# google/FluidNet

Measured on AMD Instinct MI355X. Metric: simulate_mcells_per_s, higher is better.
Workload: dtype f32

## Files before the change

fluidnet_amd/csrc/abi.cpp:

```cpp
#include "../../include/tfluids_hip.h"

#include <hip/hip_runtime.h>

#include <algorithm>
#include <cmath>
#include <cstdarg>
#include <cstdio>
#include <cstdlib>
#include <cstring>
#include <string>

#include <vector>

#include "tfl_device.hpp"
#include "tfl_host.hpp"
#include "tfl_advect.hpp"

struct tfl_layer {
  int cin = 0, cout = 0, k = 0;
  int pool = 1;
  int up = 1;
  float* w = nullptr;
  float* b = nullptr;
  int dil = 1;
// ... 285 lines not shown
    char tmp[256];
    snprintf(tmp, sizeof(tmp), "%s\"%s\": {\"calls\": %lld, \"ms\": %.6f}", i ? ", " : "", names[i].c_str(), calls[i], ms[i]);
    js += tmp;
  }
  js += "}";
  if (buf && cap > 0) {
    const size_t n = js.size() < (size_t)cap - 1 ? js.size() : (size_t)cap - 1;
    memcpy(buf, js.data(), n);
    buf[n] = 0;
  }
  return (int)names.size();
}

int64_t tfl_trace_errors(tfl_ctx* c) {
  if (!c) return -1;
  unsigned long long v = 0;
  if (hipMemcpyAsync(&v, c->d_trace_err, sizeof(v), hipMemcpyDeviceToHost, c->stream) != hipSuccess) return -1;
  if (hipMemsetAsync(c->d_trace_err, 0, sizeof(v), c->stream) != hipSuccess) return -1;
  if (hipStreamSynchronize(c->stream) != hipSuccess) return -1;
  return (int64_t)v;
}

int tfl_advectScalar(tfl_ctx* c, float dt, const tfl_tensor* s, const tfl_tensor* U, const tfl_tensor* flags,
                     const tfl_tensor* fwd, const tfl_tensor* bwd, int is3D, const char* method,
                     const tfl_tensor* fwdPos, const tfl_tensor* bwdPos, int boundaryWidth, int sampleOutsideFluid,
                     float maccormackStrength, const tfl_tensor* sDst) {
  (void)bwd; (void)boundaryWidth;
  TRY(check_flags(c, "advectScalar", flags));
  TRY(check_vel(c, "advectScalar", "U", U, flags, is3D));
  TRY(check_scalar(c, "advectScalar", "s", s, flags));
  TRY(check_scalar(c, "advectScalar", "sDst", sDst, flags));
  const int m = parse_method(method);
  if (m < 0) return fail(c, TFL_EINVAL, "advectScalar: unknown advection method '%s'", method ? method : "(null)");
  if (sDst->data == s->data && m != tfl::kMacCormackOurs)
    return fail(c, TFL_EINVAL, "advectScalar: sDst must not alias s for method '%s'", method);
  float* fwd_p = nullptr;
  float* bounds_p = nullptr;
  float* mm_p = nullptr;
  if (m == tfl::kMacCormack || m == tfl::kMacCormackOurs) {
    TRY(check_scalar(c, "advectScalar", "fwd", fwd, flags));
    fwd_p = fwd->data;
  }
  if (m == tfl::kMacCormackOurs) {
    TRY(check_vel(c, "advectScalar", "fwdPos", fwdPos, flags, is3D));
    TRY(check_vel(c, "advectScalar", "bwdPos", bwdPos, flags, is3D));
    bounds_p = fwdPos->data;
    mm_p = bwdPos->data;
  }
  WindowScope win(c);
  tfl::advect_scalar(c->stream, is3D != 0, m, flags->B, flags->Z, flags->Y, flags->X, dt, maccormackStrength,
                     sampleOutsideFluid != 0, c->d_trace_err, s->data, U->data, flags->data, fwd_p, bounds_p, mm_p,
                     sDst->data, stages_of(c));
  return check_launch(c, "advectScalar");
}

int tfl_advectVel(tfl_ctx* c, float dt, const tfl_tensor* U, const tfl_tensor* flags, const tfl_tensor* fwd,
                  const tfl_tensor* bwd, int is3D, const char* method, int boundaryWidth, float maccormackStrength,
                  const tfl_tensor* UDst) {
  (void)bwd; (void)boundaryWidth;
  TRY(check_flags(c, "advectVel", flags));
  TRY(check_vel(c, "advectVel", "U", U, flags, is3D));
  TRY(check_vel(c, "advectVel", "UDst", UDst, flags, is3D));
  int m = parse_method(method);
  if (m < 0) return fail(c, TFL_EINVAL, "advectVel: unknown advection method '%s'", method ? method : "(null)");
  if (UDst->data == U->data) return fail(c, TFL_EINVAL, "advectVel: UDst must not alias U");
  float* fwd_p = nullptr;
  if (m != tfl::kEuler && m != tfl::kEulerOurs) {
    TRY(check_vel(c, "advectVel", "fwd", fwd, flags, is3D));
    fwd_p = fwd->data;
  }
  WindowScope win(c);
  tfl::advect_vel(c->stream, is3D != 0, m, flags->B, flags->Z, flags->Y, flags->X, dt, maccormackStrength,
                  c->d_trace_err, U->data, flags->data, fwd_p, UDst->data, stages_of(c));
  return check_launch(c, "advectVel");
}

}
namespace tfl {
int advect_pair(tfl_ctx* c, float dt, float strength, const tfl_tensor* s, const tfl_tensor* U, const tfl_tensor* flags,
                const tfl_tensor* sfwd, const tfl_tensor* sbounds, const tfl_tensor* sDst, const tfl_tensor* vfwd, const tfl_tensor* UDst,
                const BcFoldArg& fold_s, const BcFoldArg& fold_v) {
  TRY(check_flags(c, "advectPair", flags));
  TRY(check_vel(c, "advectPair", "U", U, flags, 1));
  TRY(check_vel(c, "advectPair", "UDst", UDst, flags, 1));
  TRY(check_vel(c, "advectPair", "vfwd", vfwd, flags, 1));
  TRY(check_scalar(c, "advectPair", "s", s, flags));
  TRY(check_scalar(c, "advectPair", "sDst", sDst, flags));
  TRY(check_scalar(c, "advectPair", "sfwd", sfwd, flags));
  if (!sbounds || !sbounds->data || sbounds->C < 2 || !same_dims(sbounds, flags)) return fail(c, TFL_EINVAL, "advectPair: bounds needs two planes of the flags size");
  if (UDst->data == U->data) return fail(c, TFL_EINVAL, "advectPair: UDst must not alias U");
  WindowScope win(c);
  AdvArgs a; a.d = make_dom(flags->Z, flags->Y, flags->X); a.dt = dt; a.strength = strength; a.outside = 0; a.err = c->d_trace_err; a.fast = g_advect_fast;
  a.ord = BlockOrder{};
  if (!advect_pair3(c->stream, a, flags->B, s->data, U->data, flags->data, sfwd->data, sbounds->data, sDst->data, vfwd->data, UDst->data,
                    stages_of(c), fold_s, fold_v))
    return TFL_EUNSUPPORTED;
  return check_launch(c, "advectPair");
}
}
extern "C" {

int tfl_setWallBcsForward(tfl_ctx* c, const tfl_tensor* U, const tfl_tensor* flags, int is3D) {
  TRY(check_flags(c, "setWallBcsForward", flags));
  TRY(check_vel(c, "setWallBcsForward", "U", U, flags, is3D));
  tfl::set_wall_bcs(c->stream, is3D != 0, flags->B, flags->Z, flags->Y, flags->X, U->data, flags->data);
  return check_launch(c, "setWallBcsForward");
}

int tfl_velocityDivergenceForward(tfl_ctx* c, const tfl_tensor* U, const tfl_tensor* flags, const tfl_tensor* UDiv,
                                  int is3D) {
  TRY(check_flags(c, "velocityDivergenceForward", flags));
  TRY(check_vel(c, "velocityDivergenceForward", "U", U, flags, is3D));
  TRY(check_scalar(c, "velocityDivergenceForward", "UDiv", UDiv, flags));
  tfl::velocity_divergence(c->stream, is3D != 0, flags->B, flags->Z, flags->Y, flags->X, U->data, flags->data,
                           UDiv->data);
  return check_launch(c, "velocityDivergenceForward");
}

int tfl_velocityUpdateForward(tfl_ctx* c, const tfl_tensor* U, const tfl_tensor* flags, const tfl_tensor* p,
                              int is3D) {
  TRY(check_flags(c, "velocityUpdateForward", flags));
  TRY(check_vel(c, "velocityUpdateForward", "U", U, flags, is3D));
  TRY(check_scalar(c, "velocityUpdateForward", "p", p, flags));
  tfl::velocity_update(c->stream, is3D != 0, flags->B, flags->Z, flags->Y, flags->X, U->data, flags->data, p->data);
  return check_launch(c, "velocityUpdateForward");
}

int tfl_vorticityConfinement(tfl_ctx* c, const tfl_tensor* U, const tfl_tensor* flags, float strength,
                             const tfl_tensor* centered, const tfl_tensor* curl, const tfl_tensor* curlNorm,
                             const tfl_tensor* force, int is3D) {
  (void)centered; (void)force;
  TRY(check_flags(c, "vorticityConfinement", flags));
  TRY(check_vel(c, "vorticityConfinement", "U", U, flags, is3D));
  if (!curl || !curl->data || curl->C != 3 || !same_dims(curl, flags))
    return fail(c, TFL_EINVAL, "vorticityConfinement: curl must be a 3-channel grid of the flags size");
  TRY(check_scalar(c, "vorticityConfinement", "curlNorm", curlNorm, flags));
  WindowScope win(c);
  const int stg = stages_of(c);
  tfl::vorticity_confinement(c->stream, is3D != 0, flags->B, flags->Z, flags->Y, flags->X, U->data, flags->data,
                             strength, curl->data, curlNorm->data, ((stg & 2) ? 1 : 0) | ((stg & 4) ? 2 : 0));
  return check_launch(c, "vorticityConfinement");
}

int tfl_vorticityConfinementFrom(tfl_ctx* c, const tfl_tensor* USrc, const tfl_tensor* U, const tfl_tensor* flags, float strength,
                                 const tfl_tensor* curl, const tfl_tensor* curlNorm, int is3D) {
  TRY(check_flags(c, "vorticityConfinementFrom", flags));
  TRY(check_vel(c, "vorticityConfinementFrom", "U", U, flags, is3D));
  TRY(check_vel(c, "vorticityConfinementFrom", "USrc", USrc, flags, is3D));
  if (USrc->data == U->data) return fail(c, TFL_EINVAL, "vorticityConfinementFrom: U must not alias USrc (use vorticityConfinement)");
  if (!curl || !curl->data || curl->C != 3 || !same_dims(curl, flags))
    return fail(c, TFL_EINVAL, "vorticityConfinementFrom: curl must be a 3-channel grid of the flags size");
  TRY(check_scalar(c, "vorticityConfinementFrom", "curlNorm", curlNorm, flags));
  WindowScope win(c);
  if (is3D && !c->vort_from_two_launch && tfl::vorticity_confinement_fused_ok(true, flags->Z, flags->Y, flags->X) &&
      tfl::vorticity_confinement_fused(c->stream, flags->B, flags->Z, flags->Y, flags->X, USrc->data, U->data, flags->data, strength))
    return check_launch(c, "vorticityConfinementFrom");
  const tfl::ZWin w0 = tfl::g_zwin;
  const bool windowed = w0.a1 > w0.a0 || w0.b1 > w0.b0;
  if (windowed) {
    tfl::ZWin wa = {std::max(w0.a0 - 2, 0), std::min(w0.a1 + 2, (int)flags->Z), 0, 0};
    if (w0.b1 > w0.b0) { wa.b0 = std::max(w0.b0 - 2, 0); wa.b1 = std::min(w0.b1 + 2, (int)flags->Z); }
    if (w0.a1 <= w0.a0) { wa.a0 = wa.b0; wa.a1 = wa.b1; wa.b0 = wa.b1 = 0; }
    else if (wa.b1 > wa.b0 && wa.b0 <= wa.a1) { wa.a1 = wa.b1; wa.b0 = wa.b1 = 0; }
    tfl::g_zwin = wa;
    const bool a_ok = tfl::vorticity_confinement(c->stream, is3D != 0, flags->B, flags->Z, flags->Y, flags->X, U->data, flags->data, strength,
                                                 curl->data, curlNorm->data, 1, USrc->data);
    tfl::g_zwin = w0;
    if (a_ok && tfl::vorticity_confinement(c->stream, is3D != 0, flags->B, flags->Z, flags->Y, flags->X, U->data, flags->data, strength,
                                           curl->data, curlNorm->data, 2, USrc->data))
      return check_launch(c, "vorticityConfinementFrom");
    if (a_ok) return fail(c, TFL_EUNSUPPORTED, "vorticityConfinementFrom: pass B could not read USrc on this grid under a z-window");
  } else if (tfl::vorticity_confinement(c->stream, is3D != 0, flags->B, flags->Z, flags->Y, flags->X, U->data, flags->data, strength,
                                        curl->data, curlNorm->data, 3, USrc->data))
    return check_launch(c, "vorticityConfinementFrom");
  if (windowed)
    return fail(c, TFL_EUNSUPPORTED, "vorticityConfinementFrom: this grid takes the one-cell kernels, which do not run from USrc under a z-window; "
                                     "copy USrc into U and call tfl_vorticityConfinement per pass (tfl_set_stages) with the passes' own windows");
  {
    const tfl::Dom d = tfl::make_dom(flags->Z, flags->Y, flags->X);
    const size_t plane = sizeof(float) * (size_t)flags->Y * flags->X;
    const int C = is3D ? 3 : 2;
    for (int b = 0; b < flags->B; b++)
      for (int ch = 0; ch < C; ch++) {
        const size_t row = ((size_t)b * C + ch) * flags->Z;
        if (d.n0 > 0) HIP_TRY(c, hipMemcpyAsync(U->data + (row + d.w0) * (plane / 4), USrc->data + (row + d.w0) * (plane / 4), plane * d.n0, hipMemcpyDeviceToDevice, c->stream));
        if (d.nw > d.n0) HIP_TRY(c, hipMemcpyAsync(U->data + (row + d.w1) * (plane / 4), USrc->data + (row + d.w1) * (plane / 4), plane * (d.nw - d.n0), hipMemcpyDeviceToDevice, c->stream));
      }
  }
  tfl::vorticity_confinement(c->stream, is3D != 0, flags->B, flags->Z, flags->Y, flags->X, U->data, flags->data, strength,
                             curl->data, curlNorm->data, 3);
  return check_launch(c, "vorticityConfinementFrom");
}

int tfl_addBuoyancyFrom(tfl_ctx* c, const tfl_tensor* USrc, const tfl_tensor* U, const tfl_tensor* flags,
                        const tfl_tensor* density, const float gravity[3], float dt, int is3D) {
  TRY(check_flags(c, "addBuoyancy", flags));
  TRY(check_vel(c, "addBuoyancy", "U", U, flags, is3D));
  TRY(check_vel(c, "addBuoyancy", "USrc", USrc, flags, is3D));
  TRY(check_scalar(c, "addBuoyancy", "density", density, flags));
  if (!gravity) return fail(c, TFL_EINVAL, "addBuoyancy: gravity is null");
  const float sc = dt / get_dx(c, flags);
  WindowScope win(c);
  tfl::add_buoyancy(c->stream, is3D != 0, flags->B, flags->Z, flags->Y, flags->X, USrc->data, U->data, flags->data,
                    density->data, -gravity[0] * sc, -gravity[1] * sc, -gravity[2] * sc);
  return check_launch(c, "addBuoyancy");
}

int tfl_addBuoyancy(tfl_ctx* c, const tfl_tensor* U, const tfl_tensor* flags, const tfl_tensor* density,
                    const float gravity[3], float* strengthTmp, float dt, int is3D) {
  (void)strengthTmp;
  return tfl_addBuoyancyFrom(c, U, U, flags, density, gravity, dt, is3D);
}

int tfl_addGravity(tfl_ctx* c, const tfl_tensor* U, const tfl_tensor* flags, const float gravity[3], float dt,
                   int is3D, float* forceTmp) {
  (void)forceTmp;
  TRY(check_flags(c, "addGravity", flags));
  TRY(check_vel(c, "addGravity", "U", U, flags, is3D));
  if (!gravity) return fail(c, TFL_EINVAL, "addGravity: gravity is null");
  const float sc = dt / get_dx(c, flags);
  WindowScope win(c);
  tfl::add_gravity(c->stream, is3D != 0, flags->B, flags->Z, flags->Y, flags->X, U->data, flags->data,
                   gravity[0] * sc, gravity[1] * sc, gravity[2] * sc);
  return check_launch(c, "addGravity");
}

int tfl_emptyDomain(tfl_ctx* c, const tfl_tensor* flags, int is3D, int bnd) {
  TRY(check_flags(c, "emptyDomain", flags));
  if (!is3D && flags->Z != 1) return fail(c, TFL_EINVAL, "emptyDomain: 2D domain but zdepth > 1");
  tfl::empty_domain(c->stream, is3D != 0, bnd, flags->B, flags->Z, flags->Y, flags->X, flags->data);
  return check_launch(c, "emptyDomain");
}

int tfl_flagsToOccupancy(tfl_ctx* c, const tfl_tensor* flags, const tfl_tensor* occupancy) {
  TRY(check_flags(c, "flagsToOccupancy", flags));
  TRY(check_scalar(c, "flagsToOccupancy", "occupancy", occupancy, flags));
  tfl::flags_to_occupancy(c->stream, (long long)flags->B * flags->Z * flags->Y * flags->X, flags->data,
                          occupancy->data);
  return check_launch(c, "flagsToOccupancy");
}

int tfl_rectangularBlur(tfl_ctx* c, const tfl_tensor* src, int blurRad, int is3D, const tfl_tensor* dst,
                        const tfl_tensor* tmp) {
  if (!c) return TFL_EINVAL;
  if (!src || !dst || !tmp || !src->data || !dst->data || !tmp->data) return fail(c, TFL_EINVAL, "rectangularBlur: null tensor");
  if (!same_dims(dst, src) || dst->C != src->C || !same_dims(tmp, src) || tmp->C != src->C)
    return fail(c, TFL_EINVAL, "rectangularBlur: src, dst and tmp must have the same size");
  if (blurRad <= 0) return fail(c, TFL_EINVAL, "rectangularBlur: blurRad must be a positive, non-zero integer");
  if (!is3D && src->Z != 1) return fail(c, TFL_EINVAL, "rectangularBlur: 2D field but zdepth > 1");
  if (dst->data == src->data || tmp->data == src->data || tmp->data == dst->data)
    return fail(c, TFL_EINVAL, "rectangularBlur: src, dst and tmp must not alias");
  tfl::rectangular_blur(c->stream, is3D != 0, src->B, src->C, src->Z, src->Y, src->X, blurRad, src->data, dst->data, tmp->data);
  return check_launch(c, "rectangularBlur");
}

int tfl_signedDistanceField(tfl_ctx* c, const tfl_tensor* flags, int searchRad, int is3D, const tfl_tensor* dst) {
  TRY(check_flags(c, "signedDistanceField", flags));
  TRY(check_scalar(c, "signedDistanceField", "dst", dst, flags));
  if (searchRad <= 0) return fail(c, TFL_EINVAL, "signedDistanceField: searchRad must be a positive, non-zero integer");
  if (!is3D && flags->Z != 1) return fail(c, TFL_EINVAL, "signedDistanceField: 2D domain but zdepth > 1");
  tfl::signed_distance_field(c->stream, flags->B, flags->Z, flags->Y, flags->X, searchRad, flags->data, dst->data);
  return check_launch(c, "signedDistanceField");
}

int64_t tfl_pcg_workspace_floats(int32_t Z, int32_t Y, int32_t X) { return tfl::pcg_workspace_floats(Z, Y, X); }

int tfl_solveLinearSystemPCG(tfl_ctx* c, const tfl_tensor* p, const tfl_tensor* flags, const tfl_tensor* div, int is3D,
                             const char* precondType, float tol, int maxIter, int verbose, float* workspace,
                             int64_t workspace_floats, float* residual) {
  TRY(check_flags(c, "solveLinearSystemPCG", flags));
  TRY(check_scalar(c, "solveLinearSystemPCG", "p", p, flags));
  TRY(check_scalar(c, "solveLinearSystemPCG", "div", div, flags));
  if (!is3D && flags->Z != 1) return fail(c, TFL_EINVAL, "solveLinearSystemPCG: d > 1 for a 2D domain");
  int pc = -1;
  const std::string pt = precondType ? precondType : "ic0";
  if (pt == "none") pc = 0; else if (pt == "ilu0") pc = 1; else if (pt == "ic0") pc = 2;
  if (pc < 0) return fail(c, TFL_EINVAL, "solveLinearSystemPCG: precondType is not supported.");
  if (!workspace || ((uintptr_t)workspace & 7) != 0) return fail(c, TFL_EINVAL, "solveLinearSystemPCG: workspace must be 8-byte aligned");
  if (workspace_floats < tfl::pcg_workspace_floats(flags->Z, flags->Y, flags->X))
    return fail(c, TFL_EINVAL, "solveLinearSystemPCG: workspace too small (tfl_pcg_workspace_floats)");
  if ((long long)flags->Z * flags->Y * flags->X >= (1ll << 31)) return fail(c, TFL_EINVAL, "solveLinearSystemPCG: grid too large for 32-bit cell indices");
  char msg[256] = {0};
  int rc = tfl::pcg_solve(c->stream, is3D != 0, flags->B, flags->Z, flags->Y, flags->X, p->data, flags->data, div->data,
                          pc, tol, maxIter, verbose, workspace, residual, msg, sizeof(msg), c->wf_skip == 0);
  if (c->wf_skip > 0) c->wf_skip--;
  if (rc == -5) {
    c->wf_timeouts++;
    c->wf_skip = 16 << (c->wf_timeouts < 7 ? c->wf_timeouts - 1 : 6);
    fprintf(stderr, "[tfl] solveLinearSystemPCG: a pipelined triangular sweep timed out (something else holds part of the GPU?); "
                    "this solve and the next %d on this context use hyperplane sweeps (slower), then the pipelined form is retried\n", c->wf_skip);
  }
  if (rc == -5)
    rc = tfl::pcg_solve(c->stream, is3D != 0, flags->B, flags->Z, flags->Y, flags->X, p->data, flags->data, div->data,
                        pc, tol, maxIter, verbose, workspace, residual, msg, sizeof(msg), false);
  if (rc == -1 || rc == -3) return fail(c, TFL_EINVAL, "%s", msg);
  if (rc == -2) return fail(c, TFL_EINVAL, "%s", msg);
  if (rc != 0) return fail(c, TFL_EHIP, "%s", msg);
  return check_launch(c, "solveLinearSystemPCG");
}

int64_t tfl_normalize_workspace_floats(int32_t Z, int32_t Y, int32_t X) { return tfl::npm_workspace_floats(Z, Y, X); }

int tfl_normalizePressureMean(tfl_ctx* c, const tfl_tensor* p, const tfl_tensor* flags, int is3D, float* workspace,
                              int64_t workspace_floats) {
  TRY(check_flags(c, "normalizePressureMean", flags));
  TRY(check_scalar(c, "normalizePressureMean", "p", p, flags));
  if (!is3D && flags->Z != 1) return fail(c, TFL_EINVAL, "normalizePressureMean: 2D domain but zdepth > 1");
  if (!workspace || ((uintptr_t)workspace & 7) != 0) return fail(c, TFL_EINVAL, "normalizePressureMean: workspace must be 8-byte aligned");
  if (workspace_floats < tfl::npm_workspace_floats(flags->Z, flags->Y, flags->X))
// ... 367 lines not shown
      if (N > 1 && st >= g->split_stage && st < g->join_stage) {
        if (down < m->bank_down) m->bank_down = down;
        if (cp > m->bank_c) m->bank_c = cp;
      }
      down *= L.pool;
      const int bank_max = (N > 1 && mres && st >= g->split_stage && st < g->join_stage) ? down << (N - 1) : down;
      if (bank_max > m->max_down) m->max_down = bank_max;
      if (L.pool > 1 || L.up > 1 || down != 1) m->multires = true;
    }
    const int C = st == 1 ? in_c : cout[first_of[st - 1]];
    auto cmap = [&](int ci) {
      if (skip_in && ci == cin[i] - 1) return cin_p - 1;
      return joined ? (ci / C) * prev_p + ci % C : ci;
    };
    L.cin = cin_p; L.cout = cp; L.k = ksize[i];
    const int taps = is3D ? L.k * L.k * L.k : L.k * L.k;
    const int S = is3D ? L.up * L.up * L.up : L.up * L.up;
    std::vector<float> relaid((size_t)S * taps * L.cin * L.cout, 0.0f);
    for (int sub = 0; sub < S; sub++)
      for (int co = 0; co < cout[i]; co++)
        for (int ci = 0; ci < cin[i]; ci++)
          for (int t = 0; t < taps; t++)
            relaid[(((size_t)sub * taps + t) * L.cin + cmap(ci)) * L.cout + co] = weights[i][(((size_t)co * S + sub) * cin[i] + ci) * taps + t];
    std::vector<float> bias_p((size_t)S * L.cout, 0.0f);
    for (int sub = 0; sub < S; sub++)
      for (int co = 0; co < cout[i]; co++) bias_p[(size_t)sub * L.cout + co] = biases[i][(size_t)co * S + sub];
    std::vector<float> bn;
    if (g->batch_norm && !last) {
      if (!g->bn_mean[i] || !g->bn_var[i]) { m->layers.push_back(L); return cleanup("addBatchNorm: a module lacks running_mean / running_var"); }
      bn.assign((size_t)2 * L.cout, 0.0f);
      for (int co = 0; co < cout[i]; co++) {
        const double wt = (g->bn_weight && g->bn_weight[i]) ? (double)g->bn_weight[i][co] : 1.0;
        const double bi = (g->bn_bias && g->bn_bias[i]) ? (double)g->bn_bias[i][co] : 0.0;
        const double sc = wt / std::sqrt((double)g->bn_var[i][co] + g->bn_eps[i]);
        bn[co] = (float)sc;
        bn[L.cout + co] = (float)(bi - (double)g->bn_mean[i][co] * sc);
      }
    }
    if (hipMalloc((void**)&L.w, relaid.size() * sizeof(float)) != hipSuccess ||
        hipMalloc((void**)&L.b, bias_p.size() * sizeof(float)) != hipSuccess ||
        hipMemcpy(L.w, relaid.data(), relaid.size() * sizeof(float), hipMemcpyHostToDevice) != hipSuccess ||
        hipMemcpy(L.b, bias_p.data(), bias_p.size() * sizeof(float), hipMemcpyHostToDevice) != hipSuccess ||
        (!bn.empty() && (hipMalloc((void**)&L.bn, bn.size() * sizeof(float)) != hipSuccess ||
                         hipMemcpy(L.bn, bn.data(), bn.size() * sizeof(float), hipMemcpyHostToDevice) != hipSuccess))) {
      m->layers.push_back(L);
      return cleanup("uploading weights failed");
    }
    m->layers.push_back(L);
    const int width = (N > 1 && st == g->join_stage - 1 && concat) ? cp * N : cp + (o.pressure_skip ? 1 : 0);
    if (!last && width > m->max_c) m->max_c = width;
  }
  if (down != 1) return cleanup("the layers do not return to the grid resolution (pool / up factors)");
  if (N > 1 && mres) m->multires = true;
  if (m->max_c < 1) m->max_c = 1;
  return m;
}

void tfl_model_destroy(tfl_ctx* c, tfl_model* m) {
  (void)c;
  if (!m) return;
  for (auto& L : m->layers) { if (L.w) (void)hipFree(L.w); if (L.b) (void)hipFree(L.b); if (L.bn) (void)hipFree(L.bn); }
  for (int l = 0; l < 3; l++) if (m->bfrag[l]) (void)hipFree(m->bfrag[l]);
  for (int l = 0; l < 3; l++) if (m->wino[l]) (void)hipFree(m->wino[l]);
  for (int l = 0; l < 3; l++) if (m->wfrag16[l]) (void)hipFree(m->wfrag16[l]);
  if (m->d_range_err) (void)hipFree(m->d_range_err);
  if (m->h_range) (void)hipHostFree(m->h_range);
  for (int l = 0; l < 4; l++) if (m->bfrag2[l]) (void)hipFree(m->bfrag2[l]);
  if (m->tail_w4) (void)hipFree(m->tail_w4);
  if (m->tail_pack) (void)hipFree(m->tail_pack);
  if (m->tail_w5) (void)hipFree(m->tail_w5);
  if (m->d_stats) (void)hipFree(m->d_stats);
  if (m->d_ticket) (void)hipFree(m->d_ticket);
  delete m;
}

int64_t tfl_model_range_errors(tfl_ctx* c, tfl_model* m) {
  if (!c || !m) return -1;
  if (!m->d_range_err) return 0;
  unsigned long long v = 0;
  if (hipMemcpyAsync(&v, m->d_range_err, sizeof(v), hipMemcpyDeviceToHost, c->stream) != hipSuccess) return -1;
  if (hipMemsetAsync(m->d_range_err, 0, sizeof(v), c->stream) != hipSuccess) return -1;
  if (hipStreamSynchronize(c->stream) != hipSuccess) return -1;
  if (m->h_range) *(volatile unsigned long long*)m->h_range = 0;
  return (int64_t)v;
}


int64_t tfl_model_range_flag(tfl_ctx* c, tfl_model* m) {
  if (!c || !m) return -1;
  return m->h_range ? (int64_t)*(volatile unsigned long long*)m->h_range : 0;
}

static int range_gate(tfl_ctx* c, tfl_model* m, const char* who) {
  if (c && c->in_step) return TFL_OK;
  if (m && m->h_range && *(volatile unsigned long long*)m->h_range != 0)
    return fail(c, TFL_ERANGE, "%s: an earlier forward pass of this model clamped activations at the fp16 range (|x| > 65504 after the "
                               "std normalisation: a blown-up simulation); its pressure is not the reference's. Read and reset the count with "
                               "tfl_model_range_errors, or create the model under TFL_CONV_PATH=winograd (strict fp32, no range limit)", who);
  return TFL_OK;
}

static int64_t graph_ws_floats(const tfl_model* m, int B, int Z, int Y, int X, float* base, float* (*bank)[2], float** pyr = nullptr) {
  if (!m->graph || m->banks < 2) return 0;
  auto cells = [&](int f) { return (int64_t)B * (m->is3d ? (Z + f - 1) / f : Z) * ((Y + f - 1) / f) * ((X + f - 1) / f); };
  const bool mres = m->bank_type == TFL_BANKS_MRES;
  int64_t off = 0;
  for (int i = 0; i < m->banks; i++) {
    const int64_t n = (int64_t)m->bank_c * cells(mres ? m->bank_down << i : m->bank_down);
    if (base) { bank[i][0] = base + off; bank[i][1] = base + off + n; }
    off += 2 * n;
    if (mres && i > 0) {
      if (base) pyr[i] = base + off;
      off += (int64_t)m->split_c * cells(m->split_down << i);
    }
  }
  return off;
}

int64_t tfl_model_workspace_floats(const tfl_model* m, int B, int Z, int Y, int X) {
  if (!m) return -1;
  const int64_t n = (int64_t)B * Z * Y * X;
  return 4 * tfl::model_stat_blocks(B, Z, Y, X) + n * (1 + (int64_t)m->in_c + 2 * (int64_t)m->max_c + 1) + (m->m16 ? 4 : 0) +
         graph_ws_floats(m, B, Z, Y, X, nullptr, nullptr);
}

namespace {
struct ModelWs { double* partials; float* div; float* x3; float* act[2]; float* pPred; float* bank[tfl::kMaxJoinBanks][2]; float* pyr[tfl::kMaxJoinBanks]; };
int model_ws(tfl_ctx* c, const tfl_model* m, const tfl_tensor* flags, float* workspace, int64_t workspace_floats,
             ModelWs* w) {
  const int B = flags->B, Z = flags->Z, Y = flags->Y, X = flags->X;
  if (B > kMaxBatch) return fail(c, TFL_EINVAL, "model: batch size above %d", kMaxBatch);
  const int64_t n = (int64_t)B * Z * Y * X;
  if (!workspace || workspace_floats < tfl_model_workspace_floats(m, B, Z, Y, X))
    return fail(c, TFL_EINVAL, "model: workspace too small (%lld floats needed)",
                (long long)tfl_model_workspace_floats(m, B, Z, Y, X));
  if (((uintptr_t)workspace & 7) != 0) return fail(c, TFL_EINVAL, "model: workspace must be 8-byte aligned");
  w->partials = (double*)workspace;
  w->div = workspace + 4 * tfl::model_stat_blocks(B, Z, Y, X);
  w->x3 = w->div + n;
  w->act[0] = w->x3 + (int64_t)m->in_c * n;
  if (m->m16) w->act[0] = (float*)(((uintptr_t)w->act[0] + 15) & ~(uintptr_t)15);
  w->act[1] = w->act[0] + (int64_t)m->max_c * n;
  w->pPred = w->act[1] + (int64_t)m->max_c * n;
  graph_ws_floats(m, B, Z, Y, X, w->pPred + n, w->bank, w->pyr);
  return TFL_OK;
}
}

float* tfl_model_div(const tfl_model* m, int B, int Z, int Y, int X, float* workspace) {
  if (!m || !workspace) return nullptr;
  return workspace + 4 * tfl::model_stat_blocks(B, Z, Y, X);
}

static const unsigned short* wall_code_of(tfl_ctx* c, const tfl_model* m, const tfl_tensor* flags) {
  std::lock_guard<std::mutex> lock(c->wall_mu);
  for (const tfl_wall_plan* wp : c->wall_plans)
    if (wp->flags == flags->data && wp->is3d == m->is3d && wp->B == flags->B && wp->Z == flags->Z && wp->Y == flags->Y && wp->X == flags->X) return wp->code;
  return nullptr;
}

static int graph_gate(tfl_ctx* c, const tfl_model* m, const tfl_tensor* flags, const char* who) {
  if (!m->graph) return TFL_OK;
  const int f = m->max_down;
  if ((m->is3d && flags->Z % f) || flags->Y % f || flags->X % f)
    return fail(c, TFL_EINVAL, "%s: grid %dx%dx%d is not divisible by the model's downsampling factor %d (banks x pooling)", who,
                flags->Z, flags->Y, flags->X, f);
  return TFL_OK;
}

int tfl_model_begin(tfl_ctx* c, tfl_model* m, const tfl_tensor* UDiv, const tfl_tensor* flags, const tfl_tensor* UOut,
                    float* workspace, int64_t workspace_floats, int zlo, int zhi, double* stats) {
  TRY(check_flags(c, "model_begin", flags));
  if (!m) return fail(c, TFL_EINVAL, "model_begin: null model");
  TRY(range_gate(c, m, "model_begin"));
  const int is3D = m->is3d ? 1 : 0;
  TRY(check_vel(c, "model_begin", "UDiv", UDiv, flags, is3D));
  TRY(check_vel(c, "model_begin", "UOut", UOut, flags, is3D));
  if (zlo < 0 || zhi > flags->Z || zlo >= zhi) return fail(c, TFL_EINVAL, "model_begin: bad z range [%d, %d)", zlo, zhi);
  TRY(graph_gate(c, m, flags, "model_begin"));
  ModelWs w;
  TRY(model_ws(c, m, flags, workspace, workspace_floats, &w));
  WindowScope win(c);
  int stg = stages_of(c);
  if (c->defer_stats) stg &= ~4;
  m->stat_pairs_per_plane = tfl::model_stat_pairs_per_plane(flags->B, flags->Z, flags->Y, flags->X, UDiv->data, flags->data, UOut->data, w.div);
  const unsigned short* code = wall_code_of(c, m, flags);
  tfl::model_pre(c->stream, m->is3d, flags->B, flags->Z, flags->Y, flags->X, UDiv->data, flags->data, UOut->data,
                 w.div, w.partials, stats ? stats : m->d_stats, zlo, zhi, ((stg & 2) ? 1 : 0) | ((stg & 4) ? 2 : 0), m->d_ticket, code);
  return check_launch(c, "model_begin");
}

tfl_wall_plan* tfl_wall_plan_create(tfl_ctx* c, const tfl_tensor* flags) {
  if (!c || !flags || !flags->data) return nullptr;
  if (check_flags(c, "wall_plan_create", flags) != TFL_OK) return nullptr;
  const long long n = (long long)flags->B * flags->Z * flags->Y * flags->X;
  tfl_wall_plan* p = new tfl_wall_plan();
  p->flags = flags->data; p->B = flags->B; p->Z = flags->Z; p->Y = flags->Y; p->X = flags->X;
  if (hipMalloc((void**)&p->code, (size_t)n * sizeof(unsigned short)) != hipSuccess) { (void)hipGetLastError(); c->err = "wall_plan_create: hipMalloc failed"; delete p; return nullptr; }
  (void)hipDeviceSynchronize();
  p->is3d = flags->Z > 1; p->owner = c;
  tfl::wall_code(c->stream, p->is3d, flags->B, flags->Z, flags->Y, flags->X, flags->data, p->code);
  if (hipStreamSynchronize(c->stream) != hipSuccess) { (void)hipGetLastError(); (void)hipFree(p->code); c->err = "wall_plan_create: the code kernel failed"; delete p; return nullptr; }
  std::lock_guard<std::mutex> lock(c->wall_mu);
  for (tfl_wall_plan*& q : c->wall_plans)
    if (q->flags == p->flags) { q->owner = nullptr; q = p; return p; }
  c->wall_plans.push_back(p);
  return p;
}

void tfl_wall_plan_retire(tfl_wall_plan* p) {
  if (!p) return;
  tfl_ctx* o = p->owner;
  if (!o) return;
  std::lock_guard<std::mutex> lock(o->wall_mu);
  for (size_t i = 0; i < o->wall_plans.size(); i++)
    if (o->wall_plans[i] == p) { o->wall_plans.erase(o->wall_plans.begin() + (long)i); break; }
  p->owner = nullptr;
}

void tfl_wall_plan_destroy(tfl_ctx* c, tfl_wall_plan* p) {
  if (!p) return;
  (void)c;
  tfl_wall_plan_retire(p);
  if (p->code) (void)hipFree(p->code);
  delete p;
}

namespace {
float* graph_layer(hipStream_t st, const tfl_model* m, const tfl_layer& L, int B, int& Zc, int& Yc, int& Xc, const float* in,
                   float* P, float* Q, float* dst, int och, int c0, int act) {
  float* conv_out = in == P ? Q : P;
  const bool pools = L.pool > 1;
  float* cdst = (pools || !dst) ? conv_out : dst;
  const float* bs = L.bn ? L.bn : nullptr;
  const float* bt = L.bn ? L.bn + L.cout : nullptr;
  const int taps = m->is3d ? L.k * L.k * L.k : L.k * L.k;
  const int S = m->is3d ? L.up * L.up * L.up : L.up * L.up;
  for (int sub = 0; sub < S; sub++)
    if (!tfl::conv_direct_graph(st, m->is3d, B, Zc, Yc, Xc, L.cin, L.cout, L.k, act, in, L.w + (size_t)sub * taps * L.cin * L.cout,
                                L.b + (size_t)sub * L.cout, cdst, L.up, sub, cdst == dst ? och : 0, cdst == dst ? c0 : 0, L.dil,
                                pools ? nullptr : bs, pools ? nullptr : bt))
      return nullptr;
  if (m->is3d) Zc *= L.up;
  Yc *= L.up; Xc *= L.up;
  if (!pools) return cdst;
  float* pdst = dst ? dst : (conv_out == P ? Q : P);
  tfl::pool2_graph(st, m->is3d, m->pool_max, B, L.cout, Zc, Yc, Xc, conv_out, pdst, dst ? och : L.cout, dst ? c0 : 0, bs, bt);
  if (m->is3d) Zc /= 2;
  Yc /= 2; Xc /= 2;
  return pdst;
}

int graph_forward(tfl_ctx* c, const tfl_model* m, hipStream_t st, const ModelWs& w, int B, int Z, int Y, int X,
                  const float* pDiv, const double* st_in, double count) {
  const int act = 1 + m->opts.nonlin;
  const int nl = (int)m->layers.size();
  const bool mres = m->bank_type == TFL_BANKS_MRES, concat = m->aggregate == TFL_AGG_CONCAT;
  const float* in = w.x3;
  int Zc = Z, Yc = Y, Xc = X;
  auto none = [&](const tfl_layer& L) { return fail(c, TFL_EUNSUPPORTED, "model_finish: no kernel for %d output channels", L.cout); };
  for (int l = 0; l < nl;) {
    const tfl_layer& L0 = m->layers[l];
    if (m->banks > 1 && L0.stage == m->split) {
      float* join = in == w.act[0] ? w.act[1] : w.act[0];
      const int N = m->banks, Cp = m->layers[l + (m->join - m->split - 1) * N].cout, och = concat ? Cp * N : Cp;
      const float* bin[tfl::kMaxJoinBanks];
      int bZ[tfl::kMaxJoinBanks], bY[tfl::kMaxJoinBanks], bX[tfl::kMaxJoinBanks];
      bin[0] = in; bZ[0] = Zc; bY[0] = Yc; bX[0] = Xc;
      for (int i = 1; i < N; i++) {
        bin[i] = in; bZ[i] = bZ[i - 1]; bY[i] = bY[i - 1]; bX[i] = bX[i - 1];
        if (!mres) continue;
        tfl::avg_pool2(st, m->is3d, B * m->split_c, bZ[i - 1], bY[i - 1], bX[i - 1], bin[i - 1], w.pyr[i]);
        bin[i] = w.pyr[i];
        if (m->is3d) bZ[i] /= 2;
        bY[i] /= 2; bX[i] /= 2;
      }
      int slot[tfl::kMaxJoinBanks], sh[tfl::kMaxJoinBanks], n = 0;
      const float* src[tfl::kMaxJoinBanks];
      int jZ = 0, jY = 0, jX = 0;
      for (int i = 0; i < N; i++) {
        const float* x = bin[i];
        int z = bZ[i], y = bY[i], xx = bX[i];
        const bool direct = i == 0 || (concat && !mres);
        for (int s = m->split; s < m->join; s++) {
          const tfl_layer& L = m->layers[l + (s - m->split) * N + i];
          const bool last = s + 1 == m->join;
          x = graph_layer(st, m, L, B, z, y, xx, x, w.bank[i][0], w.bank[i][1], (last && direct) ? join : nullptr, och,
                          concat ? i * Cp : 0, act);
          if (!x) return none(L);
        }
        if (i == 0) { jZ = z; jY = y; jX = xx; }
        if (!direct) { slot[n] = i; sh[n] = mres ? i : 0; src[n] = x; n++; }
      }
      if (n > 0 && !tfl::bank_join(st, m->is3d, !concat, B, Cp, jZ, jY, jX, n, slot, sh, src, join, och))
        return fail(c, TFL_EINVAL, "model_finish: bad bank join");
      in = join; Zc = jZ; Yc = jY; Xc = jX;
      l += (m->join - m->split) * N;
      continue;
    }
    const bool last = l + 1 == nl;
    const bool joins_skip = m->opts.pressure_skip && l + 2 == nl;
    float* dst = last ? w.pPred : (joins_skip ? (in == w.act[0] ? w.act[1] : w.act[0]) : nullptr);
    float* out = graph_layer(st, m, L0, B, Zc, Yc, Xc, in, w.act[0], w.act[1], dst, joins_skip ? L0.cout + 1 : L0.cout, 0,
                             last ? 0 : act);
    if (!out) return none(L0);
    if (joins_skip) tfl::model_skip_channel(st, B, (long long)Z * Y * X, pDiv, st_in, count, out, L0.cout + 1, L0.cout);
    in = out;
    l++;
  }
  return TFL_OK;
}
}

int tfl_model_finish(tfl_ctx* c, tfl_model* m, const tfl_tensor* pDiv, const tfl_tensor* flags,
                     const tfl_tensor* pOut, const tfl_tensor* UOut, float* workspace, int64_t workspace_floats,
                     const double* stats, double count, const tfl_tensor* UBC, const tfl_tensor* UBCInvMask,
                     int doClamp, float lo, float hi) {
  TRY(check_flags(c, "model_finish", flags));
  if (!m) return fail(c, TFL_EINVAL, "model_finish: null model");
  const int is3D = m->is3d ? 1 : 0;
  TRY(check_vel(c, "model_finish", "UOut", UOut, flags, is3D));
  TRY(check_scalar(c, "model_finish", "pDiv", pDiv, flags));
  TRY(check_scalar(c, "model_finish", "pOut", pOut, flags));
  if ((UBC == nullptr) != (UBCInvMask == nullptr)) return fail(c, TFL_EINVAL, "model_finish: UBC and UBCInvMask go together");
  if (UBC) {
    TRY(check_vel(c, "model_finish", "UBC", UBC, flags, is3D));
    TRY(check_vel(c, "model_finish", "UBCInvMask", UBCInvMask, flags, is3D));
  }
  if (!(count > 1.0)) return fail(c, TFL_EINVAL, "model_finish: Sample variance requires more than one sample.");
  ModelWs w;
  TRY(model_ws(c, m, flags, workspace, workspace_floats, &w));
  const int B = flags->B, Z = flags->Z, Y = flags->Y, X = flags->X;
  const double* st_in = stats ? stats : m->d_stats;
  hipStream_t st = c->stream;
  TRY(graph_gate(c, m, flags, "model_finish"));
  if (m->graph && (stats || c->stages || c->zwin.a1 > c->zwin.a0 || c->zwin.b1 > c->zwin.b0))
    return fail(c, TFL_EUNSUPPORTED, "model_finish: banked, batch-norm and max-pool models run un-sharded only");
  if (m->custom) {
    if (stats || c->stages || c->zwin.a1 > c->zwin.a0 || c->zwin.b1 > c->zwin.b0)
      return fail(c, TFL_EUNSUPPORTED, "model_finish: models with non-default tfl_model_opts run un-sharded only");
    const tfl_model_opts& o = m->opts;
// ... 287 lines not shown
```

fluidnet_amd/csrc/model.hip:

```cpp
#include "tfl_device.hpp"
#include "tfl_fastmath.hpp"
#include "tfl_host.hpp"
#include "tfl_vec4.hpp"

#include <algorithm>
#include <cstdlib>

#ifndef TFL_LB_BCS
#define TFL_LB_BCS 1
#endif
#ifndef TFL_LB_PROJECT
#define TFL_LB_PROJECT 1
#endif

namespace tfl {

template <bool IS3D>
__device__ __forceinline__ void wall_mask_from(int fc, int fxm, int fxp, int fym, int fyp, int fzm, int fzp, bool& zx,
                                               bool& zy, bool& zz) {
  zx = zy = zz = false;
  const bool cf = fc & kFluid, co = fc & kObstacle;
  if (!cf && !co) return;
  zx = (fxm & kObstacle) || (co && (fxm & kFluid));
  zy = (fym & kObstacle) || (co && (fym & kFluid));
  zz = IS3D && ((fzm & kObstacle) || (co && (fzm & kFluid)));
  if (cf) {
    if ((fxm & kStick) || (fxp & kStick)) { zy = true; zz = IS3D; }
    if ((fym & kStick) || (fyp & kStick)) { zx = true; zz = IS3D; }
    if (IS3D && ((fzm & kStick) || (fzp & kStick))) { zx = true; zy = true; }
  }
}

template <bool IS3D>
__device__ __forceinline__ void wall_zero_mask(const Dom& d, const float* __restrict__ flags, int i, int j, int k, int o,
                                               bool& zx, bool& zy, bool& zz) {
  const int fc = (int)flags[o];
  if (!(fc & (kFluid | kObstacle))) { zx = zy = zz = false; return; }
  const int fxm = i > 0 ? (int)flags[o - 1] : 0;
  const int fym = j > 0 ? (int)flags[o - d.sy] : 0;
  const int fzm = (IS3D && k > 0) ? (int)flags[o - d.sz] : 0;
  int fxp = 0, fyp = 0, fzp = 0;
  if (fc & kFluid) {
    fxp = i < d.X - 1 ? (int)flags[o + 1] : 0;
    fyp = j < d.Y - 1 ? (int)flags[o + d.sy] : 0;
    fzp = (IS3D && k < d.Z - 1) ? (int)flags[o + d.sz] : 0;
  }
  wall_mask_from<IS3D>(fc, fxm, fxp, fym, fyp, fzm, fzp, zx, zy, zz);
}

template <bool IS3D, int AXIS>
__device__ __forceinline__ float u_bc_at(const Dom& d, const float* __restrict__ U, const float* __restrict__ flags,
                                         int i, int j, int k) {
  const int o = TFL_AT(d, i, j, k);
  bool zx, zy, zz;
  wall_zero_mask<IS3D>(d, flags, i, j, k, o, zx, zy, zz);
  const bool z = AXIS == 0 ? zx : (AXIS == 1 ? zy : zz);
  return z ? 0.0f : U[o + AXIS * d.sc];
}

template <bool COHERENT>
__device__ __forceinline__ void reduce_partials(const double* __restrict__ p, long long count, double* __restrict__ out, int tid) {
  __shared__ double sh[512];
  if (!COHERENT) {
    double r1, r2;
    block_sum_pairs(p, count, sh, tid, r1, r2);
    if (tid == 0) { out[0] = r1; out[1] = r2; }
    return;
  }
  double s1 = 0.0, s2 = 0.0;
  for (long long t = tid; t < count; t += 256) {
    s1 += __builtin_bit_cast(double, __hip_atomic_load(reinterpret_cast<const unsigned long long*>(p + t * 2), __ATOMIC_RELAXED, __HIP_MEMORY_SCOPE_AGENT));
    s2 += __builtin_bit_cast(double, __hip_atomic_load(reinterpret_cast<const unsigned long long*>(p + t * 2 + 1), __ATOMIC_RELAXED, __HIP_MEMORY_SCOPE_AGENT));
  }
  double* sh1 = sh; double* sh2 = sh + 256;
  sh1[tid] = s1; sh2[tid] = s2;
  __syncthreads();
  for (int w = 128; w > 0; w >>= 1) {
    if (tid < w) { sh1[tid] += sh1[tid + w]; sh2[tid] += sh2[tid + w]; }
    __syncthreads();
  }
  if (tid == 0) { out[0] = sh1[0]; out[1] = sh2[0]; }
  __syncthreads();
}

struct StatTail { unsigned* ticket; double* stats; long long per_sample; unsigned per_plane, planes; int B; };
[[maybe_unused]] constexpr int kStatTickets = 1 << 16;
template <bool FOLD>
__device__ __forceinline__ void publish_and_maybe_reduce(const StatTail& tl, double* __restrict__ partials, long long blk, double p1,
                                                         double p2, int tid) {
  if (!FOLD) {
    if (tid == 0) { partials[blk * 2] = p1; partials[blk * 2 + 1] = p2; }
    return;
  }
  __shared__ int last;
  if (tid == 0) {
    if (tl.ticket) {
      __hip_atomic_store(reinterpret_cast<unsigned long long*>(partials + blk * 2), __builtin_bit_cast(unsigned long long, p1), __ATOMIC_RELAXED, __HIP_MEMORY_SCOPE_AGENT);
      __hip_atomic_store(reinterpret_cast<unsigned long long*>(partials + blk * 2 + 1), __builtin_bit_cast(unsigned long long, p2), __ATOMIC_RELAXED, __HIP_MEMORY_SCOPE_AGENT);
      asm volatile("s_waitcnt vmcnt(0)" ::: "memory");
      unsigned* mine = tl.ticket + 1 + (unsigned)(blk / tl.per_plane);
      last = 0;
      if (atomicAdd(mine, 1u) == tl.per_plane - 1u) {
        *mine = 0u;
        last = atomicAdd(tl.ticket, 1u) == tl.planes - 1u;
      }
    } else {
      partials[blk * 2] = p1; partials[blk * 2 + 1] = p2;
      last = 0;
    }
  }
  if (!tl.ticket) return;
  __syncthreads();
  if (!last) return;
  for (int b = 0; b < tl.B; b++) reduce_partials<true>(partials + (long long)b * tl.per_sample * 2, tl.per_sample, tl.stats + b * 2, tid);
  if (tid == 0) *tl.ticket = 0u;
}

template <bool IS3D, bool FOLD = false>
__global__ __launch_bounds__(256) void k_bcs_div_stats(Dom d, const float* __restrict__ U, const float* __restrict__ flags,
                                                       float* __restrict__ Ubc, float* __restrict__ div,
                                                       double* __restrict__ partials, StatTail tl) {
  const int i = blockIdx.x * blockDim.x + threadIdx.x;
  const int j = blockIdx.y * blockDim.y + threadIdx.y;
  int b, k; dom_bk(d, b, k);
  const long long cells = d.sc;
  const int C = IS3D ? 3 : 2;
  double s1 = 0.0, s2 = 0.0;
  if (i < d.X && j < d.Y) {
    U += b * cells * C; Ubc += b * cells * C; flags += b * cells; div += b * cells;
    const int o = TFL_AT(d, i, j, k);
    bool zx, zy, zz;
    wall_zero_mask<IS3D>(d, flags, i, j, k, o, zx, zy, zz);
    const float ux = zx ? 0.0f : U[o];
    const float uy = zy ? 0.0f : U[o + d.sc];
    const float uz = IS3D ? (zz ? 0.0f : U[o + 2 * d.sc]) : 0.0f;
    Ubc[o] = ux; Ubc[o + d.sc] = uy; if (IS3D) Ubc[o + 2 * d.sc] = uz;
    s1 = (double)ux + (double)uy + (double)uz;
    s2 = (double)ux * ux + (double)uy * uy + (double)uz * uz;
    float dv = 0.0f;
    if (!on_border<IS3D>(d, i, j, k) && (((int)flags[o]) & kFluid)) {
      dv = ux - u_bc_at<IS3D, 0>(d, U, flags, i + 1, j, k) + uy - u_bc_at<IS3D, 1>(d, U, flags, i, j + 1, k);
      if (IS3D) dv += (uz - u_bc_at<IS3D, 2>(d, U, flags, i, j, k + 1));
    }
    div[o] = dv;
  }
#pragma unroll
  for (int off = 32; off > 0; off >>= 1) { s1 += __shfl_down(s1, off, 64); s2 += __shfl_down(s2, off, 64); }
  __shared__ double part[8];
  const int tid = threadIdx.y * blockDim.x + threadIdx.x;
  if ((tid & 63) == 0) { part[(tid >> 6) * 2] = s1; part[(tid >> 6) * 2 + 1] = s2; }
  __syncthreads();
  const long long blk = blockIdx.x + (long long)gridDim.x * (blockIdx.y + (long long)gridDim.y * ((long long)b * d.Z + k));
  publish_and_maybe_reduce<FOLD>(tl, partials, blk, (part[0] + part[2]) + (part[4] + part[6]), (part[1] + part[3]) + (part[5] + part[7]), tid);
}

template <bool IS3D>
__global__ __launch_bounds__(256) void k_wall_code(Dom d, const float* __restrict__ flags, unsigned short* __restrict__ code) {
  const int i = blockIdx.x * blockDim.x + threadIdx.x, j = blockIdx.y * blockDim.y + threadIdx.y;
  int b, k; dom_bk(d, b, k);
  if (i >= d.X || j >= d.Y) return;
  flags += b * d.sc; code += b * d.sc;
  const int o = TFL_AT(d, i, j, k);
  const int fc = (int)flags[o];
  const int fxm = i > 0 ? (int)flags[o - 1] : 0, fxp = i < d.X - 1 ? (int)flags[o + 1] : 0;
  const int fym = j > 0 ? (int)flags[o - d.sy] : 0, fyp = j < d.Y - 1 ? (int)flags[o + d.sy] : 0;
  const int fzm = (IS3D && k > 0) ? (int)flags[o - d.sz] : 0, fzp = (IS3D && k < d.Z - 1) ? (int)flags[o + d.sz] : 0;
  bool zx, zy, zz;
  wall_mask_from<IS3D>(fc, fxm, fxp, fym, fyp, fzm, fzp, zx, zy, zz);
  unsigned m = (zx ? 1u : 0u) | (zy ? 2u : 0u) | (zz ? 4u : 0u) | ((fc & kFluid) ? 8u : 0u) | (((fc & kEmpty) && !(fc & kOutflow)) ? 16u : 0u);
  m |= ((fxm & kFluid) ? 32u : 0u) | ((fym & kFluid) ? 64u : 0u) | ((fzm & kFluid) ? 128u : 0u);
  m |= ((fxm & kEmpty) ? 256u : 0u) | ((fym & kEmpty) ? 512u : 0u) | ((fzm & kEmpty) ? 1024u : 0u);
  code[o] = (unsigned short)m;
}

template <bool IS3D>
__global__ __launch_bounds__(256, TFL_LB_BCS) void k_bcs_div_stats_code(Dom d, const float* __restrict__ U, const unsigned short* __restrict__ code,
                                                                       float* __restrict__ Ubc, float* __restrict__ div,
                                                                       double* __restrict__ partials, StatTail tl) {
  const V4Ctx c = v4_ctx(d);
  const int j = blockIdx.y * blockDim.y + threadIdx.y;
  int b, k; dom_bk(d, b, k);
  const bool live = c.i0 < d.X && j < d.Y;
  const long long cells = d.sc;
  const int C = IS3D ? 3 : 2;
  U += b * cells * C; Ubc += b * cells * C; code += b * cells; div += b * cells;
  const int o = TFL_AT(d, c.i0, j, k);
  const bool yp = live && j < d.Y - 1, zp = live && IS3D && k < d.Z - 1;
  const unsigned long long cc_v = *reinterpret_cast<const unsigned long long*>(code + (live ? o : 0));
  const unsigned long long cy_v = *reinterpret_cast<const unsigned long long*>(code + (yp ? o + d.sy : 0));
  const unsigned long long cz_v = *reinterpret_cast<const unsigned long long*>(code + (zp ? o + d.sz : 0));
  const unsigned long long cc = live ? cc_v : 0ull, cy = yp ? cy_v : 0ull, cz = zp ? cz_v : 0ull;
  float u[3][4], uyp[4], uzp[4];
#pragma unroll
  for (int a = 0; a < 3; a++) v4_load(U, o + a * d.sc, live && a < C, 0.0f, u[a]);
  v4_load(U, o + d.sc + d.sy, yp, 0.0f, uyp);
  v4_load(U, o + 2 * d.sc + d.sz, zp, 0.0f, uzp);
  const bool need = c.last && live && c.has_r;
  const int oo = o + 4;
  const unsigned gcode = code[need ? oo : 0];
  const float gu = U[need ? oo : 0];
  double s1 = 0.0, s2 = 0.0;
  float ubx[5];
#pragma unroll
  for (int q = 0; q < 4; q++) {
    const unsigned m = (unsigned)(cc >> (16 * q));
    if (m & 1u) u[0][q] = 0.0f;
    if (m & 2u) u[1][q] = 0.0f;
    if (!IS3D || (m & 4u)) u[2][q] = 0.0f;
    ubx[q] = u[0][q];
    if (live) {
      s1 += (double)u[0][q] + (double)u[1][q] + (double)u[2][q];
      s2 += (double)u[0][q] * u[0][q] + (double)u[1][q] * u[1][q] + (double)u[2][q] * u[2][q];
    }
  }
  ubx[4] = from_lane_above(ubx[0]);
  if (c.last) ubx[4] = (need && !(gcode & 1u)) ? gu : 0.0f;
  float dv[4];
  const bool row_inner = live && j >= 1 && j <= d.Y - 2 && (!IS3D || (k >= 1 && k <= d.Z - 2));
#pragma unroll
  for (int q = 0; q < 4; q++) {
    const int i = c.i0 + q;
    dv[q] = 0.0f;
    if (row_inner && i >= 1 && i <= d.X - 2 && ((unsigned)(cc >> (16 * q)) & 8u)) {
      const float by = ((unsigned)(cy >> (16 * q)) & 2u) ? 0.0f : uyp[q];
      float t = u[0][q] - ubx[q + 1] + u[1][q] - by;
      if (IS3D) {
        const float bz = ((unsigned)(cz >> (16 * q)) & 4u) ? 0.0f : uzp[q];
        t += (u[2][q] - bz);
      }
      dv[q] = t;
    }
  }
  if (live) {
#pragma unroll
    for (int a = 0; a < 3; a++)
      if (a < C) v4_store(Ubc, o + a * d.sc, u[a]);
    v4_store(div, o, dv);
  }
#pragma unroll
  for (int off = 32; off > 0; off >>= 1) { s1 += __shfl_down(s1, off, 64); s2 += __shfl_down(s2, off, 64); }
  __shared__ double part[8];
  const int tid = threadIdx.y * blockDim.x + threadIdx.x;
  if ((tid & 63) == 0) { part[(tid >> 6) * 2] = s1; part[(tid >> 6) * 2 + 1] = s2; }
  __syncthreads();
  const long long blk = blockIdx.x + (long long)gridDim.x * (blockIdx.y + (long long)gridDim.y * ((long long)b * d.Z + k));
  publish_and_maybe_reduce<false>(tl, partials, blk, (part[0] + part[2]) + (part[4] + part[6]), (part[1] + part[3]) + (part[5] + part[7]), tid);
}

template <bool IS3D, bool FOLD = false>
__global__ __launch_bounds__(256, TFL_LB_BCS) void k_bcs_div_stats_v4(Dom d, const float* __restrict__ U, const float* __restrict__ flags,
                                                          float* __restrict__ Ubc, float* __restrict__ div,
                                                          double* __restrict__ partials, StatTail tl) {
  const V4Ctx c = v4_ctx(d);
  const int j = blockIdx.y * blockDim.y + threadIdx.y;
  int b, k; dom_bk(d, b, k);
  const bool live = c.i0 < d.X && j < d.Y;
  const long long cells = d.sc;
  const int C = IS3D ? 3 : 2;
  U += b * cells * C; Ubc += b * cells * C; flags += b * cells; div += b * cells;
  const int o = TFL_AT(d, c.i0, j, k);
  const bool ym = live && j > 0, yp = live && j < d.Y - 1, yp2 = live && j < d.Y - 2;
  const bool zm = live && IS3D && k > 0, zp = live && IS3D && k < d.Z - 1, zp2 = live && IS3D && k < d.Z - 2;
  float fc[6], fym[4], fyp[6], fzm[4], fzp[6], fyp2[4], fypzm[4], fypzp[4], fzp2[4], fymzp[4];
  v4_load6<true, true>(c, flags, o, live, 0.0f, fc);
  v4_load(flags, o - d.sy, ym, 0.0f, fym);
  v4_load6<true, true>(c, flags, o + d.sy, yp, 0.0f, fyp);
  v4_load(flags, o - d.sz, zm, 0.0f, fzm);
  v4_load6<true, true>(c, flags, o + d.sz, zp, 0.0f, fzp);
  v4_load(flags, o + 2 * d.sy, yp2, 0.0f, fyp2);
  v4_load(flags, o + d.sy - d.sz, yp && zm, 0.0f, fypzm);
  v4_load(flags, o + d.sy + d.sz, yp && zp, 0.0f, fypzp);
  v4_load(flags, o + 2 * d.sz, zp2, 0.0f, fzp2);
  v4_load(flags, o - d.sy + d.sz, ym && zp, 0.0f, fymzp);
  float u[3][4], uyp[4], uzp[4];
#pragma unroll
  for (int a = 0; a < 3; a++) v4_load(U, o + a * d.sc, live && a < C, 0.0f, u[a]);
  v4_load(U, o + d.sc + d.sy, yp, 0.0f, uyp);
  v4_load(U, o + 2 * d.sc + d.sz, zp, 0.0f, uzp);
  const bool need = c.last && live && c.has_r;
  const int oo = o + 4;
  const float gym = flags[need && ym ? oo - d.sy : 0], gyp = flags[need && yp ? oo + d.sy : 0];
  const float gzm = flags[need && zm ? oo - d.sz : 0], gzp = flags[need && zp ? oo + d.sz : 0];
  const float gu = U[need ? oo : 0];
  double s1 = 0.0, s2 = 0.0;
  float ubx[5];
#pragma unroll
  for (int q = 0; q < 4; q++) {
    bool zx, zy, zz;
    wall_mask_from<IS3D>((int)fc[q + 1], (int)fc[q], (int)fc[q + 2], (int)fym[q], (int)fyp[q + 1], (int)fzm[q], (int)fzp[q + 1],
                         zx, zy, zz);
    if (zx) u[0][q] = 0.0f;
    if (zy) u[1][q] = 0.0f;
    if (!IS3D || zz) u[2][q] = 0.0f;
    ubx[q] = u[0][q];
    if (live) {
      s1 += (double)u[0][q] + (double)u[1][q] + (double)u[2][q];
      s2 += (double)u[0][q] * u[0][q] + (double)u[1][q] * u[1][q] + (double)u[2][q] * u[2][q];
    }
  }
  ubx[4] = from_lane_above(ubx[0]);
  {
    if (c.last) {
      float v = 0.0f;
      if (need) {
        const int f = (int)fc[5];
        bool zx, zy, zz;
        wall_mask_from<IS3D>(f, (int)fc[4], 0, ym ? (int)gym : 0, yp ? (int)gyp : 0, zm ? (int)gzm : 0, zp ? (int)gzp : 0, zx, zy, zz);
        v = zx ? 0.0f : gu;
      }
      ubx[4] = v;
    }
  }
  float dv[4];
  const bool row_inner = live && j >= 1 && j <= d.Y - 2 && (!IS3D || (k >= 1 && k <= d.Z - 2));
#pragma unroll
  for (int q = 0; q < 4; q++) {
    const int i = c.i0 + q;
    dv[q] = 0.0f;
    if (row_inner && i >= 1 && i <= d.X - 2 && (((int)fc[q + 1]) & kFluid)) {
      bool zx, zy, zz;
      wall_mask_from<IS3D>((int)fyp[q + 1], (int)fyp[q], (int)fyp[q + 2], (int)fc[q + 1], (int)fyp2[q], (int)fypzm[q],
                           (int)fypzp[q], zx, zy, zz);
      const float by = zy ? 0.0f : uyp[q];
      float t = u[0][q] - ubx[q + 1] + u[1][q] - by;
      if (IS3D) {
        wall_mask_from<IS3D>((int)fzp[q + 1], (int)fzp[q], (int)fzp[q + 2], (int)fymzp[q], (int)fypzp[q], (int)fc[q + 1],
                             (int)fzp2[q], zx, zy, zz);
        const float bz = zz ? 0.0f : uzp[q];
        t += (u[2][q] - bz);
      }
      dv[q] = t;
    }
  }
  if (live) {
#pragma unroll
    for (int a = 0; a < 3; a++)
      if (a < C) v4_store(Ubc, o + a * d.sc, u[a]);
    v4_store(div, o, dv);
  }
#pragma unroll
  for (int off = 32; off > 0; off >>= 1) { s1 += __shfl_down(s1, off, 64); s2 += __shfl_down(s2, off, 64); }
  __shared__ double part[8];
  const int tid = threadIdx.y * blockDim.x + threadIdx.x;
  if ((tid & 63) == 0) { part[(tid >> 6) * 2] = s1; part[(tid >> 6) * 2 + 1] = s2; }
  __syncthreads();
  const long long blk = blockIdx.x + (long long)gridDim.x * (blockIdx.y + (long long)gridDim.y * ((long long)b * d.Z + k));
  publish_and_maybe_reduce<FOLD>(tl, partials, blk, (part[0] + part[2]) + (part[4] + part[6]), (part[1] + part[3]) + (part[5] + part[7]), tid);
}

__global__ __launch_bounds__(256) void k_reduce_stats(const double* __restrict__ partials, long long per_sample,
                                                      long long first, long long count, double* __restrict__ stats) {
  const int b = blockIdx.x;
  reduce_partials<false>(partials + ((long long)b * per_sample + first) * 2, count, stats + b * 2, (int)threadIdx.x);
}

__device__ __forceinline__ float scale_from_stats(const double* __restrict__ stats, int b, double n) {
  const double s1 = stats[b * 2], s2 = stats[b * 2 + 1];
  return (float)sqrt(fmax(n * s2 - s1 * s1, 0.0) / (n * (n - 1.0)));
}

template <bool IS3D>
__global__ __launch_bounds__(256) void k_net_input(Dom d, const float* __restrict__ pDiv, const float* __restrict__ div,
                                                   const float* __restrict__ flags, const double* __restrict__ stats,
                                                   double count, float* __restrict__ x3) {
  const int i = blockIdx.x * blockDim.x + threadIdx.x;
  const int j = blockIdx.y * blockDim.y + threadIdx.y;
  int b, k; dom_bk(d, b, k);
  if (i >= d.X || j >= d.Y) return;
  const long long cells = d.sc;
  const float scale = scale_from_stats(stats, b, count);
  const int o = TFL_AT(d, i, j, k);
  const long long bo = b * cells;
  x3 += bo * 3;
  x3[o] = pDiv[bo + o] / scale;
  x3[o + d.sc] = div[bo + o] / scale;
  const int f = (int)flags[bo + o];
  x3[o + 2 * d.sc] = (f == kFluid) ? 0.0f : ((f == kObstacle) ? 1.0f : -1.0f);
}

template <bool IS3D>
__global__ __launch_bounds__(256) void k_net_input_gen(Dom d, int in_pDiv, int in_UDiv, int in_div, const float* __restrict__ pDiv,
                                                       const float* __restrict__ Ubc, const float* __restrict__ div,
                                                       const float* __restrict__ flags, const double* __restrict__ stats,
                                                       double count, float* __restrict__ x) {
  const int i = blockIdx.x * blockDim.x + threadIdx.x;
  const int j = blockIdx.y * blockDim.y + threadIdx.y;
  int b, k; dom_bk(d, b, k);
  if (i >= d.X || j >= d.Y) return;
  const long long cells = d.sc;
  const int C = IS3D ? 3 : 2;
  const float scale = scale_from_stats(stats, b, count);
  const int o = TFL_AT(d, i, j, k);
  const long long bo = b * cells;
  x += bo * (in_pDiv + in_UDiv * C + in_div + 1);
  int ch = 0;
  if (in_pDiv) x[o + (ch++) * cells] = pDiv[bo + o] / scale;
  if (in_UDiv)
    for (int c = 0; c < C; c++) x[o + (ch++) * cells] = Ubc[bo * C + o + c * cells] / scale;
  if (in_div) x[o + (ch++) * cells] = div[bo + o] / scale;
  const int f = (int)flags[bo + o];
// ... 179 lines not shown
    const int fxm = CODE ? 0 : (q > 0 ? (int)fc[q - 1] : (int)f_left), fxp = CODE ? 0 : (q < 3 ? (int)fc[q + 1] : (int)f_right);
    const float pxm = q > 0 ? pc[q - 1] : p_left;
    float v[3];
    if (scale_ok) { v[0] = div_by<1>(u[0][q], scale, inv_scale); v[1] = div_by<1>(u[1][q], scale, inv_scale); v[2] = IS3D ? div_by<1>(u[2][q], scale, inv_scale) : 0.0f; }
    else { v[0] = u[0][q] / scale; v[1] = u[1][q] / scale; v[2] = IS3D ? u[2][q] / scale : 0.0f; }
    if (!(row_border || i < 1 || i > d.X - 2)) {
      const int fn[3] = {fxm, CODE ? 0 : (int)fym[q], (!CODE && IS3D) ? (int)fzm[q] : 0};
      const float pn[3] = {pxm, pym[q], pzm[q]};
      const bool cell_fluid = CODE ? (m & 8u) != 0 : (f & kFluid) != 0;
      const bool cell_open = CODE ? (m & 16u) != 0 : ((f & kEmpty) && !(f & kOutflow));
      if (cell_fluid) {
#pragma unroll
        for (int c = 0; c < C; c++) {
          const bool nf = CODE ? (m & (32u << c)) != 0 : (fn[c] & kFluid) != 0, ne = CODE ? (m & (256u << c)) != 0 : (fn[c] & kEmpty) != 0;
          if (nf) v[c] -= (pc[q] - pn[c]);
          if (ne) v[c] -= pc[q];
        }
      } else if (cell_open) {
#pragma unroll
        for (int c = 0; c < C; c++) {
          const bool nf = CODE ? (m & (32u << c)) != 0 : (fn[c] & kFluid) != 0;
          v[c] = nf ? v[c] + pn[c] : 0.0f;
        }
      }
    }
    bool z[3];
    if (CODE) { z[0] = m & 1u; z[1] = m & 2u; z[2] = m & 4u; }
    else wall_mask_from<IS3D>(f, fxm, fxp, (int)fym[q], (int)fyp[q], (int)fzm[q], (int)fzp[q], z[0], z[1], z[2]);
    po[q] = pc[q] * scale;
#pragma unroll
    for (int c = 0; c < C; c++) {
      float w = z[c] ? 0.0f : v[c] * scale;
      if (bc_row && i >= bx0 && i <= bx1) w = w * umk[c][q] + ubc[c][q];
      if (bc.enable_clamp) w = fminf(fmaxf(w, bc.lo), bc.hi);
      u[c][q] = w;
    }
  }
  *reinterpret_cast<float4*>(pOut + o) = make_float4(po[0], po[1], po[2], po[3]);
#pragma unroll
  for (int c = 0; c < 3; c++)
    if (c < C) *reinterpret_cast<float4*>(Uio + o + c * d.sc) = make_float4(u[c][0], u[c][1], u[c][2], u[c][3]);
  if (IS3D && bc.reach_acc) {
    float m = fmaxf(fmaxf(fabsf(u[2][0]), fabsf(u[2][1])), fmaxf(fabsf(u[2][2]), fabsf(u[2][3])));
#pragma unroll
    for (int off = 32; off > 0; off >>= 1) m = fmaxf(m, __shfl_xor(m, off, 64));
    __shared__ float wm[4];
    const int tid = threadIdx.y * blockDim.x + threadIdx.x;
    if ((tid & 63) == 0) wm[tid >> 6] = m;
    __syncthreads();
    if (tid == 0) {
      const float bm = fmaxf(fmaxf(wm[0], wm[1]), fmaxf(wm[2], wm[3]));
      if (bm > reach_seen) atomicMax(reinterpret_cast<unsigned int*>(bc.reach_acc), __float_as_uint(bm));
    }
  }
  publish_reach(bc, (blockIdx.x | blockIdx.y | blockIdx.z | threadIdx.x | threadIdx.y) == 0);
}

__global__ __launch_bounds__(256) void k_apply_bcs(long long n, float* __restrict__ x, const float* __restrict__ bcv,
                                                   const float* __restrict__ inv, int do_clamp, float lo, float hi) {
  for (long long t = (long long)blockIdx.x * blockDim.x + threadIdx.x; t < n; t += (long long)gridDim.x * blockDim.x) {
    float v = x[t];
    if (bcv) v = v * inv[t] + bcv[t];
    if (do_clamp) v = fminf(fmaxf(v, lo), hi);
    x[t] = v;
  }
}

__global__ __launch_bounds__(256) void k_apply_bcs_indexed(long long n, const int* __restrict__ idx, float* __restrict__ x,
                                                           const float* __restrict__ bcv, const float* __restrict__ inv) {
  for (long long t = (long long)blockIdx.x * blockDim.x + threadIdx.x; t < n; t += (long long)gridDim.x * blockDim.x) {
    const int e = idx[t];
    x[e] = x[e] * inv[e] + bcv[e];
  }
}

struct BcMultiArgs { long long n[8]; const int* idx[8]; float* x[8]; const float* bc[8]; const float* inv[8]; };
__global__ __launch_bounds__(256) void k_apply_bcs_indexed_multi(BcMultiArgs a) {
  const int f = blockIdx.y;
  const long long n = a.n[f];
  const int* __restrict__ idx = a.idx[f];
  float* __restrict__ x = a.x[f];
  const float* __restrict__ bcv = a.bc[f];
  const float* __restrict__ inv = a.inv[f];
  for (long long t = (long long)blockIdx.x * blockDim.x + threadIdx.x; t < n; t += (long long)gridDim.x * blockDim.x) {
    const int e = idx[t];
    x[e] = x[e] * inv[e] + bcv[e];
  }
}

__global__ __launch_bounds__(256) void k_bc_scan(long long n, const float* __restrict__ bcv, const float* __restrict__ inv,
                                                 int* __restrict__ counters, int* __restrict__ idx) {
  for (long long e = (long long)blockIdx.x * blockDim.x + threadIdx.x; e < n; e += (long long)gridDim.x * blockDim.x) {
    const float m = inv[e], b = bcv[e];
    if (m != 1.0f || b != 0.0f) {
      const int pos = atomicAdd(&counters[0], 1);
      if (idx) idx[pos] = (int)e;
      if (m != 0.0f || !(fabsf(b) <= 1e6f)) counters[1] = 1;
    }
  }
}

struct PackArgs {
  float* ptr[8];
  float* buf[8];
  long long start[9];
  long long per_row[8];
  long long zoff[8];
  int n;
};
__global__ __launch_bounds__(256) void k_pack_planes(PackArgs a, long long zstride, int unpack) {
  const long long total = a.start[a.n];
  for (long long t = (long long)blockIdx.x * blockDim.x + threadIdx.x; t < total; t += (long long)gridDim.x * blockDim.x) {
    int f = 0;
#pragma unroll
    for (int q = 1; q < 8; q++) if (q < a.n && t >= a.start[q]) f = q;
    const long long r = t - a.start[f];
    const long long row = r / a.per_row[f], within = r - row * a.per_row[f];
    float* g = a.ptr[f] + row * zstride + a.zoff[f] + within;
    if (unpack) *g = a.buf[f][r];
    else a.buf[f][r] = *g;
  }
}

#define TFL_GRID3(d, B) dim3(((d).X + 63) / 64, ((d).Y + 3) / 4, (unsigned)((d).nw * (B)))

long long model_stat_blocks(int B, int Z, int Y, int X) {
  return (long long)((X + 63) / 64) * ((Y + 3) / 4) * Z * B;
}

bool model_stats_fold_requested() {
#ifdef TFL_EXPERIMENTS
  const char* ef = getenv("TFL_STATS_FOLD");
  return ef && atoi(ef) == 1;
#else
  return false;
#endif
}

long long model_stat_pairs_per_plane(int B, int Z, int Y, int X, const float* U, const float* flags, const float* Ubc, const float* div) {
  const Dom d = make_dom(Z, Y, X);
  const dim3 grd = TFL_GRID3(d, B);
  const Vec4Launch v = vec4_launch(B, Z, Y, X, {U, flags, Ubc, div});
  return v.ok ? (long long)v.grd.x * v.grd.y : (long long)grd.x * grd.y;
}

void wall_code(hipStream_t st, bool is3d, int B, int Z, int Y, int X, const float* flags, unsigned short* code) {
  const Dom d = make_dom(Z, Y, X);
  const dim3 blk(64, 4, 1), grd = TFL_GRID3(d, B);
  if (is3d) k_wall_code<true><<<grd, blk, 0, st>>>(d, flags, code);
  else k_wall_code<false><<<grd, blk, 0, st>>>(d, flags, code);
}

void model_pre(hipStream_t st, bool is3d, int B, int Z, int Y, int X, const float* U, const float* flags, float* Ubc,
               float* div, double* partials, double* stats, int zlo, int zhi, int stages, unsigned* ticket, const unsigned short* code) {
  const Dom d = make_dom(Z, Y, X);
  const dim3 blk(64, 4, 1), grd = TFL_GRID3(d, B);
  const Vec4Launch v = vec4_launch(B, Z, Y, X, {U, flags, Ubc, div});
  const long long per_plane = v.ok ? (long long)v.grd.x * v.grd.y : (long long)grd.x * grd.y;
#ifdef TFL_EXPERIMENTS
  const bool fused = ticket && (stages & 3) == 3 && d.nw == Z && d.n0 == Z && zlo == 0 && zhi == Z && model_stats_fold_requested() &&
                     (long long)Z * B + 1 <= kStatTickets && per_plane < (1ll << 31);
#else
  const bool fused = false;
  (void)ticket; (void)zlo; (void)zhi;
#endif
  StatTail tl = {nullptr, stats, per_plane * Z, (unsigned)per_plane, (unsigned)(Z * B), B};
  if (fused) tl.ticket = ticket;
  if (stages & 1) {
    if (v.ok && code && !fused) {
      TFL_TIMED_EXT("k_bcs_div_stats", st);
      if (is3d) TFL_LAUNCH_EXT((k_bcs_div_stats_code<true>), v.grd, v.blk, 0, st, d, U, code, Ubc, div, partials, tl);
      else TFL_LAUNCH_EXT((k_bcs_div_stats_code<false>), v.grd, v.blk, 0, st, d, U, code, Ubc, div, partials, tl);
    } else if (v.ok) {
      TFL_TIMED_EXT("k_bcs_div_stats", st);
#ifdef TFL_EXPERIMENTS
      if (fused) {
        if (is3d) TFL_LAUNCH_EXT((k_bcs_div_stats_v4<true, true>), v.grd, v.blk, 0, st, d, U, flags, Ubc, div, partials, tl);
        else TFL_LAUNCH_EXT((k_bcs_div_stats_v4<false, true>), v.grd, v.blk, 0, st, d, U, flags, Ubc, div, partials, tl);
      } else
#endif
      {
        if (is3d) TFL_LAUNCH_EXT((k_bcs_div_stats_v4<true, false>), v.grd, v.blk, 0, st, d, U, flags, Ubc, div, partials, tl);
        else TFL_LAUNCH_EXT((k_bcs_div_stats_v4<false, false>), v.grd, v.blk, 0, st, d, U, flags, Ubc, div, partials, tl);
      }
    } else {
      TFL_TIMED("k_bcs_div_stats", st);
#ifdef TFL_EXPERIMENTS
      if (fused) {
        if (is3d) k_bcs_div_stats<true, true><<<grd, blk, 0, st>>>(d, U, flags, Ubc, div, partials, tl);
        else k_bcs_div_stats<false, true><<<grd, blk, 0, st>>>(d, U, flags, Ubc, div, partials, tl);
      } else
#endif
      {
        if (is3d) k_bcs_div_stats<true, false><<<grd, blk, 0, st>>>(d, U, flags, Ubc, div, partials, tl);
        else k_bcs_div_stats<false, false><<<grd, blk, 0, st>>>(d, U, flags, Ubc, div, partials, tl);
      }
    }
  }
  if ((stages & 2) && !fused) { TFL_TIMED_EXT("k_reduce_stats", st); TFL_LAUNCH_EXT(k_reduce_stats, B, 256, 0, st, (const double*)partials, per_plane * Z, per_plane * zlo, per_plane * (zhi - zlo), stats); }
}

void model_net_input(hipStream_t st, bool is3d, int B, int Z, int Y, int X, const float* pDiv, const float* div,
                     const float* flags, const double* stats, double count, float* x3) {
  const Dom d = make_dom(Z, Y, X);
  const dim3 blk(64, 4, 1), grd = TFL_GRID3(d, B);
  if (is3d) { TFL_TIMED("k_net_input", st); k_net_input<true><<<grd, blk, 0, st>>>(d, pDiv, div, flags, stats, count, x3); }
  else { TFL_TIMED("k_net_input", st); k_net_input<false><<<grd, blk, 0, st>>>(d, pDiv, div, flags, stats, count, x3); }
}

void model_net_input_gen(hipStream_t st, bool is3d, int B, int Z, int Y, int X, int in_pDiv, int in_UDiv, int in_div,
                         const float* pDiv, const float* Ubc, const float* div, const float* flags, const double* stats,
                         double count, float* x) {
  const Dom d = make_dom(Z, Y, X);
  const dim3 blk(64, 4, 1), grd = TFL_GRID3(d, B);
  TFL_TIMED("k_net_input", st);
  if (is3d) k_net_input_gen<true><<<grd, blk, 0, st>>>(d, in_pDiv, in_UDiv, in_div, pDiv, Ubc, div, flags, stats, count, x);
  else k_net_input_gen<false><<<grd, blk, 0, st>>>(d, in_pDiv, in_UDiv, in_div, pDiv, Ubc, div, flags, stats, count, x);
}

void model_field_stats(hipStream_t st, int B, long long n, const float* field, int mode, double* stats) {
  TFL_TIMED("k_field_stats", st);
  k_field_stats<<<B, 1024, 0, st>>>(n, field, mode, stats);
}

void model_skip_channel(hipStream_t st, int B, long long cells, const float* pDiv, const double* stats, double count,
                        float* dst, int och, int ch) {
  TFL_TIMED("k_skip_channel", st);
  k_skip_channel<<<dim3((unsigned)((cells + 255) / 256), (unsigned)B), 256, 0, st>>>(cells, pDiv, stats, count, dst, och, ch);
}

bool model_project(hipStream_t st, bool is3d, int B, int Z, int Y, int X, const float* pPred, const float* flags,
                   const double* stats, double count, float* Uio, float* pOut, const float* UBC, const float* UInvMask,
                   int do_clamp, float lo, float hi, const unsigned long long* range_src, unsigned long long* range_dst,
                   const float* reach_src, float* reach_dst, float* reach_acc, const unsigned short* wall_code, unsigned* reach_tick) {
  const Dom d = make_dom(Z, Y, X);
  const dim3 blk(64, 4, 1), grd = TFL_GRID3(d, B);
  BcArgs bc; bc.enable_clamp = do_clamp; bc.lo = lo; bc.hi = hi;
  bc.range_src = range_dst ? range_src : nullptr; bc.range_dst = range_dst;
  bc.reach_src = reach_dst ? reach_src : nullptr; bc.reach_dst = reach_dst;
  bc.reach_acc = nullptr; bc.wall_code = nullptr; bc.reach_tick = bc.reach_src ? reach_tick : nullptr;
  bc.UBC = UBC; bc.UInvMask = UInvMask; bc.fold = UBC ? no_fold() : take_fold();
  const uintptr_t al = (uintptr_t)pPred | (uintptr_t)flags | (uintptr_t)Uio | (uintptr_t)pOut | (uintptr_t)UBC |
                       (uintptr_t)UInvMask;
  if (X % 4 == 0 && (al & 15) == 0 && !exp_env("TFL_NO_VEC4")) {
    const dim3 vb(32, 8, 1), vg((X / 4 + 31) / 32, (Y + 7) / 8, (unsigned)(d.nw * B));
    const bool acc = is3d && reach_acc && X % 128 == 0 && Y % 8 == 0;
    if (acc) bc.reach_acc = reach_acc;
    TFL_TIMED_EXT("k_project", st);
    if (wall_code) {
      bc.wall_code = wall_code;
      if (is3d) TFL_LAUNCH_EXT((k_project_v4<true, true>), vg, vb, 0, st, d, pPred, flags, stats, count, Uio, pOut, bc);
      else TFL_LAUNCH_EXT((k_project_v4<false, true>), vg, vb, 0, st, d, pPred, flags, stats, count, Uio, pOut, bc);
    } else if (is3d) TFL_LAUNCH_EXT((k_project_v4<true>), vg, vb, 0, st, d, pPred, flags, stats, count, Uio, pOut, bc);
    else TFL_LAUNCH_EXT((k_project_v4<false>), vg, vb, 0, st, d, pPred, flags, stats, count, Uio, pOut, bc);
    return acc;
  }
  if (is3d) { TFL_TIMED("k_project", st); k_project<true><<<grd, blk, 0, st>>>(d, pPred, flags, stats, count, Uio, pOut, bc); }
  else { TFL_TIMED("k_project", st); k_project<false><<<grd, blk, 0, st>>>(d, pPred, flags, stats, count, Uio, pOut, bc); }
  return false;
}

void apply_bcs(hipStream_t st, long long n, float* x, const float* bcv, const float* inv, int do_clamp, float lo,
               float hi) {
  long long blocks = (n + 255) / 256;
  if (blocks > 4096) blocks = 4096;
  { TFL_TIMED("k_apply_bcs", st); k_apply_bcs<<<(int)(blocks > 0 ? blocks : 1), 256, 0, st>>>(n, x, bcv, inv, do_clamp, lo, hi); }
}

long long pack_planes(hipStream_t st, int n, float* const* ptrs, const int* rows, const int* zlo, const int* nplanes,
                      long long zstride, long long yx, float* buf, int unpack, float* const* bufs) {
  PackArgs a;
  a.n = n;
  a.start[0] = 0;
  for (int i = 0; i < 8; i++) {
    a.ptr[i] = i < n ? ptrs[i] : nullptr;
    a.buf[i] = i < n ? (bufs ? bufs[i] : buf + a.start[i]) : nullptr;
    a.per_row[i] = i < n ? (long long)nplanes[i] * yx : 1;
    a.zoff[i] = i < n ? (long long)zlo[i] * yx : 0;
    a.start[i + 1] = a.start[i] + (i < n ? (long long)rows[i] * a.per_row[i] : 0);
  }
  long long blocks = (a.start[n] + 255) / 256;
  if (blocks > 2048) blocks = 2048;
  if (blocks < 1) return 0;
  { TFL_TIMED(unpack ? "k_unpack_planes" : "k_pack_planes", st); k_pack_planes<<<(int)blocks, 256, 0, st>>>(a, zstride, unpack); }
  return a.start[n];
}

void bc_scan(hipStream_t st, long long n, const float* bcv, const float* inv, int* counters, int* idx) {
  const int blocks = (int)std::min<long long>((n + 255) / 256, 4096);
  k_bc_scan<<<blocks > 0 ? blocks : 1, 256, 0, st>>>(n, bcv, inv, counters, idx);
}

void apply_bcs_indexed_multi(hipStream_t st, int count, const long long* n, const int* const* idx, float* const* x,
                             const float* const* bcv, const float* const* inv) {
  BcMultiArgs a;
  long long nmax = 0;
  for (int i = 0; i < 8; i++) {
    a.n[i] = i < count ? n[i] : 0; a.idx[i] = i < count ? idx[i] : nullptr; a.x[i] = i < count ? x[i] : nullptr;
    a.bc[i] = i < count ? bcv[i] : nullptr; a.inv[i] = i < count ? inv[i] : nullptr;
    if (a.n[i] > nmax) nmax = a.n[i];
  }
  if (nmax == 0) return;
  const unsigned bx = (unsigned)std::min<long long>((nmax + 255) / 256, 4096);
  TFL_TIMED_EXT("k_apply_bcs_indexed", st);
  TFL_LAUNCH_EXT(k_apply_bcs_indexed_multi, dim3(bx, (unsigned)count, 1), 256, 0, st, a);
}

void apply_bcs_indexed(hipStream_t st, long long n, const int* idx, float* x, const float* bcv, const float* inv) {
  if (n <= 0) return;
  long long blocks = (n + 255) / 256;
  if (blocks > 4096) blocks = 4096;
  { TFL_TIMED_EXT("k_apply_bcs_indexed", st); TFL_LAUNCH_EXT(k_apply_bcs_indexed, (int)blocks, 256, 0, st, n, idx, x, bcv, inv); }
}

}
```

fluidnet_amd/csrc/simulate.cpp:

```cpp
#include "../../include/tfluids_hip.h"
#include "tfl_ctx.hpp"
#include "tfl_host.hpp"

#include <cstddef>
#include <algorithm>
#include <vector>
#include <cmath>
#include <cstdio>
#include <cstdlib>
#include <chrono>
#include <cstring>
#include <thread>
#include <string>

namespace tfl { const unsigned long long* model_range_counter(const tfl_model* m); }
namespace tfl {
int advect_pair(tfl_ctx* c, float dt, float strength, const tfl_tensor* s, const tfl_tensor* U, const tfl_tensor* flags,
                const tfl_tensor* sfwd, const tfl_tensor* sbounds, const tfl_tensor* sDst, const tfl_tensor* vfwd, const tfl_tensor* UDst,
                const BcFoldArg& fold_s, const BcFoldArg& fold_v);
}

struct tfl_bc_plan {
  tfl_tensor bc, inv;
  int* d_idx = nullptr;
  long long n_idx = 0, numel = 0;
  bool sparse = false;
  bool idem = false;
  bool boxed = false;
  int box[6] = {0, 0, 0, 0, 0, 0};
  tfl::BcFold* d_fold = nullptr;
};

namespace {

long long numel_of(const tfl_tensor* t) { return (long long)t->B * t->C * t->Z * t->Y * t->X; }

struct Todo { const tfl_tensor* x; const tfl_bc_plan* plan; };

int apply_bcs(tfl_ctx* c, const Todo* todo, int n) {
  const tfl_tensor *xs[8], *bs[8], *ms[8];
  const int32_t* is[8];
  int64_t ns[8];
  int k = 0;
  for (int i = 0; i < n; i++) {
    const tfl_bc_plan* p = todo[i].plan;
    if (p->sparse) {
      if (p->n_idx == 0) continue;
      xs[k] = todo[i].x; bs[k] = &p->bc; ms[k] = &p->inv; is[k] = p->d_idx; ns[k] = p->n_idx; k++;
      if (k == 8) { int rc = tfl_applyBCsIndexedMulti(c, k, xs, bs, ms, is, ns); if (rc) return rc; k = 0; }
    } else {
      int rc = tfl_applyBCs(c, todo[i].x, &p->bc, &p->inv, 0, 0.0f, 0.0f);
      if (rc) return rc;
    }
  }
  if (k == 1) return tfl_applyBCsIndexed(c, xs[0], bs[0], ms[0], is[0], ns[0]);
  if (k > 1) return tfl_applyBCsIndexedMulti(c, k, xs, bs, ms, is, ns);
  return TFL_OK;
}

struct Unchanged { bool p, U, density; };

int set_const_vals(tfl_ctx* c, const tfl_sim_state* s, const tfl_tensor* U_now, bool with_U, Unchanged un, unsigned density_done = 0) {
  Todo todo[10];
  int n = 0;
  auto add = [&](const tfl_tensor* x, const tfl_bc_plan* p, bool unchanged) {
    if (!p) return;
    if (unchanged && p->sparse && p->idem) return;
    todo[n].x = x; todo[n].plan = p; n++;
  };
  add(s->p, s->pBC, un.p);
  if (with_U) add(U_now, s->UBC, un.U);
  for (int i = 0; i < s->n_density; i++)
    if (!((density_done >> i) & 1u)) add(s->density[i], s->densityBC[i], un.density);
  return apply_bcs(c, todo, n);
}

bool fold_ask(tfl_ctx* c, const tfl_bc_plan* p) {
  const char* e = getenv("TFL_BC_FOLD");
  const bool off = e && atoi(e) == 0;
  c->fold_done = false;
  if (off || !p || !p->sparse || !p->boxed || !p->d_fold || p->n_idx == 0) { c->fold = tfl::no_fold(); return false; }
  c->fold = tfl::BcFoldArg{p->d_fold, (unsigned)p->box[2] | ((unsigned)p->box[4] << 16), (unsigned)p->box[3] | ((unsigned)p->box[5] << 16)};
  return true;
}
tfl::BcFoldArg fold_arg(const tfl_bc_plan* p) {
  const char* e = getenv("TFL_BC_FOLD");
  if ((e && atoi(e) == 0) || !p || !p->sparse || !p->boxed || !p->d_fold || p->n_idx == 0) return tfl::no_fold();
  return tfl::BcFoldArg{p->d_fold, (unsigned)p->box[2] | ((unsigned)p->box[4] << 16), (unsigned)p->box[3] | ((unsigned)p->box[5] << 16)};
}
bool fold_took(tfl_ctx* c) {
  const bool d = c->fold_done;
  c->fold = tfl::no_fold();
  c->fold_done = false;
  return d;
}

struct InStep {
  tfl_ctx* c;
  explicit InStep(tfl_ctx* ctx) : c(ctx) { c->in_step = true; }
  ~InStep() { c->in_step = false; }
};

struct Sizes { long long N, C; int B, Z, Y, X; bool is3d; };
Sizes sizes_of(const tfl_sim_state* s) {
  Sizes z;
  z.B = s->flags->B; z.Z = s->flags->Z; z.Y = s->flags->Y; z.X = s->flags->X;
  z.N = (long long)z.B * z.Z * z.Y * z.X; z.C = s->U->C; z.is3d = s->U->C == 3;
  return z;
}
std::string method_of(const tfl_sim_params* p) { return p->simMethod && p->simMethod[0] ? p->simMethod : "convnet"; }

}

extern "C" {

tfl_bc_plan* tfl_bc_plan_create(tfl_ctx* c, const tfl_tensor* bc, const tfl_tensor* invMask) {
  if (!c || !bc || !invMask || !bc->data || !invMask->data) return nullptr;
  if (numel_of(bc) != numel_of(invMask) || numel_of(bc) >= (1ll << 31)) return nullptr;
  tfl_bc_plan* p = new tfl_bc_plan();
  p->bc = *bc; p->inv = *invMask; p->numel = numel_of(bc);
  int* d_cnt = nullptr;
  int h_cnt[2] = {0, 0};
  (void)hipDeviceSynchronize();
  if (hipMalloc((void**)&d_cnt, 2 * sizeof(int)) != hipSuccess) { delete p; return nullptr; }
  (void)hipMemset(d_cnt, 0, 2 * sizeof(int));
  tfl::bc_scan(nullptr, p->numel, bc->data, invMask->data, d_cnt, nullptr);
  (void)hipMemcpy(h_cnt, d_cnt, 2 * sizeof(int), hipMemcpyDeviceToHost);
  p->n_idx = h_cnt[0];
  p->idem = h_cnt[1] == 0;
  p->sparse = p->n_idx * 4 < p->numel;
  if (p->sparse && p->n_idx > 0) {
    if (hipMalloc((void**)&p->d_idx, sizeof(int) * (size_t)p->n_idx) != hipSuccess) { (void)hipFree(d_cnt); delete p; return nullptr; }
    (void)hipMemset(d_cnt, 0, 2 * sizeof(int));
    tfl::bc_scan(nullptr, p->numel, bc->data, invMask->data, d_cnt, p->d_idx);
    (void)hipDeviceSynchronize();
    std::vector<int> h((size_t)p->n_idx);
    if (hipMemcpy(h.data(), p->d_idx, sizeof(int) * h.size(), hipMemcpyDeviceToHost) == hipSuccess) {
      int lo[3] = {bc->X, bc->Y, bc->Z}, hi[3] = {-1, -1, -1};
      for (int e : h) {
        const int x = e % bc->X, y = (e / bc->X) % bc->Y, z = (int)((e / ((long long)bc->X * bc->Y)) % bc->Z);
        lo[0] = std::min(lo[0], x); hi[0] = std::max(hi[0], x);
        lo[1] = std::min(lo[1], y); hi[1] = std::max(hi[1], y);
        lo[2] = std::min(lo[2], z); hi[2] = std::max(hi[2], z);
      }
      for (int a = 0; a < 3; a++) { p->box[2 * a] = lo[a]; p->box[2 * a + 1] = hi[a]; }
      p->boxed = true;
      const tfl::BcFold hf = {bc->data, invMask->data, lo[0], hi[0], lo[1], hi[1], lo[2], hi[2]};
      if ((((uintptr_t)bc->data | (uintptr_t)invMask->data) & 15) == 0 && bc->Y < 65536 && bc->Z < 65536 && hipMalloc((void**)&p->d_fold, sizeof(hf)) == hipSuccess &&
          hipMemcpy(p->d_fold, &hf, sizeof(hf), hipMemcpyHostToDevice) != hipSuccess) { (void)hipFree(p->d_fold); p->d_fold = nullptr; }
    }
  }
  (void)hipFree(d_cnt);
  return p;
}

void tfl_bc_plan_destroy(tfl_ctx* c, tfl_bc_plan* p) {
  (void)c;
  if (!p) return;
  if (p->d_idx) (void)hipFree(p->d_idx);
  if (p->d_fold) (void)hipFree(p->d_fold);
  delete p;
}

int64_t tfl_simulate_workspace_floats(tfl_ctx* c, const tfl_sim_params* prm, const tfl_sim_state* s) {
  if (!c || !prm || !s || !s->flags || !s->U) return 0;
  const Sizes z = sizes_of(s);
  long long need = std::max((3 + 2 * z.C) * z.N, 3 * z.C * z.N);
  need = std::max(need, (2 * z.C + 4) * z.N);
  const std::string sm = method_of(prm);
  if (sm == "convnet" && s->model) need = std::max<long long>(need, tfl_model_workspace_floats(s->model, z.B, z.Z, z.Y, z.X));
  if (sm == "jacobi") need = std::max(need, 3 * z.N + z.B);
  if (sm == "pcg") need = std::max<long long>(need, z.N + 2 + tfl_pcg_workspace_floats(z.Z, z.Y, z.X));
  return need + 2;
}

int tfl_simulate_step(tfl_ctx* c, const tfl_sim_params* prm, const tfl_sim_state* s, float* ws, int64_t ws_floats) {
  if (!c || !prm || !s || !s->p || !s->U || !s->flags) return TFL_EINVAL;
  if (s->n_density < 0 || s->n_density > 8) return TFL_EINVAL;
  if (!ws || ((uintptr_t)ws & 15) != 0 || ws_floats < tfl_simulate_workspace_floats(c, prm, s)) return TFL_EINVAL;
  const Sizes z = sizes_of(s);
  const int is3D = z.is3d ? 1 : 0;
  const char* method = (prm->advectionMethod && prm->advectionMethod[0]) ? prm->advectionMethod : "maccormackOurs";
  const bool ours = std::strcmp(method, "maccormackOurs") == 0;
  auto view = [&](float* base, int C) { tfl_tensor t = *s->flags; t.data = base; t.C = C; return t; };
  int rc;
  if (s->model && method_of(prm) == "convnet" && tfl_model_range_flag(c, s->model) > 0) {
    c->err = "simulate_step: an earlier step's ConvNet projection clamped activations at the fp16 range (a blown-up simulation); "
             "read the count with tfl_model_range_errors, or create the model under TFL_CONV_PATH=winograd (strict fp32)";
    return TFL_ERANGE;
  }
  if (s->model && method_of(prm) == "convnet" && tfl::model_is_graph(s->model)) {
    const int f = tfl::model_grid_factor(s->model);
    if ((z.is3d && z.Z % f) || z.Y % f || z.X % f) {
      c->err = "simulate_step: the grid is not divisible by the model's downsampling factor " + std::to_string(f) + " (banks x pooling)";
      return TFL_EINVAL;
    }
  }
  InStep in_step(c);

  unsigned density_done = 0;
  for (int i = 0; i < s->n_density; i++) {
    tfl_tensor fwd = view(ws, 1), bwd = view(ws + z.N, 1), fwdPos = view(ws + 2 * z.N, (int)z.C),
               bwdPos = view(ws + (2 + z.C) * z.N, (int)z.C), out = view(ws + (2 + 2 * z.C) * z.N, 1);
    const tfl_tensor* dst = ours ? s->density[i] : &out;
    fold_ask(c, s->densityBC[i]);
    rc = tfl_advectScalar(c, prm->dt, s->density[i], s->U, s->flags, &fwd, &bwd, is3D, method, &fwdPos, &bwdPos, 1, 0,
                          prm->maccormackStrength, dst);
    if (fold_took(c)) density_done |= 1u << i;
    if (rc) return rc;
    if (!ours) { rc = tfl_copy(c, s->density[i], &out); if (rc) return rc; }
  }
  tfl_tensor vfwd = view(ws, (int)z.C), vbwd = view(ws + z.C * z.N, (int)z.C), Uadv = view(ws + 2 * z.C * z.N, (int)z.C);
  const bool buoyant = s->n_density > 0 && prm->buoyancyScale > 0.0;
  const double dx = tfl_getDx(c, s->flags);
  const float bsc = (float)(-(dx / 4.0) * prm->buoyancyScale);
  const float bg[3] = {prm->gravity[0] * bsc, prm->gravity[1] * bsc, prm->gravity[2] * bsc};
  const bool U_pair_asked = fold_ask(c, s->UBC);
  bool buoy_folded = false;
  {
    const char* e = getenv("TFL_BUOY_FOLD");
    const bool rho_final = buoyant && (!s->densityBC[0] || (density_done & 1u));
    if (rho_final && ours && is3D && !(e && atoi(e) == 0) && (!s->UBC || U_pair_asked)) {
      float dxf;
      if (c->dx_dim > 0) dxf = 1.0f / (float)c->dx_dim;
      else if (c->dx_override > 0.0f) dxf = c->dx_override;
      else dxf = 1.0f / (float)std::max(std::max(s->flags->X, s->flags->Y), s->flags->Z);
      const float bs = prm->dt / dxf;
      c->buoy = tfl::BuoyFold{s->density[0]->data, -bg[0] * bs, -bg[1] * bs, -bg[2] * bs};
    }
    c->buoy_done = false;
  }
  rc = tfl_advectVel(c, prm->dt, s->U, s->flags, &vfwd, &vbwd, is3D, method, 1, prm->maccormackStrength, &Uadv);
  const bool Uadv_done = fold_took(c);
  buoy_folded = c->buoy_done;
  c->buoy = tfl::no_buoy(); c->buoy_done = false;
  if (rc) return rc;
  const bool vort = prm->vorticityConfinementAmp > 0.0;
  const bool vfused = vort && tfl::vorticity_confinement_fused_ok(is3D != 0, (int)z.Z, (int)z.Y, (int)z.X);
  tfl_tensor curl = z.is3d ? view(ws + 3 * z.N, 3) : view(ws, 3), cnorm = z.is3d ? view(ws + 9 * z.N, 1) : view(ws + 3 * z.N, 1);
  tfl_tensor Utmp = view(ws, (int)z.C);
  const tfl_tensor* cur = &Uadv;
  rc = set_const_vals(c, s, cur, !Uadv_done, Unchanged{false, false, false}, density_done);
  if (rc) return rc;

  const std::string sm = method_of(prm);
  const bool fold_forces = !prm->outputDiv && sm == "convnet";
  const bool gravity_on = prm->gravityScale > 0.0;
  bool U_folded = false;
  if (buoyant && !buoy_folded) {
    const tfl_tensor* dst = vfused ? &Utmp : s->U;
    const bool last = fold_forces && !gravity_on && !vort;
    if (last) fold_ask(c, s->UBC);
    rc = tfl_addBuoyancyFrom(c, cur, dst, s->flags, s->density[0], bg, prm->dt, is3D);
    if (last) U_folded = fold_took(c);
    if (rc) return rc;
    cur = dst;
  }
  if (gravity_on) {
    const float sc = (float)((-dx / 4.0) * prm->gravityScale);
    const float g[3] = {prm->gravity[0] * sc, prm->gravity[1] * sc, prm->gravity[2] * sc};
    rc = tfl_addGravity(c, cur, s->flags, g, prm->dt, is3D, nullptr);
    if (rc) return rc;
  }
  if (vort) {
    const float strength = (float)(dx * prm->vorticityConfinementAmp);
    if (fold_forces) fold_ask(c, s->UBC);
    if (cur != s->U) {
      c->vort_from_two_launch = !vfused;
      rc = tfl_vorticityConfinementFrom(c, cur, s->U, s->flags, strength, &curl, &cnorm, is3D);
      c->vort_from_two_launch = false;
    } else {
      tfl_tensor centered = view(ws + 4 * z.N, (int)z.C), force = view(ws + (4 + z.C) * z.N, (int)z.C);
      rc = tfl_vorticityConfinement(c, s->U, s->flags, strength, &centered, &curl, &cnorm, &force, is3D);
    }
    if (fold_forces) U_folded = fold_took(c);
    if (rc) return rc;
    cur = s->U;
  }
  if (cur != s->U && (prm->outputDiv || sm != "convnet")) {
    rc = tfl_copy(c, s->U, cur);
    if (rc) return rc;
    cur = s->U;
  }
  if (prm->outputDiv) return TFL_OK;

  if (sm != "convnet") {
    rc = tfl_setWallBcsForward(c, s->U, s->flags, is3D);
    if (rc) return rc;
  }
  rc = set_const_vals(c, s, cur, !U_folded, Unchanged{true, false, true});
  if (rc) return rc;
  const int max_iter = prm->maxIter > 0 ? prm->maxIter : 100;
  if (sm == "convnet") {
    if (!s->model) return TFL_EINVAL;
    const bool late_ubc = s->UBC && s->UBC->sparse && s->UBC->idem;
    const tfl_tensor* ubc = (s->UBC && !late_ubc) ? &s->UBC->bc : nullptr;
    const tfl_tensor* umask = (s->UBC && !late_ubc) ? &s->UBC->inv : nullptr;
    if (late_ubc) fold_ask(c, s->UBC);
    rc = tfl_model_forward(c, s->model, s->p, cur, s->flags, s->p, s->U, ws, ws_floats, ubc, umask, 1, -1e6f, 1e6f);
    const bool folded = fold_took(c);
    if (rc) return rc;
    return set_const_vals(c, s, s->U, late_ubc && !folded, Unchanged{false, false, true});
  }
  tfl_tensor div = view(ws, 1);
  rc = tfl_velocityDivergenceForward(c, s->U, s->flags, &div, is3D);
  if (rc) return rc;
  if (sm == "jacobi") {
    tfl_tensor pPrev = view(ws + z.N, 1), pDelta = view(ws + 2 * z.N, 1), norm = view(ws + 3 * z.N, 1);
    norm.B = z.B; norm.Z = norm.Y = norm.X = 1;
    rc = tfl_solveLinearSystemJacobi(c, s->p, s->flags, &div, &pPrev, &pDelta, &norm, is3D, 0.0f, max_iter, 0, nullptr);
  } else if (sm == "pcg") {
    float* pws = ws + ((z.N + 1) & ~1ll);
    float res = 0.0f;
    rc = tfl_solveLinearSystemPCG(c, s->p, s->flags, &div, is3D, prm->pcgPrecond && prm->pcgPrecond[0] ? prm->pcgPrecond : "ic0",
                                  1e-4f, max_iter, 0, pws, ws_floats - (pws - ws), &res);
  } else {
    return TFL_EINVAL;
  }
  if (rc) return rc;
  rc = tfl_velocityUpdateForward(c, s->U, s->flags, s->p, is3D);
  if (rc) return rc;
  rc = set_const_vals(c, s, s->U, true, Unchanged{false, false, true});
  if (rc) return rc;
  return tfl_applyBCs(c, s->U, nullptr, nullptr, 1, -1e6f, 1e6f);
}


namespace {

struct Halo { const tfl_tensor* t; int below, above; };

struct Msg {
  int tag, n;
  Halo f[10];
  float *send_lo, *recv_lo, *send_hi, *recv_hi;
  long long n_send_lo, n_recv_lo, n_send_hi, n_recv_hi;
};

struct SlabGeom {
  int Zl, o0, o1, R, H;
  int J;
  bool lower, upper;
  long long yx, N;
  int B;
};

int slab_geom(tfl_ctx* c, const tfl_sim_state* s, const tfl_slab* sl, SlabGeom* g) {
  if (!s || !s->flags || !s->U || !sl) return TFL_EINVAL;
  if (s->n_density < 0 || s->n_density > 8) { if (c) c->err = "simulate_step_slab: 0 to 8 density channels"; return TFL_EINVAL; }
  g->Zl = s->flags->Z; g->B = s->flags->B;
  g->o0 = sl->own_lo; g->o1 = sl->own_hi;
  g->R = sl->reach > 0 ? sl->reach : 1;
  g->H = tfl_slab_halo(g->R);
  g->yx = (long long)s->flags->Y * s->flags->X;
  g->N = (long long)g->B * g->Zl * g->yx;
  g->lower = sl->z_first + sl->own_lo > 0;
  g->upper = sl->z_first + sl->own_hi < sl->z_total;
  g->J = g->lower ? (g->upper ? std::min(g->o0, g->Zl - g->o1) : g->o0) : (g->upper ? g->Zl - g->o1 : 0);
  const bool ok = g->o0 >= 0 && g->o1 > g->o0 && g->o1 <= g->Zl && sl->z_first >= 0 && sl->z_first + g->Zl <= sl->z_total &&
                  (g->lower ? g->o0 >= g->H : (g->o0 == 0 && sl->z_first == 0)) &&
                  (g->upper ? g->Zl - g->o1 >= g->H : (g->o1 == g->Zl && sl->z_first + g->Zl == sl->z_total)) &&
                  ((!g->lower && !g->upper) || g->o1 - g->o0 >= g->H);
  if (!ok) { if (c) c->err = "simulate_step_slab: inconsistent slab description (halo too thin, or owned range thinner than the halo)"; return TFL_EINVAL; }
  return TFL_OK;
}

long long msg_floats(const SlabGeom& g, const Halo* f, int n, bool to_lower, bool send) {
  long long planes = 0;
  for (int i = 0; i < n; i++) {
    const int cnt = (to_lower == send) ? f[i].above : f[i].below;
    planes += (long long)f[i].t->B * f[i].t->C * cnt;
  }
  return planes * g.yx;
}

long long msg_layout(const SlabGeom& g, Msg* m, int count, float* base) {
  long long off = 0;
  auto take = [&](long long n) { float* p = base ? base + off : nullptr; off += (n + 3) & ~3ll; return p; };
  for (int i = 0; i < count; i++) {
    Msg& q = m[i];
    q.n_send_lo = g.lower ? msg_floats(g, q.f, q.n, true, true) : 0;
    q.n_recv_lo = g.lower ? msg_floats(g, q.f, q.n, true, false) : 0;
    q.n_send_hi = g.upper ? msg_floats(g, q.f, q.n, false, true) : 0;
    q.n_recv_hi = g.upper ? msg_floats(g, q.f, q.n, false, false) : 0;
    q.send_lo = take(q.n_send_lo); q.recv_lo = take(q.n_recv_lo); q.send_hi = take(q.n_send_hi); q.recv_hi = take(q.n_recv_hi);
  }
  return off;
}

void pack_msg(tfl_ctx* c, const SlabGeom& g, const Msg& q, bool unpack) {
  float* ptrs[20]; float* bufs[20]; int rows[20], zlo[20], np[20];
  int n = 0;
  for (int side = 0; side < 2; side++) {
    const bool lower = side == 0;
    if (lower ? !g.lower : !g.upper) continue;
    float* buf = unpack ? (lower ? q.recv_lo : q.recv_hi) : (lower ? q.send_lo : q.send_hi);
    for (int i = 0; i < q.n; i++) {
      const Halo& h = q.f[i];
      ptrs[n] = h.t->data; rows[n] = h.t->B * h.t->C;
      if (!unpack) { np[n] = lower ? h.above : h.below; zlo[n] = lower ? g.o0 : g.o1 - h.below; }
      else { np[n] = lower ? h.below : h.above; zlo[n] = lower ? g.o0 - h.below : g.o1; }
      bufs[n] = buf;
      buf += (long long)rows[n] * np[n] * g.yx;
      n++;
    }
  }
  for (int i = 0; i < n; i += 8)
    tfl::pack_planes(c->stream, std::min(8, n - i), ptrs + i, rows + i, zlo + i, np + i, g.yx * g.Zl, g.yx, nullptr, unpack ? 1 : 0, bufs + i);
}

int msg_chunks(const SlabGeom& g, const Msg& q, bool lower, bool send, tfl_comm_chunk* out) {
  if (lower ? !g.lower : !g.upper) return 0;
  int n = 0;
  for (int i = 0; i < q.n; i++) {
    const Halo& h = q.f[i];
    int np, zlo;
    if (send) { np = lower ? h.above : h.below; zlo = lower ? g.o0 : g.o1 - h.below; }
    else { np = lower ? h.below : h.above; zlo = lower ? g.o0 - h.below : g.o1; }
    for (int row = 0; row < h.t->B * h.t->C; row++) {
      out[n].ptr = h.t->data + ((long long)row * g.Zl + zlo) * g.yx;
      out[n].n = (long long)np * g.yx;
      n++;
    }
  }
  return n;
}
constexpr int kMaxChunks = 64;

static inline decltype(tfl_comm::exchange_start_v) start_v_of(const tfl_comm* comm) {
  return comm->size >= (int32_t)(offsetof(tfl_comm, exchange_start_v) + sizeof(comm->exchange_start_v)) ? comm->exchange_start_v : nullptr;
}

int msg_start(tfl_ctx* c, const SlabGeom& g, const tfl_comm* comm, const Msg& q) {
  if ((!g.lower && !g.upper) || q.n == 0) return TFL_OK;
  if (auto start_v = start_v_of(comm)) {
    int rows = 0;
    for (int i = 0; i < q.n; i++) rows += q.f[i].t->B * q.f[i].t->C;
    if (q.n > 0 && rows <= kMaxChunks) {
      tfl_comm_chunk slo[kMaxChunks], rlo[kMaxChunks], shi[kMaxChunks], rhi[kMaxChunks];
      const int n_lo = msg_chunks(g, q, true, true, slo), n_hi = msg_chunks(g, q, false, true, shi);
      msg_chunks(g, q, true, false, rlo); msg_chunks(g, q, false, false, rhi);
      if (start_v(comm->user, q.tag, n_lo, slo, rlo, n_hi, shi, rhi) != 0) { c->err = "simulate_step_slab: comm callback failed (exchange_start_v)"; return TFL_EINVAL; }
      return TFL_OK;
    }
  }
  pack_msg(c, g, q, false);
  if (comm->exchange_start(comm->user, q.tag, q.send_lo, q.n_send_lo, q.recv_lo, q.n_recv_lo, q.send_hi, q.n_send_hi,
                           q.recv_hi, q.n_recv_hi) != 0) { c->err = "simulate_step_slab: comm callback failed (exchange_start)"; return TFL_EINVAL; }
  return TFL_OK;
}
int msg_finish(tfl_ctx* c, const SlabGeom& g, const tfl_comm* comm, const Msg& q) {
  if ((!g.lower && !g.upper) || q.n == 0) return TFL_OK;
// ... 628 lines not shown
```

fluidnet_amd/csrc/tfl_ctx.hpp:

```cpp
#pragma once
#include <hip/hip_runtime.h>

#include <mutex>
#include <string>
#include <vector>

#include "tfl_host.hpp"

struct tfl_wall_plan {
  const float* flags = nullptr;
  unsigned short* code = nullptr;
  int B = 0, Z = 0, Y = 0, X = 0;
  bool is3d = false;
  struct tfl_ctx* owner = nullptr;
};

struct tfl_ctx {
  std::vector<tfl_wall_plan*> wall_plans;
  std::mutex wall_mu;
  int device = 0;
  hipStream_t stream = nullptr;
  std::string err;
  unsigned long long* d_trace_err = nullptr;
  double* d_resid = nullptr;
  double* h_resid = nullptr;
  float dx_override = 0.0f;
  int dx_dim = 0;
  tfl::ZWin zwin = {0, 0, 0, 0};
  tfl::ZOrigin zorigin = {0, 0};
  int advect_fast = 0;
  int stages = 0;
  float* d_reach = nullptr;
  float* h_reach = nullptr;
  float* d_reach_host = nullptr;
  unsigned* d_reach_tick = nullptr;
  bool reach_sink = false;
  bool reach_folded = false;
  unsigned reach_issued = 0;
  unsigned reach_hist[2] = {0, 0};
  double* h_reach_flags = nullptr;
  int needed_reach = 0;
  tfl::BcFoldArg fold = {nullptr, 0u, 0u};
  bool fold_done = false;
  tfl::BuoyFold buoy = {nullptr, 0.0f, 0.0f, 0.0f};
  bool buoy_done = false;
  bool vort_from_two_launch = false;
  int wf_skip = 0;
  int wf_timeouts = 0;
  bool defer_stats = false;
  bool in_step = false;
  bool capturing = false;
};
```

fluidnet_amd/csrc/tfl_host.hpp:

```cpp
#pragma once
#include <hip/hip_runtime.h>
#include <hip/hip_ext.h>

#include <cstdlib>

#include "tfl_device.hpp"

struct tfl_model;

namespace tfl {

inline const char* exp_env(const char* name) {
#ifdef TFL_EXPERIMENTS
  return getenv(name);
#else
  (void)name;
  return nullptr;
#endif
}

struct ZWin { int a0, a1, b0, b1; };
extern thread_local ZWin g_zwin;
struct ZOrigin { int first, total; };
extern thread_local ZOrigin g_zorigin;
extern thread_local int g_advect_fast;
struct BcFold { const float* bc; const float* inv; int x0, x1, y0, y1, z0, z1; };
struct BcFoldArg { const BcFold* dev; unsigned lo, hi; };
extern thread_local BcFoldArg g_fold;
extern thread_local bool g_fold_done;
inline BcFoldArg take_fold() { if (g_fold.dev) g_fold_done = true; return g_fold; }
inline BcFoldArg no_fold() { return BcFoldArg{nullptr, 0u, 0u}; }

struct BuoyFold { const float* rho; float sx, sy, sz; };
extern thread_local BuoyFold g_buoy;
extern thread_local bool g_buoy_done;
inline BuoyFold no_buoy() { return BuoyFold{nullptr, 0.0f, 0.0f, 0.0f}; }
inline BuoyFold take_buoy() { if (g_buoy.rho) g_buoy_done = true; return g_buoy; }

__device__ __forceinline__ bool fold_row(const BcFold& f, int j, int k) {
  return j >= f.y0 && j <= f.y1 && k >= f.z0 && k <= f.z1;
}
__device__ __forceinline__ bool fold_col(const BcFold& f, int i) { return i >= f.x0 && i <= f.x1; }
__device__ __forceinline__ bool fold_block(const BcFoldArg& a, int ya, int yb, int za, int zb) {
  return (a.dev != nullptr) & (ya <= (int)(a.hi & 0xffffu)) & (yb >= (int)(a.lo & 0xffffu)) & (za <= (int)(a.hi >> 16)) &
         (zb >= (int)(a.lo >> 16));
}

inline Dom make_dom(int Z, int Y, int X) {
  Dom d; d.X = X; d.Y = Y; d.Z = Z; d.sy = X; d.sz = X * Y; d.sc = X * Y * Z; d.one = 1;
  d.w0 = 0; d.n0 = Z; d.w1 = 0; d.nw = Z;
  d.zg = 0; d.Zg = Z;
  if (g_zorigin.total > 0) { d.zg = g_zorigin.first; d.Zg = g_zorigin.total; }
  const ZWin w = g_zwin;
  if (w.a1 > w.a0 || w.b1 > w.b0) {
    auto clip = [Z](int v) { return v < 0 ? 0 : (v > Z ? Z : v); };
    const int a0 = clip(w.a0), a1 = clip(w.a1) > a0 ? clip(w.a1) : a0;
    const int b0 = clip(w.b0), b1 = clip(w.b1) > b0 ? clip(w.b1) : b0;
    d.w0 = a0; d.n0 = a1 - a0; d.w1 = b0; d.nw = d.n0 + (b1 - b0);
  }
  return d;
}
inline int zwin_planes(int Z) { return make_dom(Z, 1, 1).nw; }

struct KernelTimer {
  KernelTimer(const char* name, hipStream_t st, bool ext = false);
  ~KernelTimer();
  hipEvent_t start() const;
  hipEvent_t stop() const;
  int slot_;
  hipStream_t st_;
  bool ext_;
};
#define TFL_TIMED(name, st) ::tfl::KernelTimer tfl_timer_(name, st)
#define TFL_TIMED_EXT(name, st) ::tfl::KernelTimer tfl_timer_(name, st, true)
#define TFL_LAUNCH_EXT(kernel, grid, block, shmem, st, ...)                                                        \
  do {                                                                                                             \
    if (tfl_timer_.start())                                                                                        \
      hipExtLaunchKernelGGL(kernel, dim3(grid), dim3(block), (uint32_t)(shmem), st, tfl_timer_.start(),            \
                            tfl_timer_.stop(), 0, __VA_ARGS__);                                                    \
    else                                                                                                           \
      hipLaunchKernelGGL(kernel, dim3(grid), dim3(block), (uint32_t)(shmem), st, __VA_ARGS__);                      \
  } while (0)

void advect_scalar(hipStream_t st, bool is3d, int method, int B, int Z, int Y, int X, float dt, float strength,
                   int outside, unsigned long long* err, const float* s, const float* U, const float* flags,
                   float* fwd, float* bounds, float* mm, float* dst, int stages = 7);
void advect_vel(hipStream_t st, bool is3d, int method, int B, int Z, int Y, int X, float dt, float strength,
                unsigned long long* err, const float* U, const float* flags, float* fwd, float* dst, int stages = 7);

void minmax3(hipStream_t st, bool is3d, int B, int Z, int Y, int X, int outside, const float* s, const float* flags,
             float* lo3, float* hi3);

void set_wall_bcs(hipStream_t st, bool is3d, int B, int Z, int Y, int X, float* U, const float* flags);
void velocity_divergence(hipStream_t st, bool is3d, int B, int Z, int Y, int X, const float* U, const float* flags,
                         float* div);
void velocity_update(hipStream_t st, bool is3d, int B, int Z, int Y, int X, float* U, const float* flags,
                     const float* p);
void set_wall_bcs_planes(hipStream_t st, int B, int Z, int Y, int X, int k0, int k1, float* U, const float* flags);
void velocity_divergence_planes(hipStream_t st, int B, int Z, int Y, int X, int k0, int k1, const float* U, const float* flags,
                                float* div);
void velocity_update_planes(hipStream_t st, int B, int Z, int Y, int X, int k0, int k1, float* U, const float* flags,
                            const float* p);
void add_buoyancy(hipStream_t st, bool is3d, int B, int Z, int Y, int X, const float* Usrc, float* U, const float* flags,
                  const float* density, float sx, float sy, float sz);
void add_gravity(hipStream_t st, bool is3d, int B, int Z, int Y, int X, float* U, const float* flags, float fx,
                 float fy, float fz);
void empty_domain(hipStream_t st, bool is3d, int bnd, int B, int Z, int Y, int X, float* flags);
void flags_to_occupancy(hipStream_t st, long long numel, const float* flags, float* occ);
void rectangular_blur(hipStream_t st, bool is3d, int B, int C, int Z, int Y, int X, int rad, const float* src, float* dst,
                      float* tmp);
void signed_distance_field(hipStream_t st, int B, int Z, int Y, int X, int rad, const float* flags, float* dst);
void stream_copy(hipStream_t st, long long n4, const float* src, float* dst);
void absmax(hipStream_t st, long long n, const float* x, float* out, bool reset);
void reach_flags(hipStream_t st, const float* maxu, float dt, int n, double* flags, const unsigned long long* range_count = nullptr);
void reach_publish(hipStream_t st, const float* src, float* dst, unsigned* tick);

bool vorticity_confinement(hipStream_t st, bool is3d, int B, int Z, int Y, int X, float* U, const float* flags,
                           float strength, float* curl, float* curl_norm, int stages = 3, const float* Usrc = nullptr);

bool vorticity_confinement_fused_ok(bool is3d, int Z, int Y, int X);
bool vorticity_confinement_fused(hipStream_t st, int B, int Z, int Y, int X, const float* Uin, float* Uout, const float* flags,
                                 float strength);

void jacobi_iteration(hipStream_t st, bool is3d, int B, int Z, int Y, int X, const float* p_prev, const float* flags,
                      const float* div, float* p, double* resid_sq );

void jacobi_sweep_slab(hipStream_t st, int B, int Z, int Y, int X, int zg, int Zg, int k0, int k1, const float* p_prev,
                       const float* flags, const float* div, float* p);

bool jacobi_solve_lds(hipStream_t st, int B, int Y, int X, const float* flags, const float* div, float* p, float* p_prev,
                      int iters, double* resid_sq);

long long pcg_workspace_floats(int Z, int Y, int X);
int pcg_solve(hipStream_t st, bool is3d, int B, int Z, int Y, int X, float* p, const float* flags, const float* div,
              int precond, float tol, int max_iter, int verbose, float* workspace, float* residual, char* msg, size_t msg_len, bool allow_wavefronts = true);

long long npm_workspace_floats(int Z, int Y, int X);
int normalize_pressure_mean(hipStream_t st, bool is3d, int B, int Z, int Y, int X, float* p, const float* flags,
                            float* workspace, char* msg, size_t msg_len);

long long model_stat_blocks(int B, int Z, int Y, int X);
bool model_stats_fold_requested();
long long model_stat_pairs_per_plane(int B, int Z, int Y, int X, const float* U, const float* flags, const float* Ubc, const float* div);
void model_pre(hipStream_t st, bool is3d, int B, int Z, int Y, int X, const float* U, const float* flags, float* Ubc,
               float* div, double* partials, double* stats, int zlo, int zhi, int stages = 3, unsigned* ticket = nullptr,
               const unsigned short* wall_code = nullptr);
void wall_code(hipStream_t st, bool is3d, int B, int Z, int Y, int X, const float* flags, unsigned short* code);
void model_net_input(hipStream_t st, bool is3d, int B, int Z, int Y, int X, const float* pDiv, const float* div,
                     const float* flags, const double* stats, double count, float* x3);
void model_net_input_gen(hipStream_t st, bool is3d, int B, int Z, int Y, int X, int in_pDiv, int in_UDiv, int in_div,
                         const float* pDiv, const float* Ubc, const float* div, const float* flags, const double* stats,
                         double count, float* x);
void model_field_stats(hipStream_t st, int B, long long n, const float* field, int mode, double* stats);
void model_skip_channel(hipStream_t st, int B, long long cells, const float* pDiv, const double* stats, double count,
                        float* dst, int och, int ch);
bool model_project(hipStream_t st, bool is3d, int B, int Z, int Y, int X, const float* pPred, const float* flags,
                   const double* stats, double count, float* Uio, float* pOut, const float* UBC, const float* UInvMask,
                   int do_clamp, float lo, float hi, const unsigned long long* range_src = nullptr,
                   unsigned long long* range_dst = nullptr, const float* reach_src = nullptr, float* reach_dst = nullptr,
                   float* reach_acc = nullptr, const unsigned short* wall_code = nullptr, unsigned* reach_tick = nullptr);
void apply_bcs(hipStream_t st, long long n, float* x, const float* bcv, const float* inv, int do_clamp, float lo,
               float hi);

void bc_scan(hipStream_t st, long long n, const float* bcv, const float* inv, int* counters, int* idx);
void apply_bcs_indexed_multi(hipStream_t st, int count, const long long* n, const int* const* idx, float* const* x,
                             const float* const* bcv, const float* const* inv);
void apply_bcs_indexed(hipStream_t st, long long n, const int* idx, float* x, const float* bcv, const float* inv);

long long pack_planes(hipStream_t st, int n, float* const* ptrs, const int* rows, const int* zlo, const int* nplanes,
                      long long zstride, long long yx, float* buf, int unpack, float* const* bufs = nullptr);

bool model_is_graph(const tfl_model* m);
int model_grid_factor(const tfl_model* m);

bool conv_direct(hipStream_t st, bool is3d, int B, int Z, int Y, int X, int cin, int cout, int ksz, int act,
                 const float* in, const float* w, const float* bias, float* out, int upf = 1, int sub = 0, int out_ch = 0);
void avg_pool2(hipStream_t st, bool is3d, int rows, int Z, int Y, int X, const float* in, float* out);
bool conv_direct_graph(hipStream_t st, bool is3d, int B, int Z, int Y, int X, int cin, int cout, int ksz, int act,
                       const float* in, const float* w, const float* bias, float* out, int upf, int sub, int out_ch, int c0,
                       int dil, const float* bn_s, const float* bn_t);
void pool2_graph(hipStream_t st, bool is3d, bool max, int B, int C, int Z, int Y, int X, const float* in, float* out, int och,
                 int c0, const float* bn_s, const float* bn_t);
constexpr int kMaxJoinBanks = 8;
bool bank_join(hipStream_t st, bool is3d, bool add, int B, int C, int Z, int Y, int X, int n, const int* slot, const int* sh,
               const float* const* src, float* out, int och);

void conv3_mfma_first(hipStream_t st, int B, int Z, int Y, int X, const float* in_planar3, const float* bfrag,
                      const float* bias, float* out_cl8);
void conv3_mfma_first_fused(hipStream_t st, int B, int Z, int Y, int X, const float* pDiv, const float* div,
                            const float* flags, const double* stats, double count, const float* bfrag,
                            const float* bias, float* out_cl8);
void conv3_mfma_mid(hipStream_t st, int B, int Z, int Y, int X, const float* in_cl8, const float* bfrag,
                    const float* bias, float* out_cl8);
void conv3_mfma_tail(hipStream_t st, int B, int Z, int Y, int X, const float* in_cl8, const float* bfrag,
                     const float* bias, const float* w4, const float* b4, const float* w5, const float* b5,
                     float* p_out);

void conv3_valu_first_fused(hipStream_t st, int B, int Z, int Y, int X, const float* pDiv, const float* div, const float* flags,
                            const double* stats, double count, const float* wq, const float* bias, float* out_p8);
void conv3_valu_mid(hipStream_t st, int B, int Z, int Y, int X, const float* in_p8, const float* wq, const float* bias,
                    float* out_p8);
void conv3_valu_tail(hipStream_t st, int B, int Z, int Y, int X, const float* in_p8, const float* wq, const float* tail_pack,
                     float* p_out);

void conv3_m16_first_fused(hipStream_t st, int B, int Z, int Y, int X, const float* pDiv, const float* div, const float* flags,
                           const double* stats, double count, const void* wfrag, const float* bias, float post, void* out_h2,
                           unsigned long long* range_err, const double* partials = nullptr, long long per_sample = 0,
                           double* stats_out = nullptr);
bool conv3_m16_first_sums_partials();
void conv3_m16_mid(hipStream_t st, int B, int Z, int Y, int X, const void* in_h2, const void* wfrag, const float* bias, float post,
                   void* out_h2, unsigned long long* range_err);
void conv3_m16_tail(hipStream_t st, int B, int Z, int Y, int X, const void* in_h2, const void* wfrag, const float* tail_pack,
                    float post, float* p_out, unsigned long long* range_err);
bool conv3_m16_first2_fused(hipStream_t st, int B, int Z, int Y, int X, const float* pDiv, const float* div, const float* flags,
                            const double* stats, double count, const void* wfrag1, const float* bias1, float post1,
                            const void* wfrag2, const float* bias2, float post2, void* out_h2, unsigned long long* range_err);
bool conv3_m16_fuse12_requested();
size_t conv3_m16_frag_halves(int cin);
float conv3_m16_pack_tail(const float* w4 , uint16_t* frag_buf_of_a_cin8_layer);
float conv3_m16_pack_weights(const float* w, int cin, uint16_t* out);

void velocity_divergence_bwd(hipStream_t st, bool is3d, int B, int Z, int Y, int X, const float* flags,
                             const float* grad_out, float* grad_U);
void velocity_update_bwd(hipStream_t st, bool is3d, int B, int Z, int Y, int X, const float* flags,
                         const float* grad_out, float* grad_p);
void upsample_nearest_fwd(hipStream_t st, int ratio, long long rows, int Zo, int Yo, int Xo, const float* in, float* out);
void upsample_nearest_bwd(hipStream_t st, int ratio, long long rows, int Zi, int Yi, int Xi, const float* go, float* gi);

void conv2_mfma_first_fused(hipStream_t st, int B, int Y, int X, const float* pDiv, const float* div, const float* flags,
                            const double* stats, double count, const float* bfrag, const float* bias, float* out16);
void conv2_mfma_mid(hipStream_t st, int B, int Y, int X, const float* in16, const float* bfrag, const float* bias,
                    float* out16);
void conv2_mfma_tail(hipStream_t st, int B, int Y, int X, const float* in16, const float* bfrag, const float* bias,
                     const float* w5, const float* b5, float* p_out);

}
```

fluidnet_amd/csrc/vorticity.hip:

```cpp
#include "tfl_device.hpp"
#include "tfl_fastmath.hpp"
#include "tfl_host.hpp"
#include "tfl_vec4.hpp"
#include <type_traits>

#include <atomic>
#include <cstdlib>

#ifndef TFL_LB_CURL
#define TFL_LB_CURL 1
#endif
#ifndef TFL_LB_CONFINE
#define TFL_LB_CONFINE 4
#endif

namespace tfl {

template <bool IS3D, int AXIS>
__device__ __forceinline__ float centred_c(const Dom& d, const float* __restrict__ U, int i, int j, int k) {
  if (on_border<IS3D>(d, i, j, k)) return 0.0f;
  const int a = TFL_AT(d, i, j, k) + AXIS * d.sc;
  const int step = AXIS == 0 ? 1 : (AXIS == 1 ? d.sy : d.sz);
  return 0.5f * (U[a] + U[a + step]);
}
// ... 337 lines not shown
    c_bits[r] = (in ? 1 : 0) | (gx + 1 == d.X - 1 ? 2 : 0) | (gx - 1 == 0 ? 4 : 0) | (gy + 1 == d.Y - 1 ? 8 : 0) | (gy - 1 == 0 ? 16 : 0);
  }
  const int f_it = (ty + 2) * FCX + tx + 2;
  const bool f_in = i >= 1 && i <= d.X - 2 && j >= 1 && j <= d.Y - 2;
  const bool e_col = tid < FBY, e_row = tid >= 64 && tid < 64 + FBX;
  const int e_cx = e_col ? 1 : (tid - 64) + 2, e_cy = e_col ? tid + 2 : 1;
  const int e_it = (e_col || e_row) ? e_cy * FCX + e_cx : f_it;
  const int e_gx = x0 - 2 + e_cx, e_gy = y0 - 2 + e_cy;
  const bool e_in = (e_col || e_row) && e_gx >= 1 && e_gx <= d.X - 2 && e_gy >= 1 && e_gy <= d.Y - 2;
  const int e_dst = e_col ? (tid + 1) * FEX : FEY * FEX + (tid - 64) + 1;
  const bool out_xy = i < d.X && j < d.Y;
  const int o_xy = TFL_AT(d, min(i, d.X - 1), min(j, d.Y - 1), 0);

  auto force = [&](int it, bool use, const float* cn0, const float* cnp, const float* cnm, const float* cv) -> v3 {
    const float* c0 = cn0 + it;
    v3 g = mk3(0.5f * (c0[1] - c0[-1]), 0.5f * (c0[FCX] - c0[-FCX]), 0.5f * (cnp[it] - cnm[it]));
    g = normalize3_x(g, use);
    const v3 w = mk3(cv[it], cv[FCN + it], cv[2 * FCN + it]);
    const v3 f = mk3(((g.y * w.z) - (g.z * w.y)) * strength, ((g.z * w.x) - (g.x * w.z)) * strength,
                     ((g.x * w.y) - (g.y * w.x)) * strength);
    return use ? f : mk3(0.0f, 0.0f, 0.0f);
  };

  float nu[2][3];
  auto load_plane = [&](int t) {
    const int gz = min(max(t, 0), d.Z - 1) * d.sz;
#pragma unroll
    for (int r = 0; r < 2; r++) {
      if (r == 1 && tid >= FUN - 512) continue;
      const int o = st_o[r] + gz;
      nu[r][0] = Uin[o]; nu[r][1] = Uin[o + d.sc]; nu[r][2] = Uin[o + 2 * d.sc];
    }
  };
  load_plane(za - 3);
  float fz_prev = 0.0f;
#pragma unroll 1
  for (int t = za - 3; t <= zb + 2; t++) {
    {
      float* dst = Ut + (t & 3) * 3 * FUN + tid;
      dst[0] = nu[0][0]; dst[FUN] = nu[0][1]; dst[2 * FUN] = nu[0][2];
      if (tid < FUN - 512) { dst[512] = nu[1][0]; dst[FUN + 512] = nu[1][1]; dst[2 * FUN + 512] = nu[1][2]; }
    }
    __syncthreads();
    load_plane(t + 1);
    const int zo = t - 3;
    const bool out_live = out_xy && zo >= za && zo < zb;
    const bool out_inner = out_live && f_in && zo >= 1 && zo <= d.Z - 2;
    float pu0 = 0.0f, pu1 = 0.0f, pu2 = 0.0f, pfc = 0.0f, pnx = 0.0f, pny = 0.0f, pnz = 0.0f;
    if (out_live) {
      const float* own = Ut + (zo & 3) * 3 * FUN + (ty + 3) * FUX + tx + 3;
      pu0 = own[0]; pu1 = own[FUN]; pu2 = own[2 * FUN];
      const int o = o_xy + zo * d.sz;
      if (out_inner) { pfc = flags[o]; pnx = flags[o - 1]; pny = flags[o - d.sy]; pnz = flags[o - d.sz]; }
    }
    const int zc = t - 2;
    if (zc >= za - 2 && zc <= zb) {
      const bool z_in = zc >= 1 && zc <= d.Z - 2, zpb = zc + 1 == d.Z - 1, zmb = zc - 1 == 0;
      const float* P0 = Ut + (zc & 3) * 3 * FUN;
      const float* Pp = Ut + ((zc + 1) & 3) * 3 * FUN;
      const float* Pm = Ut + ((zc - 1) & 3) * 3 * FUN;
      float* cvw = Cv + (zc & 1) * 3 * FCN;
      float* cnw = Cn + ((zc + 6) % 3) * FCN;
#pragma unroll
      for (int r = 0; r < 2; r++) {
        if (r == 1 && (tid & ~63) >= FCN - 512) continue;
        const bool ok = z_in && (c_bits[r] & 1) && (r == 0 || tid < FCN - 512);
        const bool xpb = c_bits[r] & 2, xmb = c_bits[r] & 4, ypb = c_bits[r] & 8, ymb = c_bits[r] & 16;
        const float* ux0 = P0 + c_base[r];
        const float* uy0 = ux0 + FUN;
        const float* uz0 = ux0 + 2 * FUN;
        const float* uxp = Pp + c_base[r];
        const float* uxm = Pm + c_base[r];
        const float y_xp0 = uy0[1], y_xp1 = uy0[1 + FUX], y_xm0 = uy0[-1], y_xm1 = uy0[-1 + FUX];
        const float x_yp0 = ux0[FUX], x_yp1 = ux0[FUX + 1], x_ym0 = ux0[-FUX], x_ym1 = ux0[-FUX + 1];
        const float z_yp0 = uz0[FUX], z_yp1 = uxp[2 * FUN + FUX], z_ym0 = uz0[-FUX], z_ym1 = uxp[2 * FUN - FUX];
        const float y_zp0 = uxp[FUN], y_zp1 = uxp[FUN + FUX], y_zm0 = uxm[FUN], y_zm1 = uxm[FUN + FUX];
        const float x_zp0 = uxp[0], x_zp1 = uxp[1], x_zm0 = uxm[0], x_zm1 = uxm[1];
        const float z_xp0 = uz0[1], z_xp1 = uxp[2 * FUN + 1], z_xm0 = uz0[-1], z_xm1 = uxp[2 * FUN - 1];
        const float cy_xp = xpb ? 0.0f : 0.5f * (y_xp0 + y_xp1);
        const float cy_xm = xmb ? 0.0f : 0.5f * (y_xm0 + y_xm1);
        const float cx_yp = ypb ? 0.0f : 0.5f * (x_yp0 + x_yp1);
        const float cx_ym = ymb ? 0.0f : 0.5f * (x_ym0 + x_ym1);
        v3 w;
        w.z = 0.5f * ((cy_xp - cy_xm) - (cx_yp - cx_ym));
        const float cz_yp = ypb ? 0.0f : 0.5f * (z_yp0 + z_yp1);
        const float cz_ym = ymb ? 0.0f : 0.5f * (z_ym0 + z_ym1);
        const float cy_zp = zpb ? 0.0f : 0.5f * (y_zp0 + y_zp1);
        const float cy_zm = zmb ? 0.0f : 0.5f * (y_zm0 + y_zm1);
        w.x = 0.5f * ((cz_yp - cz_ym) - (cy_zp - cy_zm));
        const float cx_zp = zpb ? 0.0f : 0.5f * (x_zp0 + x_zp1);
        const float cx_zm = zmb ? 0.0f : 0.5f * (x_zm0 + x_zm1);
        const float cz_xp = xpb ? 0.0f : 0.5f * (z_xp0 + z_xp1);
        const float cz_xm = xmb ? 0.0f : 0.5f * (z_xm0 + z_xm1);
        w.y = 0.5f * ((cx_zp - cx_zm) - (cz_xp - cz_xm));
        float nrm = norm3_x(w, ok);
        nrm = ok ? nrm : 0.0f;
        w = ok ? w : mk3(0.0f, 0.0f, 0.0f);
        if (r == 0 || tid < FCN - 512) {
          cvw[c_it[r]] = w.x; cvw[FCN + c_it[r]] = w.y; cvw[2 * FCN + c_it[r]] = w.z;
          cnw[c_it[r]] = nrm;
        }
      }
    }
    __syncthreads();
    const int zf = t - 3;
    v3 f0 = mk3(0.0f, 0.0f, 0.0f);
    if (zf >= za - 1 && zf <= zb - 1) {
      const bool z_in = zf >= 1 && zf <= d.Z - 2;
      const float* cn0 = Cn + ((zf + 6) % 3) * FCN;
      const float* cnp = Cn + ((zf + 7) % 3) * FCN;
      const float* cnm = Cn + ((zf + 5) % 3) * FCN;
      const float* cv = Cv + (zf & 1) * 3 * FCN;
      f0 = force(f_it, z_in && f_in, cn0, cnp, cnm, cv);
      Fe[(ty + 1) * FEX + tx + 1] = f0.x;
      Fe[(FEY + ty + 1) * FEX + tx + 1] = f0.y;
      if (tid < 128) {
        const v3 fe = force(e_it, z_in && e_in, cn0, cnp, cnm, cv);
        if (e_col || e_row) Fe[e_dst] = e_col ? fe.x : fe.y;
      }
    }
    __syncthreads();
    if (out_live) {
      float u0 = pu0, u1 = pu1, u2 = pu2;
      {
        const int fc = (int)pfc;
        const bool cf = fc & kFluid, ce = fc & kEmpty;
        const int nx = (int)pnx, ny = (int)pny, nz = (int)pnz;
        const bool any = out_inner && (cf || ce);
        const bool ax = any && ((nx & kFluid) || (cf && (nx & kEmpty)));
        const bool ay = any && ((ny & kFluid) || (cf && (ny & kEmpty)));
        const bool az = any && ((nz & kFluid) || (cf && (nz & kEmpty)));
        const float a0 = u0 + (0.5f * (Fe[(ty + 1) * FEX + tx] + f0.x));
        const float a1 = u1 + (0.5f * (Fe[(FEY + ty) * FEX + tx + 1] + f0.y));
        const float a2 = u2 + (0.5f * (fz_prev + f0.z));
        u0 = ax ? a0 : u0; u1 = ay ? a1 : u1; u2 = az ? a2 : u2;
      }
      const int o = o_xy + zf * d.sz;
      Uout[o] = u0; Uout[o + d.sc] = u1; Uout[o + 2 * d.sc] = u2;
    }
    fz_prev = f0.z;
  }
}

namespace {
__device__ __forceinline__ __amdgpu_buffer_rsrc_t gbuf(const void* p, long long bytes) {
  return __builtin_amdgcn_make_buffer_rsrc(const_cast<void*>(p), 0, (int)(unsigned)bytes, 0x00020000);
}
__device__ __forceinline__ float ldb(__amdgpu_buffer_rsrc_t r, unsigned lane_off, unsigned plane_off) {
  return __builtin_bit_cast(float, __builtin_amdgcn_raw_buffer_load_b32(r, (int)lane_off, (int)plane_off, 0));
}
__device__ __forceinline__ void stb(__amdgpu_buffer_rsrc_t r, unsigned lane_off, unsigned plane_off, float v) {
  __builtin_amdgcn_raw_buffer_store_b32(__builtin_bit_cast(unsigned, v), r, (int)lane_off, (int)plane_off, 0);
}
}

namespace {
template <int BX, int BY>
struct PipeGeo {
  static constexpr int PBX = BX, PBY = BY, NT = BX * BY;
  static constexpr int PCX = PBX + 3, PCY = PBY + 3, PCN = PCX * PCY;
  static constexpr int QX = PCX + 2, QY = PCY + 2, QN = QX * QY;
  static constexpr int PEX = PBX + 1, PEY = PBY + 1;
  static constexpr int kLds = (4 * 3 * QN + 4 * PCN + 3 * 3 * PCN + 2 * 2 * PEY * PEX) * 4;
  static constexpr int kE = BX == 64 ? 256 : 192, kER = BX == 64 ? 320 : kE + PBY;
  static_assert(QN <= 2 * NT && PCN <= 2 * NT && NT % 64 == 0, "two rounds cover the tiles");
};
constexpr int kPipeFill = 9;
}

template <int BX, int BY>
__global__ __launch_bounds__(BX * BY) void k_vort_pipe(Dom d, int cols_x, int cols_y, int cz, int chunks_a, int chunks, int n_blocks,
                                                    const float* __restrict__ Uin, float* __restrict__ Uout,
                                                    const float* __restrict__ flags, float strength, int xcd_order, BcFoldArg folda) {
  using G = PipeGeo<BX, BY>;
  constexpr int PBX = G::PBX, PBY = G::PBY, NT = G::NT, PCX = G::PCX, PCN = G::PCN, QX = G::QX, QN = G::QN, PEX = G::PEX, PEY = G::PEY;
  extern __shared__ float lds[];
  float* Cr = lds;
  float* Cn = Cr + 4 * 3 * QN;
  float* Cv = Cn + 4 * PCN;
  float* Fe = Cv + 3 * 3 * PCN;
  const int blk = xcd_order ? (int)xcd_contiguous(blockIdx.x, (unsigned)n_blocks) : (int)blockIdx.x;
  if (blk >= n_blocks) return;
  int tq = blk;
  const int bx = tq % cols_x; tq /= cols_x;
  const int by = tq % cols_y; tq /= cols_y;
  const int ch = tq % chunks;
  const int b = tq / chunks;
  const int za = ch < chunks_a ? d.w0 + ch * cz : d.w1 + (ch - chunks_a) * cz;
  const int z_end = ch < chunks_a ? d.w0 + d.n0 : d.w1 + (d.nw - d.n0);
  const int zb = min(za + cz, z_end);
  const int x0 = bx * PBX, y0 = by * PBY;
  const long long cells = d.sc;
  Uin += b * cells * 3; Uout += b * cells * 3; flags += b * cells;
  const int tid = threadIdx.x, tx = tid % PBX, ty = tid / PBX;
  const int wave = __builtin_amdgcn_readfirstlane(tid >> 6);
  const int i = x0 + tx, j = y0 + ty;

  constexpr int kS1 = NT - (QN - NT);
  const bool two_st = wave * 64 + 63 >= kS1;
  int st_it[2], st_o[2], st_ox[2], st_oy[2];
  bool st_sh[2];
  st_it[0] = tid; st_it[1] = tid >= kS1 ? NT + (tid - kS1) : tid;
#pragma unroll
  for (int r = 0; r < 2; r++) {
    const int qy = st_it[r] / QX, qx = st_it[r] - qy * QX;
    const int gx = x0 - 3 + qx, gy = y0 - 3 + qy;
    const int xa = min(max(gx, 0), d.X - 1), ya = min(max(gy, 0), d.Y - 1);
    st_o[r] = TFL_AT(d, xa, ya, 0);
    st_ox[r] = TFL_AT(d, min(xa + 1, d.X - 1), ya, 0);
    st_oy[r] = TFL_AT(d, xa, min(ya + 1, d.Y - 1), 0);
    st_sh[r] = gx <= 0 || gx >= d.X - 1 || gy <= 0 || gy >= d.Y - 1;
  }
  constexpr int kC1 = PCN - NT;
  int c_it[2], c_base[2];
  bool c_in[2];
#pragma unroll
  for (int r = 0; r < 2; r++) {
    const int it = min(tid + NT * r, PCN - 1);
    const int cy = it / PCX, cx = it - cy * PCX;
    const int gx = x0 - 2 + cx, gy = y0 - 2 + cy;
    c_it[r] = it;
    c_base[r] = (cy + 1) * QX + (cx + 1);
    c_in[r] = tid + NT * r < PCN && gx >= 1 && gx <= d.X - 2 && gy >= 1 && gy <= d.Y - 2;
  }
  const int f_it = (ty + 2) * PCX + tx + 2;
  const bool f_in = i >= 1 && i <= d.X - 2 && j >= 1 && j <= d.Y - 2;
  constexpr int kE = G::kE, kER = G::kER;
  const bool e_col = tid >= kE && tid < kE + PBY, e_row = tid >= kER && tid < kER + PBX;
  const bool e_wave = wave >= kE / 64 && wave <= (kER + PBX - 1) / 64;
  const int e_cx = e_col ? 1 : (tid - kER) + 2, e_cy = e_col ? (tid - kE) + 2 : 1;
  const int e_it = (e_col || e_row) ? e_cy * PCX + e_cx : f_it;
  const int e_gx = x0 - 2 + e_cx, e_gy = y0 - 2 + e_cy;
  const bool e_in = (e_col || e_row) && e_gx >= 1 && e_gx <= d.X - 2 && e_gy >= 1 && e_gy <= d.Y - 2;
  const int e_dst = e_col ? ((tid - kE) + 1) * PEX : PEY * PEX + (tid - kER) + 1;
  const bool out_xy = i < d.X && j < d.Y;
  const int o_xy = TFL_AT(d, min(i, d.X - 1), min(j, d.Y - 1), 0);
  const int o_safe = o_xy + (i >= 1 ? 0 : 1) + (j >= 1 ? 0 : d.sy);
  const unsigned st_o4[2] = {(unsigned)st_o[0] * 4u, (unsigned)st_o[1] * 4u}, st_ox4[2] = {(unsigned)st_ox[0] * 4u, (unsigned)st_ox[1] * 4u};
  const unsigned st_oy4[2] = {(unsigned)st_oy[0] * 4u, (unsigned)st_oy[1] * 4u};
  const unsigned o_xy4 = (unsigned)o_xy * 4u, o_safe4 = (unsigned)o_safe * 4u, o_safe_x4 = (unsigned)(o_safe - 1) * 4u, o_safe_y4 = (unsigned)(o_safe - d.sy) * 4u;
  const unsigned sc4 = (unsigned)d.sc * 4u, sz4 = (unsigned)d.sz * 4u;
  const __amdgpu_buffer_rsrc_t rU = gbuf(Uin, cells * 12), rF = gbuf(flags, cells * 4), wU = gbuf(Uout, cells * 12);
  const bool fold_blk = fold_block(folda, y0, y0 + PBY - 1, za, zb - 1);
  BcFold fold = {nullptr, nullptr, 0, -1, 0, -1, 0, -1};
  if (fold_blk) { fold = *folda.dev; fold.bc += b * cells * 3; fold.inv += b * cells * 3; }
  const bool fold_xy = fold_blk && out_xy && j >= fold.y0 && j <= fold.y1 && fold_col(fold, i);

  auto force = [&](int it, bool use, const float* cn0, const float* cnp, const float* cnm, const float* cv) -> v3 {
    const float* c0 = cn0 + it;
    v3 g = mk3(0.5f * (c0[1] - c0[-1]), 0.5f * (c0[PCX] - c0[-PCX]), 0.5f * (cnp[it] - cnm[it]));
    g = normalize3_x(g, use);
    const v3 w = mk3(cv[it], cv[PCN + it], cv[2 * PCN + it]);
    const v3 f = mk3(((g.y * w.z) - (g.z * w.y)) * strength, ((g.z * w.x) - (g.x * w.z)) * strength,
                     ((g.x * w.y) - (g.y * w.x)) * strength);
    return use ? f : mk3(0.0f, 0.0f, 0.0f);
  };

  float nl[2][5];
  auto load_plane = [&](int t) {
    const unsigned px = (unsigned)min(max(t, 0), d.Z - 1) * sz4, py = px + sc4, pzc = py + sc4;
#pragma unroll
    for (int r = 0; r < 2; r++) {
      if (r == 1 && !two_st) continue;
      nl[r][0] = ldb(rU, st_o4[r], px); nl[r][1] = ldb(rU, st_ox4[r], px); nl[r][2] = ldb(rU, st_o4[r], py); nl[r][3] = ldb(rU, st_oy4[r], py);
      nl[r][4] = ldb(rU, st_o4[r], pzc);
    }
  };
  const int t0 = za - 3, t1 = zb + 5;
  float cxp[2] = {0.0f, 0.0f}, cyp[2] = {0.0f, 0.0f}, uzp[2] = {0.0f, 0.0f};
  float fn[3] = {0.0f, 0.0f, 0.0f}, fzc = 0.0f, un[3] = {0.0f, 0.0f, 0.0f};
  v3 fcar = mk3(0.0f, 0.0f, 0.0f);
  float fzcar = 0.0f;
  int cv3 = ((t0 - 3) % 3 + 3) % 3;
  auto step = [&](int t, auto steady_tag) {
    constexpr bool STEADY = decltype(steady_tag)::value;
    const int zo = t - 6;
    const bool out_act = STEADY || (zo >= za && zo < zb);
    const bool out_live = out_xy && out_act;
    const bool out_inner = out_live && f_in && zo >= 1 && zo <= d.Z - 2;
    float pfc = 0.0f, pnx = 0.0f, pny = 0.0f, pnz = 0.0f, pu0 = 0.0f, pu1 = 0.0f, pu2 = 0.0f;
    if (out_act) { pfc = out_inner ? fn[0] : 0.0f; pnx = out_inner ? fn[1] : 0.0f; pny = out_inner ? fn[2] : 0.0f; pnz = out_inner ? fzc : 0.0f; }
    pu0 = un[0]; pu1 = un[1]; pu2 = un[2];
    if (STEADY || (zo + 1 >= za && zo + 1 < zb)) {
      fzc = fn[0];
      const unsigned pz = (unsigned)min(max(zo + 1, 0), d.Z - 1) * sz4;
      fn[0] = ldb(rF, o_safe4, pz); fn[1] = ldb(rF, o_safe_x4, pz); fn[2] = ldb(rF, o_safe_y4, pz);
      un[0] = ldb(rU, o_xy4, pz); un[1] = ldb(rU, o_xy4, pz + sc4); un[2] = ldb(rU, o_xy4, pz + 2u * sc4);
    }
    if (STEADY || t <= zb + 2) {
      const bool zsh = t - 1 <= 0 || t - 1 >= d.Z - 1;
      float* dst = Cr + ((t - 1) & 3) * 3 * QN;
#pragma unroll
      for (int r = 0; r < 2; r++) {
        if (r == 1 && !two_st) continue;
        const float cxn = 0.5f * (nl[r][0] + nl[r][1]), cyn = 0.5f * (nl[r][2] + nl[r][3]);
        const float czp = 0.5f * (uzp[r] + nl[r][4]);
        const bool z0 = zsh || st_sh[r];
        if (STEADY || t > t0) { dst[st_it[r]] = z0 ? 0.0f : cxp[r]; dst[QN + st_it[r]] = z0 ? 0.0f : cyp[r]; dst[2 * QN + st_it[r]] = z0 ? 0.0f : czp; }
        cxp[r] = cxn; cyp[r] = cyn; uzp[r] = nl[r][4];
      }
      if (STEADY || t <= zb + 1) load_plane(t + 1);
    }
    const int zc = t - 3;
    if (STEADY || (zc >= za - 2 && zc <= zb)) {
      const bool z_in = zc >= 1 && zc <= d.Z - 2;
      const float* P0 = Cr + (zc & 3) * 3 * QN;
      const float* Pp = Cr + ((zc + 1) & 3) * 3 * QN;
      const float* Pm = Cr + ((zc - 1) & 3) * 3 * QN;
      float* cvw = Cv + cv3 * 3 * PCN;
      float* cnw = Cn + (zc & 3) * PCN;
#pragma unroll
      for (int r = 0; r < 2; r++) {
        if (r == 1 && wave * 64 >= kC1) continue;
        const bool mine = r == 0 || tid < kC1;
        const bool ok = z_in && c_in[r] && mine;
        const float* q0 = P0 + c_base[r];
        const float* qp = Pp + c_base[r];
        const float* qm = Pm + c_base[r];
        const float cy_xp = q0[QN + 1], cy_xm = q0[QN - 1], cx_yp = q0[QX], cx_ym = q0[-QX];
        const float cz_yp = q0[2 * QN + QX], cz_ym = q0[2 * QN - QX], cy_zp = qp[QN], cy_zm = qm[QN];
        const float cx_zp = qp[0], cx_zm = qm[0], cz_xp = q0[2 * QN + 1], cz_xm = q0[2 * QN - 1];
        v3 w;
        w.z = 0.5f * ((cy_xp - cy_xm) - (cx_yp - cx_ym));
        w.x = 0.5f * ((cz_yp - cz_ym) - (cy_zp - cy_zm));
        w.y = 0.5f * ((cx_zp - cx_zm) - (cz_xp - cz_xm));
        float nrm = norm3_x(w, ok);
        nrm = ok ? nrm : 0.0f;
        w = ok ? w : mk3(0.0f, 0.0f, 0.0f);
        if (mine) {
          cvw[c_it[r]] = w.x; cvw[PCN + c_it[r]] = w.y; cvw[2 * PCN + c_it[r]] = w.z;
          cnw[c_it[r]] = nrm;
        }
      }
    }
    const int zf = t - 5;
    v3 f0 = mk3(0.0f, 0.0f, 0.0f);
    if (STEADY || (zf >= za - 1 && zf <= zb - 1)) {
      const bool z_in = zf >= 1 && zf <= d.Z - 2;
      const float* cn0 = Cn + (zf & 3) * PCN;
      const float* cnp = Cn + ((zf + 1) & 3) * PCN;
      const float* cnm = Cn + ((zf - 1) & 3) * PCN;
      const int cvf = cv3 >= 2 ? cv3 - 2 : cv3 + 1;
      const float* cv = Cv + cvf * 3 * PCN;
      float* fe = Fe + (zf & 1) * 2 * PEY * PEX;
      f0 = force(f_it, z_in && f_in, cn0, cnp, cnm, cv);
      fe[(ty + 1) * PEX + tx + 1] = f0.x;
      fe[(PEY + ty + 1) * PEX + tx + 1] = f0.y;
      if (e_wave) {
        const v3 fq = force(e_it, z_in && e_in, cn0, cnp, cnm, cv);
        if (e_col || e_row) fe[e_dst] = e_col ? fq.x : fq.y;
      }
    }
    if (out_act) {
      const float* fe = Fe + (zo & 1) * 2 * PEY * PEX;
      float u0 = pu0, u1 = pu1, u2 = pu2;
      const int fc = (int)pfc;
      const bool cf = fc & kFluid, ce = fc & kEmpty;
      const int nx = (int)pnx, ny = (int)pny, nz = (int)pnz;
      const bool any = out_inner && (cf || ce);
      const bool ax = any && ((nx & kFluid) || (cf && (nx & kEmpty)));
      const bool ay = any && ((ny & kFluid) || (cf && (ny & kEmpty)));
      const bool az = any && ((nz & kFluid) || (cf && (nz & kEmpty)));
      const float a0 = u0 + (0.5f * (fe[(ty + 1) * PEX + tx] + fcar.x));
      const float a1 = u1 + (0.5f * (fe[(PEY + ty) * PEX + tx + 1] + fcar.y));
      const float a2 = u2 + (0.5f * (fzcar + fcar.z));
      u0 = ax ? a0 : u0; u1 = ay ? a1 : u1; u2 = az ? a2 : u2;
      if (fold_blk) {
        const bool fq = fold_xy && out_live && zo >= fold.z0 && zo <= fold.z1;
        const long long o = fq ? (long long)zo * d.sz + o_xy : 0;
        const float m0 = fold.inv[o], m1 = fold.inv[o + d.sc], m2 = fold.inv[o + 2 * d.sc];
        const float b0 = fold.bc[o], b1 = fold.bc[o + d.sc], b2 = fold.bc[o + 2 * d.sc];
        const float g0 = u0 * m0 + b0, g1 = u1 * m1 + b1, g2 = u2 * m2 + b2;
        u0 = fq ? g0 : u0; u1 = fq ? g1 : u1; u2 = fq ? g2 : u2;
      }
      if (out_live) {
        const unsigned po = (unsigned)zo * sz4;
        stb(wU, o_xy4, po, u0); stb(wU, o_xy4, po + sc4, u1); stb(wU, o_xy4, po + 2u * sc4, u2);
      }
    }
    fzcar = fcar.z; fcar = f0;
    cv3 = cv3 == 2 ? 0 : cv3 + 1;
    __syncthreads();
  };
  const int ts = min(max(za + 6, t0), t1 + 1), te = min(zb + 1, t1);
#ifdef TFL_VORT_TIMING
  long long tk[40]; int nk = 0;
  tk[nk++] = wall_clock64();
#define TFL_VT() if (nk < 40) tk[nk++] = wall_clock64()
#else
#define TFL_VT()
#endif
  {
    float pl[4][2][5];
#pragma unroll
    for (int q = 0; q < 4; q++) {
      const unsigned px = (unsigned)min(max(t0 + q, 0), d.Z - 1) * sz4, py = px + sc4, pzc = py + sc4;
#pragma unroll
      for (int r = 0; r < 2; r++) {
        if (r == 1 && !two_st) continue;
        pl[q][r][0] = ldb(rU, st_o4[r], px); pl[q][r][1] = ldb(rU, st_ox4[r], px); pl[q][r][2] = ldb(rU, st_o4[r], py); pl[q][r][3] = ldb(rU, st_oy4[r], py);
        pl[q][r][4] = ldb(rU, st_o4[r], pzc);
      }
    }
    load_plane(za + 1);
    fn[0] = ldb(rF, o_safe4, (unsigned)min(max(za - 1, 0), d.Z - 1) * sz4);
#pragma unroll
    for (int q = 0; q < 3; q++) {
      const int pz = t0 + q;
      const bool zsh = pz <= 0 || pz >= d.Z - 1;
      float* dst = Cr + (pz & 3) * 3 * QN;
#pragma unroll
      for (int r = 0; r < 2; r++) {
        if (r == 1 && !two_st) continue;
        const float cx = 0.5f * (pl[q][r][0] + pl[q][r][1]), cy = 0.5f * (pl[q][r][2] + pl[q][r][3]);
        const float cz = 0.5f * (pl[q][r][4] + pl[q + 1][r][4]);
        const bool z0 = zsh || st_sh[r];
        dst[st_it[r]] = z0 ? 0.0f : cx; dst[QN + st_it[r]] = z0 ? 0.0f : cy; dst[2 * QN + st_it[r]] = z0 ? 0.0f : cz;
      }
    }
#pragma unroll
    for (int r = 0; r < 2; r++) {
      if (r == 1 && !two_st) continue;
      cxp[r] = 0.5f * (pl[3][r][0] + pl[3][r][1]); cyp[r] = 0.5f * (pl[3][r][2] + pl[3][r][3]); uzp[r] = pl[3][r][4];
    }
    cv3 = (cv3 + 4) % 3;
    __syncthreads();
  }
  TFL_VT();
  int t = za + 1;
#pragma unroll 1
  for (; t < ts; t++) { step(t, std::false_type{}); TFL_VT(); }
#pragma unroll 1
  for (; t <= te; t++) { step(t, std::true_type{}); TFL_VT(); }
#pragma unroll 1
  for (; t <= t1; t++) { step(t, std::false_type{}); TFL_VT(); }
#ifdef TFL_VORT_TIMING
  if (tid == 0 && (blk == 0 || blk == n_blocks / 2 + 3)) {
    for (int q = 1; q < nk; q++) printf("vt blk %d step %d (t-za %d) %lld\n", blk, q - 1, q - 1, tk[q] - tk[q - 1]);
  }
#endif
}

static int vort_fused_slots() {
  static std::atomic<int> slots_of[64];
  int dev = 0;
  (void)hipGetDevice(&dev);
  if (dev < 0 || dev >= 64) dev = 0;
  int slots = slots_of[dev].load();
  if (!slots) {
    int cus = 256, per = 0;
    (void)hipDeviceGetAttribute(&cus, hipDeviceAttributeMultiprocessorCount, dev);
    const bool attr_ok = hipFuncSetAttribute((const void*)k_vort_fused, hipFuncAttributeMaxDynamicSharedMemorySize, kFusedLds) == hipSuccess;
    if (!attr_ok || hipOccupancyMaxActiveBlocksPerMultiprocessor(&per, (const void*)k_vort_fused, 512, kFusedLds) != hipSuccess || per <= 0) {
      (void)hipGetLastError();
      slots = -1;
    } else slots = cus * per;
    slots_of[dev].store(slots);
  }
  return slots > 0 ? slots : 0;
}

template <int BX, int BY>
static int vort_pipe_slots_of() {
  static std::atomic<int> slots_of[64];
  int dev = 0;
  (void)hipGetDevice(&dev);
  if (dev < 0 || dev >= 64) dev = 0;
  int slots = slots_of[dev].load();
  if (!slots) {
    int cus = 256, per = 0;
    (void)hipDeviceGetAttribute(&cus, hipDeviceAttributeMultiprocessorCount, dev);
    using G = PipeGeo<BX, BY>;
    const bool attr_ok = hipFuncSetAttribute((const void*)k_vort_pipe<BX, BY>, hipFuncAttributeMaxDynamicSharedMemorySize, G::kLds) == hipSuccess;
    if (!attr_ok || hipOccupancyMaxActiveBlocksPerMultiprocessor(&per, (const void*)k_vort_pipe<BX, BY>, G::NT, G::kLds) != hipSuccess || per <= 0) {
      (void)hipGetLastError();
      slots = -1;
    } else slots = cus * per;
    slots_of[dev].store(slots);
  }
  return slots > 0 ? slots : 0;
}

static int vort_pipe_slots() { return vort_pipe_slots_of<64, 16>(); }

static int march_chunk(long long tiles, int na, int nb, int slots, int fill, int cmin) {
  int cz = cmin;
  long long best = -1;
  for (int c = cmin; c <= 64; c++) {
    const long long blocks = tiles * ((na + c - 1) / c + (nb + c - 1) / c);
    const long long cost = ((blocks + slots - 1) / slots) * (c + fill);
    if (best < 0 || cost < best) { best = cost; cz = c; }
  }
  return cz;
}


template <int BX, int BY>
static bool launch_vort_pipe(hipStream_t st, const Dom& d, int B, int X, int Y, int na, int nb, const float* Uin, float* Uout,
                             const float* flags, float strength, int xcd_order) {
  using G = PipeGeo<BX, BY>;
  const int pslots = vort_pipe_slots_of<BX, BY>();
  const int pcx = (X + BX - 1) / BX, pcy = (Y + BY - 1) / BY;
  const long long tiles = (long long)pcx * pcy * B;
  if (pslots <= 0 || tiles * (na + nb) <= 0) return false;
  if ((long long)d.Z * Y * X * 12 >= (1ll << 32)) return false;
  int cz = march_chunk(tiles, na, nb, pslots, kPipeFill, 4);
  if (const char* e = exp_env("TFL_VORT_CZ")) cz = atoi(e) > 0 ? atoi(e) : cz;
  const int chunks_a = (na + cz - 1) / cz, chunks = chunks_a + (nb + cz - 1) / cz;
  const int n_blocks = (int)(pcx * pcy * chunks * B);
  TFL_TIMED_EXT("k_vort_fused", st);
  const BcFoldArg fold = take_fold();
  TFL_LAUNCH_EXT((k_vort_pipe<BX, BY>), n_blocks, G::NT, G::kLds, st, d, pcx, pcy, cz, chunks_a, chunks, n_blocks, Uin, Uout, flags, strength, xcd_order, fold);
  return true;
}

bool vorticity_confinement_fused_ok(bool is3d, int Z, int Y, int X) {
  static const int mode = getenv("TFL_VORT_FUSED") ? atoi(getenv("TFL_VORT_FUSED")) : -1;
  static const int pipe_mode = getenv("TFL_VORT_PIPE") ? atoi(getenv("TFL_VORT_PIPE")) : -1;
  if (!is3d || Z < 3 || mode == 0) return false;
  const long long cells = (long long)Z * Y * X;
  const bool pipe = pipe_mode != 0 && vort_pipe_slots() > 0;
  if (mode == 1) return pipe || vort_fused_slots() > 0;
  if (pipe && cells >= 2000000ll && Z >= 32) return true;
  if (pipe && cells >= 600000ll && Z >= 32 && X % PipeGeo<64, 16>::PBX == 0 && Y % PipeGeo<64, 16>::PBY == 0) return true;
  return cells >= 3000000ll && (pipe || vort_fused_slots() > 0);
}

bool vorticity_confinement_fused(hipStream_t st, int B, int Z, int Y, int X, const float* Uin, float* Uout, const float* flags,
                                 float strength) {
  if (Z < 3 || Uin == Uout) return false;
  const Dom d = make_dom(Z, Y, X);
  const int na = d.n0, nb = d.nw - d.n0;
  const int xcd_order = xcd_order_enabled() ? 1 : 0;
  static const int pipe_mode = getenv("TFL_VORT_PIPE") ? atoi(getenv("TFL_VORT_PIPE")) : -1;
  if (pipe_mode != 0) {
#ifdef TFL_EXPERIMENTS
    static const int tile = exp_env("TFL_VORT_TILE") ? atoi(exp_env("TFL_VORT_TILE")) : 64;
    if (tile == 32 && launch_vort_pipe<32, 16>(st, d, B, X, Y, na, nb, Uin, Uout, flags, strength, xcd_order)) return true;
#endif
    if (launch_vort_pipe<64, 16>(st, d, B, X, Y, na, nb, Uin, Uout, flags, strength, xcd_order)) return true;
  }
  const int cxn = (X + FBX - 1) / FBX, cyn = (Y + FBY - 1) / FBY;
  if ((long long)cxn * cyn * (na + nb) * B <= 0) return true;
  const int slots = vort_fused_slots();
  if (slots <= 0) return false;
  int cz = march_chunk((long long)cxn * cyn * B, na, nb, slots, 6, 4);
  if (const char* e = exp_env("TFL_VORT_CZ")) cz = atoi(e) > 0 ? atoi(e) : cz;
  const int chunks_a = (na + cz - 1) / cz, chunks = chunks_a + (nb + cz - 1) / cz;
  const int n_blocks = cxn * cyn * chunks * B;
  TFL_TIMED_EXT("k_vort_fused", st);
  TFL_LAUNCH_EXT(k_vort_fused, n_blocks, 512, kFusedLds, st, d, cxn, cyn, cz, chunks_a, chunks, n_blocks, Uin, Uout, flags, strength, xcd_order);
  return true;
}

bool vorticity_confinement(hipStream_t st, bool is3d, int B, int Z, int Y, int X, float* U, const float* flags,
                           float strength, float* curl, float* curl_norm, int stages, const float* Usrc) {
  const Dom d = make_dom(Z, Y, X);
  const dim3 blk(64, 4, 1), grd((X + 63) / 64, (Y + 3) / 4, (unsigned)(d.nw * B));
  const float* Uin = Usrc ? Usrc : U;
  const Vec4Launch v = vec4_launch(B, Z, Y, X, {U, flags, curl, curl_norm, Uin});
  const bool pa = stages & 1, pb = stages & 2;
  if (v.ok) {
    const BcFoldArg fold = pb ? take_fold() : no_fold();
    const BlockOrder ord = make_block_order(v.grd.x, v.grd.y, v.grd.z, is3d && xcd_order_enabled(), xcd_run(v.grd.x, v.grd.y));
    if (is3d) {
      if (pa) { TFL_TIMED_EXT("k_curl", st); TFL_LAUNCH_EXT((k_curl_v4<true>), v.grd, v.blk, 0, st, d, Uin, curl, curl_norm, ord); }
      if (pb) { TFL_TIMED_EXT("k_confine", st); TFL_LAUNCH_EXT((k_confine_v4<true>), v.grd, v.blk, 0, st, d, Uin, U, flags, (const float*)curl, (const float*)curl_norm, strength, fold, ord); }
    } else {
      if (pa) { TFL_TIMED("k_curl", st); k_curl_v4<false><<<v.grd, v.blk, 0, st>>>(d, Uin, curl, curl_norm, ord); }
      if (pb) { TFL_TIMED("k_confine", st); k_confine_v4<false><<<v.grd, v.blk, 0, st>>>(d, Uin, U, flags, curl, curl_norm, strength, fold, ord); }
    }
    return true;
  }
  if (Usrc && Usrc != U) return false;
  if (is3d) {
    if (pa) { TFL_TIMED("k_curl", st); k_curl<true><<<grd, blk, 0, st>>>(d, U, curl, curl_norm); }
    if (pb) { TFL_TIMED("k_confine", st); k_confine<true><<<grd, blk, 0, st>>>(d, U, flags, curl, curl_norm, strength); }
  } else {
    if (pa) { TFL_TIMED("k_curl", st); k_curl<false><<<grd, blk, 0, st>>>(d, U, curl, curl_norm); }
    if (pb) { TFL_TIMED("k_confine", st); k_confine<false><<<grd, blk, 0, st>>>(d, U, flags, curl, curl_norm, strength); }
  }
  return true;
}

}
```

Measured before the change: 8550.

## Fold wall boundary zeroing into fused vorticity kernel and skip BC store in model_pre

The fused vorticity pipe kernel now reads the per-cell wall code and zeroes velocity components at wall cells before storing. The output is tracked in the context as already boundary-conditioned. model_pre can then launch a divergence+stats kernel that skips writing back the BC-applied velocity. This drops one full 3-channel velocity write pass per step, at the cost of a 16-bit code load per cell in the vorticity kernel and extra host-side state tracking that must be invalidated correctly.

```diff
diff --git a/fluidnet_amd/csrc/abi.cpp b/fluidnet_amd/csrc/abi.cpp
--- a/fluidnet_amd/csrc/abi.cpp
+++ b/fluidnet_amd/csrc/abi.cpp
@@ -461,9 +461,13 @@
     return fail(c, TFL_EINVAL, "vorticityConfinementFrom: curl must be a 3-channel grid of the flags size");
   TRY(check_scalar(c, "vorticityConfinementFrom", "curlNorm", curlNorm, flags));
   WindowScope win(c);
+  bool bcs_done = false;
   if (is3D && !c->vort_from_two_launch && tfl::vorticity_confinement_fused_ok(true, flags->Z, flags->Y, flags->X) &&
-      tfl::vorticity_confinement_fused(c->stream, flags->B, flags->Z, flags->Y, flags->X, USrc->data, U->data, flags->data, strength))
+      tfl::vorticity_confinement_fused(c->stream, flags->B, flags->Z, flags->Y, flags->X, USrc->data, U->data, flags->data, strength,
+                                       c->vort_bcs_code, &bcs_done)) {
+    if (bcs_done) { c->u_bc_code = c->vort_bcs_code; c->u_bc_data = U->data; }
     return check_launch(c, "vorticityConfinementFrom");
+  }
   const tfl::ZWin w0 = tfl::g_zwin;
   const bool windowed = w0.a1 > w0.a0 || w0.b1 > w0.b0;
   if (windowed) {
@@ -1137,12 +1141,16 @@
   return workspace + 4 * tfl::model_stat_blocks(B, Z, Y, X);
 }
 
-static const unsigned short* wall_code_of(tfl_ctx* c, const tfl_model* m, const tfl_tensor* flags) {
+}
+
+const unsigned short* wall_code_of(tfl_ctx* c, const tfl_model* m, const tfl_tensor* flags) {
   std::lock_guard<std::mutex> lock(c->wall_mu);
   for (const tfl_wall_plan* wp : c->wall_plans)
     if (wp->flags == flags->data && wp->is3d == m->is3d && wp->B == flags->B && wp->Z == flags->Z && wp->Y == flags->Y && wp->X == flags->X) return wp->code;
   return nullptr;
 }
+
+extern "C" {
 
 static int graph_gate(tfl_ctx* c, const tfl_model* m, const tfl_tensor* flags, const char* who) {
   if (!m->graph) return TFL_OK;
@@ -1170,8 +1178,11 @@
   if (c->defer_stats) stg &= ~4;
   m->stat_pairs_per_plane = tfl::model_stat_pairs_per_plane(flags->B, flags->Z, flags->Y, flags->X, UDiv->data, flags->data, UOut->data, w.div);
   const unsigned short* code = wall_code_of(c, m, flags);
+  const bool u_is_bc = code && c->u_bc_code == code && c->u_bc_data == UDiv->data && UDiv->data == UOut->data;
+  c->u_bc_code = nullptr; c->u_bc_data = nullptr;
   tfl::model_pre(c->stream, m->is3d, flags->B, flags->Z, flags->Y, flags->X, UDiv->data, flags->data, UOut->data,
-                 w.div, w.partials, stats ? stats : m->d_stats, zlo, zhi, ((stg & 2) ? 1 : 0) | ((stg & 4) ? 2 : 0), m->d_ticket, code);
+                 w.div, w.partials, stats ? stats : m->d_stats, zlo, zhi, ((stg & 2) ? 1 : 0) | ((stg & 4) ? 2 : 0), m->d_ticket, code,
+                 u_is_bc);
   return check_launch(c, "model_begin");
 }
 
diff --git a/fluidnet_amd/csrc/model.hip b/fluidnet_amd/csrc/model.hip
--- a/fluidnet_amd/csrc/model.hip
+++ b/fluidnet_amd/csrc/model.hip
@@ -173,79 +173,88 @@
   code[o] = (unsigned short)m;
 }
 
+#define TFL_BCS_DIV_STATS_CODE_BODY(IS3D, STORE_U) \
+  const V4Ctx c = v4_ctx(d); \
+  const int j = blockIdx.y * blockDim.y + threadIdx.y; \
+  int b, k; dom_bk(d, b, k); \
+  const bool live = c.i0 < d.X && j < d.Y; \
+  const long long cells = d.sc; \
+  const int C = IS3D ? 3 : 2; \
+  U += b * cells * C; Ubc += b * cells * C; code += b * cells; div += b * cells; \
+  const int o = TFL_AT(d, c.i0, j, k); \
+  const bool yp = live && j < d.Y - 1, zp = live && IS3D && k < d.Z - 1; \
+   \
+  const unsigned long long cc_v = *reinterpret_cast<const unsigned long long*>(code + (live ? o : 0));       \
+  const unsigned long long cy_v = *reinterpret_cast<const unsigned long long*>(code + (yp ? o + d.sy : 0)); \
+  const unsigned long long cz_v = *reinterpret_cast<const unsigned long long*>(code + (zp ? o + d.sz : 0)); \
+  const unsigned long long cc = live ? cc_v : 0ull, cy = yp ? cy_v : 0ull, cz = zp ? cz_v : 0ull; \
+  float u[3][4], uyp[4], uzp[4]; \
+_Pragma("unroll") \
+  for (int a = 0; a < 3; a++) v4_load(U, o + a * d.sc, live && a < C, 0.0f, u[a]); \
+  v4_load(U, o + d.sc + d.sy, yp, 0.0f, uyp); \
+  v4_load(U, o + 2 * d.sc + d.sz, zp, 0.0f, uzp); \
+  const bool need = c.last && live && c.has_r; \
+  const int oo = o + 4; \
+  const unsigned gcode = code[need ? oo : 0]; \
+  const float gu = U[need ? oo : 0]; \
+  double s1 = 0.0, s2 = 0.0; \
+  float ubx[5]; \
+_Pragma("unroll") \
+  for (int q = 0; q < 4; q++) { \
+    const unsigned m = (unsigned)(cc >> (16 * q)); \
+    if (m & 1u) u[0][q] = 0.0f; \
+    if (m & 2u) u[1][q] = 0.0f; \
+    if (!IS3D || (m & 4u)) u[2][q] = 0.0f; \
+    ubx[q] = u[0][q]; \
+    if (live) { \
+      s1 += (double)u[0][q] + (double)u[1][q] + (double)u[2][q]; \
+      s2 += (double)u[0][q] * u[0][q] + (double)u[1][q] * u[1][q] + (double)u[2][q] * u[2][q]; \
+    } \
+  } \
+  ubx[4] = from_lane_above(ubx[0]); \
+  if (c.last) ubx[4] = (need && !(gcode & 1u)) ? gu : 0.0f; \
+  float dv[4]; \
+  const bool row_inner = live && j >= 1 && j <= d.Y - 2 && (!IS3D || (k >= 1 && k <= d.Z - 2)); \
+_Pragma("unroll") \
+  for (int q = 0; q < 4; q++) { \
+    const int i = c.i0 + q; \
+    dv[q] = 0.0f; \
+    if (row_inner && i >= 1 && i <= d.X - 2 && ((unsigned)(cc >> (16 * q)) & 8u)) {    \
+      const float by = ((unsigned)(cy >> (16 * q)) & 2u) ? 0.0f : uyp[q]; \
+      float t = u[0][q] - ubx[q + 1] + u[1][q] - by; \
+      if (IS3D) { \
+        const float bz = ((unsigned)(cz >> (16 * q)) & 4u) ? 0.0f : uzp[q]; \
+        t += (u[2][q] - bz); \
+      } \
+      dv[q] = t; \
+    } \
+  } \
+  if (live) { \
+_Pragma("unroll") \
+    for (int a = 0; a < 3; a++) \
+      if (STORE_U && a < C) v4_store(Ubc, o + a * d.sc, u[a]); \
+    v4_store(div, o, dv); \
+  } \
+_Pragma("unroll") \
+  for (int off = 32; off > 0; off >>= 1) { s1 += __shfl_down(s1, off, 64); s2 += __shfl_down(s2, off, 64); } \
+  __shared__ double part[8]; \
+  const int tid = threadIdx.y * blockDim.x + threadIdx.x; \
+  if ((tid & 63) == 0) { part[(tid >> 6) * 2] = s1; part[(tid >> 6) * 2 + 1] = s2; } \
+  __syncthreads(); \
+  const long long blk = blockIdx.x + (long long)gridDim.x * (blockIdx.y + (long long)gridDim.y * ((long long)b * d.Z + k)); \
+  publish_and_maybe_reduce<false>(tl, partials, blk, (part[0] + part[2]) + (part[4] + part[6]), (part[1] + part[3]) + (part[5] + part[7]), tid);
 template <bool IS3D>
 __global__ __launch_bounds__(256, TFL_LB_BCS) void k_bcs_div_stats_code(Dom d, const float* __restrict__ U, const unsigned short* __restrict__ code,
                                                                        float* __restrict__ Ubc, float* __restrict__ div,
                                                                        double* __restrict__ partials, StatTail tl) {
-  const V4Ctx c = v4_ctx(d);
-  const int j = blockIdx.y * blockDim.y + threadIdx.y;
-  int b, k; dom_bk(d, b, k);
-  const bool live = c.i0 < d.X && j < d.Y;
-  const long long cells = d.sc;
-  const int C = IS3D ? 3 : 2;
-  U += b * cells * C; Ubc += b * cells * C; code += b * cells; div += b * cells;
-  const int o = TFL_AT(d, c.i0, j, k);
-  const bool yp = live && j < d.Y - 1, zp = live && IS3D && k < d.Z - 1;
-  const unsigned long long cc_v = *reinterpret_cast<const unsigned long long*>(code + (live ? o : 0));
-  const unsigned long long cy_v = *reinterpret_cast<const unsigned long long*>(code + (yp ? o + d.sy : 0));
-  const unsigned long long cz_v = *reinterpret_cast<const unsigned long long*>(code + (zp ? o + d.sz : 0));
-  const unsigned long long cc = live ? cc_v : 0ull, cy = yp ? cy_v : 0ull, cz = zp ? cz_v : 0ull;
-  float u[3][4], uyp[4], uzp[4];
-#pragma unroll
-  for (int a = 0; a < 3; a++) v4_load(U, o + a * d.sc, live && a < C, 0.0f, u[a]);
-  v4_load(U, o + d.sc + d.sy, yp, 0.0f, uyp);
-  v4_load(U, o + 2 * d.sc + d.sz, zp, 0.0f, uzp);
-  const bool need = c.last && live && c.has_r;
-  const int oo = o + 4;
-  const unsigned gcode = code[need ? oo : 0];
-  const float gu = U[need ? oo : 0];
-  double s1 = 0.0, s2 = 0.0;
-  float ubx[5];
-#pragma unroll
-  for (int q = 0; q < 4; q++) {
-    const unsigned m = (unsigned)(cc >> (16 * q));
-    if (m & 1u) u[0][q] = 0.0f;
-    if (m & 2u) u[1][q] = 0.0f;
-    if (!IS3D || (m & 4u)) u[2][q] = 0.0f;
-    ubx[q] = u[0][q];
-    if (live) {
-      s1 += (double)u[0][q] + (double)u[1][q] + (double)u[2][q];
-      s2 += (double)u[0][q] * u[0][q] + (double)u[1][q] * u[1][q] + (double)u[2][q] * u[2][q];
-    }
-  }
-  ubx[4] = from_lane_above(ubx[0]);
-  if (c.last) ubx[4] = (need && !(gcode & 1u)) ? gu : 0.0f;
-  float dv[4];
-  const bool row_inner = live && j >= 1 && j <= d.Y - 2 && (!IS3D || (k >= 1 && k <= d.Z - 2));
-#pragma unroll
-  for (int q = 0; q < 4; q++) {
-    const int i = c.i0 + q;
-    dv[q] = 0.0f;
-    if (row_inner && i >= 1 && i <= d.X - 2 && ((unsigned)(cc >> (16 * q)) & 8u)) {
-      const float by = ((unsigned)(cy >> (16 * q)) & 2u) ? 0.0f : uyp[q];
-      float t = u[0][q] - ubx[q + 1] + u[1][q] - by;
-      if (IS3D) {
-        const float bz = ((unsigned)(cz >> (16 * q)) & 4u) ? 0.0f : uzp[q];
-        t += (u[2][q] - bz);
-      }
-      dv[q] = t;
-    }
-  }
-  if (live) {
-#pragma unroll
-    for (int a = 0; a < 3; a++)
-      if (a < C) v4_store(Ubc, o + a * d.sc, u[a]);
-    v4_store(div, o, dv);
-  }
-#pragma unroll
-  for (int off = 32; off > 0; off >>= 1) { s1 += __shfl_down(s1, off, 64); s2 += __shfl_down(s2, off, 64); }
-  __shared__ double part[8];
-  const int tid = threadIdx.y * blockDim.x + threadIdx.x;
-  if ((tid & 63) == 0) { part[(tid >> 6) * 2] = s1; part[(tid >> 6) * 2 + 1] = s2; }
-  __syncthreads();
-  const long long blk = blockIdx.x + (long long)gridDim.x * (blockIdx.y + (long long)gridDim.y * ((long long)b * d.Z + k));
-  publish_and_maybe_reduce<false>(tl, partials, blk, (part[0] + part[2]) + (part[4] + part[6]), (part[1] + part[3]) + (part[5] + part[7]), tid);
-}
+  TFL_BCS_DIV_STATS_CODE_BODY(IS3D, true)
+}
+__global__ __launch_bounds__(256, TFL_LB_BCS) void k_div_stats_code(Dom d, const float* __restrict__ U, const unsigned short* __restrict__ code,
+                                                                   float* __restrict__ Ubc, float* __restrict__ div,
+                                                                   double* __restrict__ partials, StatTail tl) {
+  TFL_BCS_DIV_STATS_CODE_BODY(true, false)
+}
+#undef TFL_BCS_DIV_STATS_CODE_BODY
 
 template <bool IS3D, bool FOLD = false>
 __global__ __launch_bounds__(256, TFL_LB_BCS) void k_bcs_div_stats_v4(Dom d, const float* __restrict__ U, const float* __restrict__ flags,
@@ -731,7 +740,8 @@
 }
 
 void model_pre(hipStream_t st, bool is3d, int B, int Z, int Y, int X, const float* U, const float* flags, float* Ubc,
-               float* div, double* partials, double* stats, int zlo, int zhi, int stages, unsigned* ticket, const unsigned short* code) {
+               float* div, double* partials, double* stats, int zlo, int zhi, int stages, unsigned* ticket, const unsigned short* code,
+               bool u_is_bc) {
   const Dom d = make_dom(Z, Y, X);
   const dim3 blk(64, 4, 1), grd = TFL_GRID3(d, B);
   const Vec4Launch v = vec4_launch(B, Z, Y, X, {U, flags, Ubc, div});
@@ -746,7 +756,10 @@
   StatTail tl = {nullptr, stats, per_plane * Z, (unsigned)per_plane, (unsigned)(Z * B), B};
   if (fused) tl.ticket = ticket;
   if (stages & 1) {
-    if (v.ok && code && !fused) {
+    if (v.ok && code && !fused && u_is_bc && is3d && U == Ubc) {
+      TFL_TIMED_EXT("k_div_stats", st);
+      TFL_LAUNCH_EXT(k_div_stats_code, v.grd, v.blk, 0, st, d, U, code, Ubc, div, partials, tl);
+    } else if (v.ok && code && !fused) {
       TFL_TIMED_EXT("k_bcs_div_stats", st);
       if (is3d) TFL_LAUNCH_EXT((k_bcs_div_stats_code<true>), v.grd, v.blk, 0, st, d, U, code, Ubc, div, partials, tl);
       else TFL_LAUNCH_EXT((k_bcs_div_stats_code<false>), v.grd, v.blk, 0, st, d, U, code, Ubc, div, partials, tl);
diff --git a/fluidnet_amd/csrc/simulate.cpp b/fluidnet_amd/csrc/simulate.cpp
--- a/fluidnet_amd/csrc/simulate.cpp
+++ b/fluidnet_amd/csrc/simulate.cpp
@@ -73,6 +73,11 @@
   for (int i = 0; i < s->n_density; i++)
     if (!((density_done >> i) & 1u)) add(s->density[i], s->densityBC[i], un.density);
   return apply_bcs(c, todo, n);
+}
+
+static bool vort_bcs_enabled() {
+  const char* e = tfl::exp_env("TFL_VORT_BCS");
+  return !(e && atoi(e) == 0);
 }
 
 bool fold_ask(tfl_ctx* c, const tfl_bc_plan* p) {
@@ -262,13 +267,15 @@
     rc = tfl_addGravity(c, cur, s->flags, g, prm->dt, is3D, nullptr);
     if (rc) return rc;
   }
+  c->u_bc_code = nullptr; c->u_bc_data = nullptr;
   if (vort) {
     const float strength = (float)(dx * prm->vorticityConfinementAmp);
     if (fold_forces) fold_ask(c, s->UBC);
     if (cur != s->U) {
       c->vort_from_two_launch = !vfused;
+      c->vort_bcs_code = (vfused && fold_forces && s->model && z.is3d && vort_bcs_enabled()) ? wall_code_of(c, s->model, s->flags) : nullptr;
       rc = tfl_vorticityConfinementFrom(c, cur, s->U, s->flags, strength, &curl, &cnorm, is3D);
-      c->vort_from_two_launch = false;
+      c->vort_from_two_launch = false; c->vort_bcs_code = nullptr;
     } else {
       tfl_tensor centered = view(ws + 4 * z.N, (int)z.C), force = view(ws + (4 + z.C) * z.N, (int)z.C);
       rc = tfl_vorticityConfinement(c, s->U, s->flags, strength, &centered, &curl, &cnorm, &force, is3D);
@@ -288,6 +295,7 @@
     rc = tfl_setWallBcsForward(c, s->U, s->flags, is3D);
     if (rc) return rc;
   }
+  if (!U_folded && s->UBC) { c->u_bc_code = nullptr; c->u_bc_data = nullptr; }
   rc = set_const_vals(c, s, cur, !U_folded, Unchanged{true, false, true});
   if (rc) return rc;
   const int max_iter = prm->maxIter > 0 ? prm->maxIter : 100;
@@ -298,6 +306,7 @@
     const tfl_tensor* umask = (s->UBC && !late_ubc) ? &s->UBC->inv : nullptr;
     if (late_ubc) fold_ask(c, s->UBC);
     rc = tfl_model_forward(c, s->model, s->p, cur, s->flags, s->p, s->U, ws, ws_floats, ubc, umask, 1, -1e6f, 1e6f);
+    c->u_bc_code = nullptr; c->u_bc_data = nullptr;
     const bool folded = fold_took(c);
     if (rc) return rc;
     return set_const_vals(c, s, s->U, late_ubc && !folded, Unchanged{false, false, true});
diff --git a/fluidnet_amd/csrc/tfl_ctx.hpp b/fluidnet_amd/csrc/tfl_ctx.hpp
--- a/fluidnet_amd/csrc/tfl_ctx.hpp
+++ b/fluidnet_amd/csrc/tfl_ctx.hpp
@@ -45,9 +45,14 @@
   tfl::BuoyFold buoy = {nullptr, 0.0f, 0.0f, 0.0f};
   bool buoy_done = false;
   bool vort_from_two_launch = false;
+  const unsigned short* vort_bcs_code = nullptr;
+  const unsigned short* u_bc_code = nullptr;
+  const float* u_bc_data = nullptr;
   int wf_skip = 0;
   int wf_timeouts = 0;
   bool defer_stats = false;
   bool in_step = false;
   bool capturing = false;
 };
+
+const unsigned short* wall_code_of(tfl_ctx* c, const tfl_model* m, const tfl_tensor* flags);
diff --git a/fluidnet_amd/csrc/tfl_host.hpp b/fluidnet_amd/csrc/tfl_host.hpp
--- a/fluidnet_amd/csrc/tfl_host.hpp
+++ b/fluidnet_amd/csrc/tfl_host.hpp
@@ -120,7 +120,7 @@
 
 bool vorticity_confinement_fused_ok(bool is3d, int Z, int Y, int X);
 bool vorticity_confinement_fused(hipStream_t st, int B, int Z, int Y, int X, const float* Uin, float* Uout, const float* flags,
-                                 float strength);
+                                 float strength, const unsigned short* code = nullptr, bool* bcs_done = nullptr);
 
 void jacobi_iteration(hipStream_t st, bool is3d, int B, int Z, int Y, int X, const float* p_prev, const float* flags,
                       const float* div, float* p, double* resid_sq );
@@ -144,7 +144,7 @@
 long long model_stat_pairs_per_plane(int B, int Z, int Y, int X, const float* U, const float* flags, const float* Ubc, const float* div);
 void model_pre(hipStream_t st, bool is3d, int B, int Z, int Y, int X, const float* U, const float* flags, float* Ubc,
                float* div, double* partials, double* stats, int zlo, int zhi, int stages = 3, unsigned* ticket = nullptr,
-               const unsigned short* wall_code = nullptr);
+               const unsigned short* wall_code = nullptr, bool u_is_bc = false);
 void wall_code(hipStream_t st, bool is3d, int B, int Z, int Y, int X, const float* flags, unsigned short* code);
 void model_net_input(hipStream_t st, bool is3d, int B, int Z, int Y, int X, const float* pDiv, const float* div,
                      const float* flags, const double* stats, double count, float* x3);
diff --git a/fluidnet_amd/csrc/vorticity.hip b/fluidnet_amd/csrc/vorticity.hip
--- a/fluidnet_amd/csrc/vorticity.hip
+++ b/fluidnet_amd/csrc/vorticity.hip
@@ -513,6 +513,9 @@
 __device__ __forceinline__ void stb(__amdgpu_buffer_rsrc_t r, unsigned lane_off, unsigned plane_off, float v) {
   __builtin_amdgcn_raw_buffer_store_b32(__builtin_bit_cast(unsigned, v), r, (int)lane_off, (int)plane_off, 0);
 }
+__device__ __forceinline__ unsigned ldb16(__amdgpu_buffer_rsrc_t r, unsigned lane_off, unsigned plane_off) {
+  return (unsigned)__builtin_amdgcn_raw_buffer_load_b16(r, (int)lane_off, (int)plane_off, 0);
+}
 }
 
 namespace {
@@ -529,10 +532,11 @@
 constexpr int kPipeFill = 9;
 }
 
-template <int BX, int BY>
+template <int BX, int BY, bool BCS>
 __global__ __launch_bounds__(BX * BY) void k_vort_pipe(Dom d, int cols_x, int cols_y, int cz, int chunks_a, int chunks, int n_blocks,
                                                     const float* __restrict__ Uin, float* __restrict__ Uout,
-                                                    const float* __restrict__ flags, float strength, int xcd_order, BcFoldArg folda) {
+                                                    const float* __restrict__ flags, float strength, int xcd_order, BcFoldArg folda,
+                                                    const unsigned short* __restrict__ code) {
   using G = PipeGeo<BX, BY>;
   constexpr int PBX = G::PBX, PBY = G::PBY, NT = G::NT, PCX = G::PCX, PCN = G::PCN, QX = G::QX, QN = G::QN, PEX = G::PEX, PEY = G::PEY;
   extern __shared__ float lds[];
@@ -602,6 +606,8 @@
   const unsigned o_xy4 = (unsigned)o_xy * 4u, o_safe4 = (unsigned)o_safe * 4u, o_safe_x4 = (unsigned)(o_safe - 1) * 4u, o_safe_y4 = (unsigned)(o_safe - d.sy) * 4u;
   const unsigned sc4 = (unsigned)d.sc * 4u, sz4 = (unsigned)d.sz * 4u;
   const __amdgpu_buffer_rsrc_t rU = gbuf(Uin, cells * 12), rF = gbuf(flags, cells * 4), wU = gbuf(Uout, cells * 12);
+  const __amdgpu_buffer_rsrc_t rC = gbuf(BCS ? code + b * cells : nullptr, BCS ? cells * 2 : 0);
+  const unsigned o_xy2 = (unsigned)o_xy * 2u, sz2 = (unsigned)d.sz * 2u;
   const bool fold_blk = fold_block(folda, y0, y0 + PBY - 1, za, zb - 1);
   BcFold fold = {nullptr, nullptr, 0, -1, 0, -1, 0, -1};
   if (fold_blk) { fold = *folda.dev; fold.bc += b * cells * 3; fold.inv += b * cells * 3; }
@@ -630,6 +636,7 @@
   const int t0 = za - 3, t1 = zb + 5;
   float cxp[2] = {0.0f, 0.0f}, cyp[2] = {0.0f, 0.0f}, uzp[2] = {0.0f, 0.0f};
   float fn[3] = {0.0f, 0.0f, 0.0f}, fzc = 0.0f, un[3] = {0.0f, 0.0f, 0.0f};
+  unsigned cn = 0u;
   v3 fcar = mk3(0.0f, 0.0f, 0.0f);
   float fzcar = 0.0f;
   int cv3 = ((t0 - 3) % 3 + 3) % 3;
@@ -642,11 +649,13 @@
     float pfc = 0.0f, pnx = 0.0f, pny = 0.0f, pnz = 0.0f, pu0 = 0.0f, pu1 = 0.0f, pu2 = 0.0f;
     if (out_act) { pfc = out_inner ? fn[0] : 0.0f; pnx = out_inner ? fn[1] : 0.0f; pny = out_inner ? fn[2] : 0.0f; pnz = out_inner ? fzc : 0.0f; }
     pu0 = un[0]; pu1 = un[1]; pu2 = un[2];
+    const unsigned pcode = cn;
     if (STEADY || (zo + 1 >= za && zo + 1 < zb)) {
       fzc = fn[0];
       const unsigned pz = (unsigned)min(max(zo + 1, 0), d.Z - 1) * sz4;
       fn[0] = ldb(rF, o_safe4, pz); fn[1] = ldb(rF, o_safe_x4, pz); fn[2] = ldb(rF, o_safe_y4, pz);
       un[0] = ldb(rU, o_xy4, pz); un[1] = ldb(rU, o_xy4, pz + sc4); un[2] = ldb(rU, o_xy4, pz + 2u * sc4);
+      if (BCS) cn = ldb16(rC, o_xy2, (unsigned)min(max(zo + 1, 0), d.Z - 1) * sz2);
     }
     if (STEADY || t <= zb + 2) {
       const bool zsh = t - 1 <= 0 || t - 1 >= d.Z - 1;
@@ -734,6 +743,9 @@
         const float g0 = u0 * m0 + b0, g1 = u1 * m1 + b1, g2 = u2 * m2 + b2;
         u0 = fq ? g0 : u0; u1 = fq ? g1 : u1; u2 = fq ? g2 : u2;
       }
+      if (BCS) {
+        u0 = (pcode & 1u) ? 0.0f : u0; u1 = (pcode & 2u) ? 0.0f : u1; u2 = (pcode & 4u) ? 0.0f : u2;
+      }
       if (out_live) {
         const unsigned po = (unsigned)zo * sz4;
         stb(wU, o_xy4, po, u0); stb(wU, o_xy4, po + sc4, u1); stb(wU, o_xy4, po + 2u * sc4, u2);
@@ -821,7 +833,7 @@
   return slots > 0 ? slots : 0;
 }
 
-template <int BX, int BY>
+template <int BX, int BY, bool BCS = false>
 static int vort_pipe_slots_of() {
   static std::atomic<int> slots_of[64];
   int dev = 0;
@@ -832,8 +844,8 @@
     int cus = 256, per = 0;
     (void)hipDeviceGetAttribute(&cus, hipDeviceAttributeMultiprocessorCount, dev);
     using G = PipeGeo<BX, BY>;
-    const bool attr_ok = hipFuncSetAttribute((const void*)k_vort_pipe<BX, BY>, hipFuncAttributeMaxDynamicSharedMemorySize, G::kLds) == hipSuccess;
-    if (!attr_ok || hipOccupancyMaxActiveBlocksPerMultiprocessor(&per, (const void*)k_vort_pipe<BX, BY>, G::NT, G::kLds) != hipSuccess || per <= 0) {
+    const bool attr_ok = hipFuncSetAttribute((const void*)k_vort_pipe<BX, BY, BCS>, hipFuncAttributeMaxDynamicSharedMemorySize, G::kLds) == hipSuccess;
+    if (!attr_ok || hipOccupancyMaxActiveBlocksPerMultiprocessor(&per, (const void*)k_vort_pipe<BX, BY, BCS>, G::NT, G::kLds) != hipSuccess || per <= 0) {
       (void)hipGetLastError();
       slots = -1;
     } else slots = cus * per;
@@ -842,7 +854,7 @@
   return slots > 0 ? slots : 0;
 }
 
-static int vort_pipe_slots() { return vort_pipe_slots_of<64, 16>(); }
+static int vort_pipe_slots() { return vort_pipe_slots_of<64, 16, false>(); }
 
 static int march_chunk(long long tiles, int na, int nb, int slots, int fill, int cmin) {
   int cz = cmin;
@@ -858,9 +870,9 @@
 
 template <int BX, int BY>
 static bool launch_vort_pipe(hipStream_t st, const Dom& d, int B, int X, int Y, int na, int nb, const float* Uin, float* Uout,
-                             const float* flags, float strength, int xcd_order) {
+                             const float* flags, float strength, int xcd_order, const unsigned short* code) {
   using G = PipeGeo<BX, BY>;
-  const int pslots = vort_pipe_slots_of<BX, BY>();
+  const int pslots = code ? vort_pipe_slots_of<BX, BY, true>() : vort_pipe_slots_of<BX, BY, false>();
   const int pcx = (X + BX - 1) / BX, pcy = (Y + BY - 1) / BY;
   const long long tiles = (long long)pcx * pcy * B;
   if (pslots <= 0 || tiles * (na + nb) <= 0) return false;
@@ -869,9 +881,15 @@
   if (const char* e = exp_env("TFL_VORT_CZ")) cz = atoi(e) > 0 ? atoi(e) : cz;
   const int chunks_a = (na + cz - 1) / cz, chunks = chunks_a + (nb + cz - 1) / cz;
   const int n_blocks = (int)(pcx * pcy * chunks * B);
-  TFL_TIMED_EXT("k_vort_fused", st);
   const BcFoldArg fold = take_fold();
-  TFL_LAUNCH_EXT((k_vort_pipe<BX, BY>), n_blocks, G::NT, G::kLds, st, d, pcx, pcy, cz, chunks_a, chunks, n_blocks, Uin, Uout, flags, strength, xcd_order, fold);
+  if (code) {
+    TFL_TIMED_EXT("k_vort_bcs", st);
+    TFL_LAUNCH_EXT((k_vort_pipe<BX, BY, true>), n_blocks, G::NT, G::kLds, st, d, pcx, pcy, cz, chunks_a, chunks, n_blocks, Uin, Uout, flags, strength, xcd_order, fold, code);
+  } else {
+    TFL_TIMED_EXT("k_vort_fused", st);
+    TFL_LAUNCH_EXT((k_vort_pipe<BX, BY, false>), n_blocks, G::NT, G::kLds, st, d, pcx, pcy, cz, chunks_a, chunks, n_blocks, Uin, Uout, flags, strength, xcd_order, fold,
+                   (const unsigned short*)nullptr);
+  }
   return true;
 }
 
@@ -888,7 +906,8 @@
 }
 
 bool vorticity_confinement_fused(hipStream_t st, int B, int Z, int Y, int X, const float* Uin, float* Uout, const float* flags,
-                                 float strength) {
+                                 float strength, const unsigned short* code, bool* bcs_done) {
+  if (bcs_done) *bcs_done = false;
   if (Z < 3 || Uin == Uout) return false;
   const Dom d = make_dom(Z, Y, X);
   const int na = d.n0, nb = d.nw - d.n0;
@@ -897,9 +916,15 @@
   if (pipe_mode != 0) {
 #ifdef TFL_EXPERIMENTS
     static const int tile = exp_env("TFL_VORT_TILE") ? atoi(exp_env("TFL_VORT_TILE")) : 64;
-    if (tile == 32 && launch_vort_pipe<32, 16>(st, d, B, X, Y, na, nb, Uin, Uout, flags, strength, xcd_order)) return true;
+    if (tile == 32 && launch_vort_pipe<32, 16>(st, d, B, X, Y, na, nb, Uin, Uout, flags, strength, xcd_order, code)) {
+      if (bcs_done) *bcs_done = code != nullptr;
+      return true;
+    }
 #endif
-    if (launch_vort_pipe<64, 16>(st, d, B, X, Y, na, nb, Uin, Uout, flags, strength, xcd_order)) return true;
+    if (launch_vort_pipe<64, 16>(st, d, B, X, Y, na, nb, Uin, Uout, flags, strength, xcd_order, code)) {
+      if (bcs_done) *bcs_done = code != nullptr;
+      return true;
+    }
   }
   const int cxn = (X + FBX - 1) / FBX, cyn = (Y + FBY - 1) / FBY;
   if ((long long)cxn * cyn * (na + nb) * B <= 0) return true;
```

Result: faster. 8658 (median of 6 runs) (+1.3%).
